# ArturKKK/graphcast-lite

Measured on AMD Instinct MI355X. Metric: training samples/sec (6h windows) + achieved HBM GB/s on mesh GCNConv, higher is better.
Workload: dtype f32

## Files before the change

### graphcast-lite_amd/csrc/aggregate.hip

```cpp
#include <algorithm>

#include <atomic>

#include "common.h"
#include "halo.h"
#include "mfma_io.h"

namespace {

template <int LPR, bool VL, bool VS, bool PRES, bool SPLIT>
__device__ __forceinline__ void agg_heavy_row(const int row, const int b, const int32_t* __restrict__ rowptr,
                                              const int32_t* __restrict__ col, const float* __restrict__ w,
                                              const float* __restrict__ H, int64_t ldh, int64_t bsh,
                                              const float* __restrict__ bias, float* __restrict__ Y, int64_t ldy,
                                              int64_t bsy, int32_t F, const int32_t* __restrict__ present,
                                              const float* __restrict__ H2, int64_t ldh2, int64_t bsh2, int32_t head) {
  constexpr int NG = 256 / LPR;
  __shared__ float red[NG][LPR * 4 + 1];
  const int g = threadIdx.x / LPR, l = threadIdx.x % LPR;
  const int c0 = l * 4;
  const bool cactive = c0 < F;
  const int cc = cactive ? c0 : 0;
  const float* __restrict__ Hb = H + (int64_t)b * bsh;
  const float* __restrict__ H2b = SPLIT ? H2 + (int64_t)b * bsh2 : nullptr;
  const int start = rowptr[row], end = rowptr[row + 1];
  float a0 = 0.f, a1 = 0.f, a2 = 0.f, a3 = 0.f;
  auto ld4 = [&](int j, float& x0, float& x1, float& x2, float& x3) {
    const float* p = Hb + (int64_t)j * ldh + cc;
    if (PRES) p = present[j] >= 0 ? p : reinterpret_cast<const float*>(gcl::mfma_io::zero4);
    if (SPLIT) p = j < head ? p : H2b + (int64_t)(j - head) * ldh2 + cc;
    if (VL) {
      const float4 v = *reinterpret_cast<const float4*>(p);
      x0 = v.x; x1 = v.y; x2 = v.z; x3 = v.w;
    } else {
      x0 = p[0];
      x1 = (cc + 1 < F) ? p[1] : 0.f;
      x2 = (cc + 2 < F) ? p[2] : 0.f;
      x3 = (cc + 3 < F) ? p[3] : 0.f;
    }
  };
  for (int e = start + g; e < end; e += 4 * NG) {
    const int e1 = e + NG, e2 = e + 2 * NG, e3 = e + 3 * NG;
    const int j0 = col[e], j1 = col[e1 < end ? e1 : e], j2 = col[e2 < end ? e2 : e], j3 = col[e3 < end ? e3 : e];
    const float w0 = w[e], w1 = e1 < end ? w[e1] : 0.f, w2 = e2 < end ? w[e2] : 0.f, w3 = e3 < end ? w[e3] : 0.f;
    float p0, p1, p2, p3, q0, q1, q2, q3, r0, r1, r2, r3, s0, s1, s2, s3;
    ld4(j0, p0, p1, p2, p3);
    ld4(j1, q0, q1, q2, q3);
    ld4(j2, r0, r1, r2, r3);
    ld4(j3, s0, s1, s2, s3);
    a0 += w0 * p0; a1 += w0 * p1; a2 += w0 * p2; a3 += w0 * p3;
    if (e1 < end) { a0 += w1 * q0; a1 += w1 * q1; a2 += w1 * q2; a3 += w1 * q3; }
    if (e2 < end) { a0 += w2 * r0; a1 += w2 * r1; a2 += w2 * r2; a3 += w2 * r3; }
    if (e3 < end) { a0 += w3 * s0; a1 += w3 * s1; a2 += w3 * s2; a3 += w3 * s3; }
  }
  red[g][c0] = a0; red[g][c0 + 1] = a1; red[g][c0 + 2] = a2; red[g][c0 + 3] = a3;
  __syncthreads();
  if (g == 0 && cactive) {
    float t0 = 0.f, t1 = 0.f, t2 = 0.f, t3 = 0.f;
#pragma unroll
    for (int q = 0; q < NG; ++q) { t0 += red[q][c0]; t1 += red[q][c0 + 1]; t2 += red[q][c0 + 2]; t3 += red[q][c0 + 3]; }
    if (bias) {
      t0 += bias[c0];
      if (c0 + 1 < F) t1 += bias[c0 + 1];
      if (c0 + 2 < F) t2 += bias[c0 + 2];
      if (c0 + 3 < F) t3 += bias[c0 + 3];
    }
    float* yp = Y + (int64_t)b * bsy + (int64_t)row * ldy + c0;
    if (VS) {
      *reinterpret_cast<float4*>(yp) = make_float4(t0, t1, t2, t3);
    } else {
      yp[0] = t0;
      if (c0 + 1 < F) yp[1] = t1;
      if (c0 + 2 < F) yp[2] = t2;
      if (c0 + 3 < F) yp[3] = t3;
    }
  }
}
// ... 13 lines not shown
}

template <int LPR, bool VL, bool VS, int EW, int ITER, bool PRES = false, bool SPLIT = false, bool HV = false>
__global__ __launch_bounds__(256) void agg_kernel(const int32_t* __restrict__ rowptr, const int32_t* __restrict__ col,
                                                  const float* __restrict__ w, const int32_t* __restrict__ ecol,
                                                  const float* __restrict__ ew, const float* __restrict__ H,
                                                  int64_t ldh, int64_t bsh, const float* __restrict__ bias,
                                                  float* __restrict__ Y, int64_t ldy, int64_t bsy, int32_t n,
                                                  int32_t B, int32_t F, int32_t nRB, int32_t xcd_map,
                                                  int32_t nt_store, const int32_t* __restrict__ order16,
                                                  const int32_t* __restrict__ present = nullptr,
                                                  const float* __restrict__ H2 = nullptr, int64_t ldh2 = 0,
                                                  int64_t bsh2 = 0, int32_t head = 0,
                                                  const int32_t* __restrict__ rows_heavy = nullptr, int32_t n_heavy = 0,
                                                  int32_t n_hb = 0, int32_t n_hb_pad = 0) {
  static_assert(!(PRES && SPLIT), "absent rows and a two-part source are not combined");
  constexpr int RPW = 64 / LPR;
  constexpr int EL = LPR < gcl::kEll ? LPR : gcl::kEll;
  static_assert(EW <= EL, "ELL width exceeds the lanes of a row group");
  int bid = blockIdx.x;
  if (HV) {
    if (bid < n_hb) {
      agg_heavy_row<LPR, VL, VS, PRES, SPLIT>(rows_heavy[bid % n_heavy], bid / n_heavy, rowptr, col, w, H, ldh, bsh, bias, Y, ldy,
                                              bsy, F, present, H2, ldh2, bsh2, head);
      return;
    }
    if (bid < n_hb_pad) return;
    bid -= n_hb_pad;
  }
  int b, rb;
  if (xcd_map) {
    const int xcd = bid & (gcl::kNumXCD - 1);
    const int slot = bid >> 3;
    b = xcd + gcl::kNumXCD * (slot / nRB);
    rb = slot % nRB;
  } else {
    b = bid / nRB;
    rb = bid % nRB;
  }
  if (b >= B) return;
  if (order16) {
    constexpr int RPB = RPW * 4 * ITER, K = 16 / RPB;
    rb = order16[rb / (K > 0 ? K : 1)] * (K > 0 ? K : 1) + rb % (K > 0 ? K : 1);
  }
  const int lane = threadIdx.x & 63;
  const int wave = threadIdx.x >> 6;
  const int sub = lane / LPR;
  const int l = lane % LPR;
  const int gbase = sub * LPR;
  const int c0 = l * 4;
  const bool cactive = c0 < F;
  const int cc = cactive ? c0 : 0;
  const float* __restrict__ Hb = H + (int64_t)b * bsh;
  const float* __restrict__ H2b = SPLIT ? H2 + (int64_t)b * bsh2 : nullptr;
  float* __restrict__ Yb = Y + (int64_t)b * bsy;

  float bz0 = 0.f, bz1 = 0.f, bz2 = 0.f, bz3 = 0.f;
  if (bias && cactive) {
    bz0 = bias[c0];
    if (VS || c0 + 1 < F) bz1 = bias[c0 + 1];
    if (VS || c0 + 2 < F) bz2 = bias[c0 + 2];
    if (VS || c0 + 3 < F) bz3 = bias[c0 + 3];
  }

  auto ld4 = [&](int j, float& x0, float& x1, float& x2, float& x3) {
    const float* p = Hb + (int64_t)j * ldh + cc;
    if (PRES) p = j >= 0 ? p : reinterpret_cast<const float*>(gcl::mfma_io::zero4);
    if (SPLIT) p = j < head ? p : H2b + (int64_t)(j - head) * ldh2 + cc;
    if (VL) {
      const float4 v = *reinterpret_cast<const float4*>(p);
      x0 = v.x; x1 = v.y; x2 = v.z; x3 = v.w;
    } else {
      x0 = p[0];
      x1 = (cc + 1 < F) ? p[1] : 0.f;
      x2 = (cc + 2 < F) ? p[2] : 0.f;
      x3 = (cc + 3 < F) ? p[3] : 0.f;
    }
  };

  const int row_first = (rb * 4 + wave) * (RPW * ITER) + sub;
  auto meta = [&](int row, int& start, int& end, int& cj, float& wj) {
    const int rc = row < n ? row : n - 1;
    start = rowptr[rc];
    end = rowptr[rc + 1];
    cj = ecol[(int64_t)rc * gcl::kEll + (l & (EL - 1))];
    wj = ew[(int64_t)rc * gcl::kEll + (l & (EL - 1))];
    if (PRES) cj = present[cj] >= 0 ? cj : -1;
  };
  int start, end, cj;
  float wj;
  meta(row_first, start, end, cj, wj);

#pragma unroll 1
  for (int it = 0; it < ITER; ++it) {
    const int row = row_first + it * RPW;
    int nstart = 0, nend = 0, ncj = 0;
    float nwj = 0.f;
    if (it + 1 < ITER) meta(row + RPW, nstart, nend, ncj, nwj);

    const int deg_all = end - start;
    const bool heavy = deg_all > gcl::kHeavy;
    const int deg = heavy ? 0 : deg_all;
    if (heavy) end = start;
    float a0 = 0.f, a1 = 0.f, a2 = 0.f, a3 = 0.f;
    {
      int jj[EW];
      float ww[EW], v0[EW], v1[EW], v2[EW], v3[EW];
// ... 250 lines not shown
            a0 = __fmaf_rn(wk, v.x, a0);
            a1 = __fmaf_rn(wk, v.y, a1);
            a2 = __fmaf_rn(wk, v.z, a2);
            a3 = __fmaf_rn(wk, v.w, a3);
          }
        }
      }
#undef GCL_HALO_MULADD
#undef GCL_HALO_FMA
      if (row < n && cactive && !(last & gcl::kHaloSkip)) {
        a0 += bz0; a1 += bz1; a2 += bz2; a3 += bz3;
        float* __restrict__ yp = Yb + (int64_t)row * ldy + c0;
        if (SMAP) {
          const int cr = sm[SMAP ? it : 0];
          yp = cr >= 0 ? Yc + (int64_t)b * bsc + (int64_t)cr * ldc + c0 : yp;
        }
        v4f v = {a0, a1, a2, a3};
        if (nt_store) __builtin_nontemporal_store(v, reinterpret_cast<v4f*>(yp));
        else *reinterpret_cast<v4f*>(yp) = v;
      }
    }
    GCL_AGG_STAMP(3)
#ifdef GCL_STAMPS
    st_acc[5] += 1;
#endif
    if (++m >= mend) break;
    __syncthreads();
    GCL_AGG_STAMP(4)
  }
#ifdef GCL_STAMPS
  if (lane == 0 && (blockIdx.x * NW + wave) < 4096)
    for (int i = 0; i < 8; ++i) agg_stamps[(blockIdx.x * NW + wave) * 8 + i] = st_acc[i];
#endif
}

#ifdef GCL_STAMPS
extern "C" int gcl_debug_read_agg_stamps(unsigned long long* host_out, int count) {
  GCL_CHECK_HIP(hipDeviceSynchronize());
  GCL_CHECK_HIP(hipMemcpyFromSymbol(host_out, HIP_SYMBOL(agg_stamps), sizeof(unsigned long long) * count));
  return GCL_OK;
}
#endif

struct AggArgs {
  const int32_t *rowptr, *col, *ecol, *heavy;
  const float *w, *ew;
  int ell_width, n_heavy;
  const gcl_halo* halo;
  const int32_t* order16 = nullptr;
  int32_t n_order16 = 0;
  const float* h2 = nullptr;
  int64_t ldh2 = 0, bsh2 = 0;
  int32_t head = 0;
  const int32_t* smap = nullptr;
  float* yc = nullptr;
  int64_t ldc = 0, bsc = 0;
  bool dry = false;
  bool heavy_inside = false;
};

template <int LPR>
int launch_agg_halo(const AggArgs& ga, const float* h, int64_t ldh, int64_t bsh, const float* bias, float* y,
                    int64_t ldy, int64_t bsy, int32_t n, int32_t B, int32_t F, hipStream_t st,
                    const int32_t* present = nullptr) {
  const int enabled = gcl::env_int("GCL_AGG_HALO", 1);
  static const int force_t = gcl::env_int("GCL_AGG_HALO_T", 0);
  static const int bpc_env = gcl::env_int("GCL_AGG_HALO_BPC", 0);
  static const int nt = gcl::env_int("GCL_AGG_NT", 1);
  if (!enabled || ga.ell_width != 8) return -1;
  if ((int64_t)n * ldh * 4 >= (int64_t)1 << 31 || ldh * 4 >= (int64_t)1 << 24 || n >= 1 << 24) return -1;
  constexpr int RPW = 64 / LPR;
  const gcl_halo* hl = nullptr;
  for (int t = 0; t < 2; ++t) {
    const gcl_halo& c = ga.halo[t];
    if (c.T == 0 || (force_t && c.T != force_t)) continue;
    const int64_t bytes = (int64_t)(c.smax + 1) * LPR * 16;
    if (bytes > 80 * 1024 || gcl::cdiv((c.smax - c.T) / RPW, 4) > 32) continue;
    hl = &c;
    break;
  }
  if (!hl) return -1;
  if (ga.dry) return GCL_OK;
  const int64_t lds = (int64_t)(hl->smax + 1) * LPR * 16;
  const int per_cu = (int)std::min<int64_t>(8, gcl::kLdsBytes / lds);
  const int J = 32 * (bpc_env > 0 ? bpc_env : per_cu);
  const int mpw = (int)gcl::cdiv((hl->smax - hl->T) / RPW, 4);
  dim3 grid((unsigned)(gcl::kNumXCD * J)), block(256);
  auto go = [&](auto kern) -> int {
    GCL_ENSURE_DYN_LDS(kern, (size_t)lds);
    hipLaunchKernelGGL(kern, grid, block, (size_t)lds, st, hl->list, hl->cnt, reinterpret_cast<const int2*>(hl->rec),
                       ga.rowptr, hl->opos, ga.w, hl->smax, h, ldh, bsh, bias, y, ldy, bsy, n, B, F, hl->ntiles, nt, present,
                       ga.smap, ga.yc, ga.ldc, ga.bsc);
    return GCL_OK;
  };
  int rc;
  if (ga.smap && hl->T == 64)
    rc = mpw <= 4 ? go(&agg_halo_loop_kernel<LPR, 64, 4, false, true>) : mpw <= 8 ? go(&agg_halo_loop_kernel<LPR, 64, 8, false, true>)
       : mpw <= 16 ? go(&agg_halo_loop_kernel<LPR, 64, 16, false, true>) : go(&agg_halo_loop_kernel<LPR, 64, 32, false, true>);
  else if (ga.smap)
    rc = mpw <= 4 ? go(&agg_halo_loop_kernel<LPR, 32, 4, false, true>) : mpw <= 8 ? go(&agg_halo_loop_kernel<LPR, 32, 8, false, true>)
       : mpw <= 16 ? go(&agg_halo_loop_kernel<LPR, 32, 16, false, true>) : go(&agg_halo_loop_kernel<LPR, 32, 32, false, true>);
  else if (present && hl->T == 64)
    rc = mpw <= 4 ? go(&agg_halo_loop_kernel<LPR, 64, 4, true>) : mpw <= 8 ? go(&agg_halo_loop_kernel<LPR, 64, 8, true>)
       : mpw <= 16 ? go(&agg_halo_loop_kernel<LPR, 64, 16, true>) : go(&agg_halo_loop_kernel<LPR, 64, 32, true>);
  else if (present)
    rc = mpw <= 4 ? go(&agg_halo_loop_kernel<LPR, 32, 4, true>) : mpw <= 8 ? go(&agg_halo_loop_kernel<LPR, 32, 8, true>)
       : mpw <= 16 ? go(&agg_halo_loop_kernel<LPR, 32, 16, true>) : go(&agg_halo_loop_kernel<LPR, 32, 32, true>);
  else if (hl->T == 64)
    rc = mpw <= 4 ? go(&agg_halo_loop_kernel<LPR, 64, 4>) : mpw <= 8 ? go(&agg_halo_loop_kernel<LPR, 64, 8>)
       : mpw <= 16 ? go(&agg_halo_loop_kernel<LPR, 64, 16>) : go(&agg_halo_loop_kernel<LPR, 64, 32>);
  else
    rc = mpw <= 4 ? go(&agg_halo_loop_kernel<LPR, 32, 4>) : mpw <= 8 ? go(&agg_halo_loop_kernel<LPR, 32, 8>)
       : mpw <= 16 ? go(&agg_halo_loop_kernel<LPR, 32, 16>) : go(&agg_halo_loop_kernel<LPR, 32, 32>);
  if (rc) return rc;
  GCL_CHECK_LAUNCH();
  return GCL_OK;
}

std::atomic<long long> g_heavy_launches{0};

template <int LPR>
int launch_agg_heavy(const AggArgs& ga, const float* h, int64_t ldh, int64_t bsh, const float* bias, float* y,
                     int64_t ldy, int64_t bsy, int32_t B, int32_t F, bool vl, bool vs, hipStream_t st,
                     const int32_t* present = nullptr) {
  g_heavy_launches.fetch_add(1, std::memory_order_relaxed);
  dim3 hgrid((unsigned)ga.n_heavy, (unsigned)B), block(256);
  if (ga.h2) {
    hipLaunchKernelGGL((agg_heavy_kernel<LPR, true, true, false, true>), hgrid, block, 0, st, ga.heavy, ga.rowptr, ga.col,
                       ga.w, h, ldh, bsh, bias, y, ldy, bsy, F, (const int32_t*)nullptr, ga.h2, ga.ldh2, ga.bsh2, ga.head);
    GCL_CHECK_LAUNCH();
    return GCL_OK;
  }
  if (present) {
#define GCL_AGGH(VL_, VS_)                                                                                       \
  hipLaunchKernelGGL((agg_heavy_kernel<LPR, VL_, VS_, true>), hgrid, block, 0, st, ga.heavy, ga.rowptr, ga.col, ga.w, \
                     h, ldh, bsh, bias, y, ldy, bsy, F, present)
    if (vl && vs) GCL_AGGH(true, true);
    else if (vl) GCL_AGGH(true, false);
    else if (vs) GCL_AGGH(false, true);
    else GCL_AGGH(false, false);
#undef GCL_AGGH
    GCL_CHECK_LAUNCH();
    return GCL_OK;
  }
#define GCL_AGGH(VL_, VS_)                                                                                       \
  hipLaunchKernelGGL((agg_heavy_kernel<LPR, VL_, VS_>), hgrid, block, 0, st, ga.heavy, ga.rowptr, ga.col, ga.w, h, \
                     ldh, bsh, bias, y, ldy, bsy, F, (const int32_t*)nullptr)
  if (vl && vs) GCL_AGGH(true, true);
  else if (vl) GCL_AGGH(true, false);
  else if (vs) GCL_AGGH(false, true);
  else GCL_AGGH(false, false);
#undef GCL_AGGH
  GCL_CHECK_LAUNCH();
  return GCL_OK;
}

template <int LPR>
int launch_agg(const AggArgs& ga, const float* h, int64_t ldh, int64_t bsh, const float* bias, float* y, int64_t ldy,
               int64_t bsy, int32_t n, int32_t B, int32_t F, hipStream_t st, const int32_t* present = nullptr) {
  constexpr int RPW = 64 / LPR;
  constexpr int EL = LPR < gcl::kEll ? LPR : gcl::kEll;
  if ((ga.smap || ga.dry) && ga.n_heavy > 0) return -1;
  const bool vl = (ldh % 4 == 0) && (bsh % 4 == 0) && gcl::aligned16(h) && ldh >= ((F + 3) / 4) * 4;
  const bool vs = (ldy % 4 == 0) && (bsy % 4 == 0) && gcl::aligned16(y) && (F % 4 == 0);
  if constexpr (LPR >= 16) {
    if (!ga.h2 && vl && vs && (!bias || gcl::aligned16(bias))) {
      const int hr = launch_agg_halo<LPR>(ga, h, ldh, bsh, bias, y, ldy, bsy, n, B, F, st, present);
      if (hr >= 0) {
        if (hr != GCL_OK || ga.n_heavy == 0 || ga.dry) return hr;
        return launch_agg_heavy<LPR>(ga, h, ldh, bsh, bias, y, ldy, bsy, B, F, true, true, st, present);
      }
    }
  }
  if (ga.smap || ga.dry) return -1;
  static const int iter_env = gcl::env_int("GCL_AGG_ITER", 0);
  static const int ew_env = gcl::env_int("GCL_AGG_EW", 0);
  static const int nt = gcl::env_int("GCL_AGG_NT", 1);
  int ewidth = ew_env > 0 ? ew_env : ga.ell_width;
  if (ewidth > EL) ewidth = EL;
  ewidth = ewidth >= 8 ? 8 : ewidth >= 4 ? 4 : ewidth >= 2 ? 2 : 1;
  const int iter = (!present && !ga.h2 && (iter_env == 1 || iter_env == 2 || iter_env == 4 || iter_env == 8)) ? iter_env
                                                                                                     : (ewidth >= 4 ? 1 : 2);
  int32_t nRB = (int32_t)gcl::cdiv(n, RPW * 4 * iter);
  if (ga.order16 && RPW * 4 * iter <= 16) nRB = ga.n_order16 * (16 / (RPW * 4 * iter));
  const int xcd_map = B >= gcl::kNumXCD ? 1 : 0;
  const int64_t nb = xcd_map ? (int64_t)gcl::kNumXCD * gcl::cdiv(B, gcl::kNumXCD) * nRB : (int64_t)B * nRB;
  GCL_CHECK_ARG(nb < (int64_t)INT32_MAX, "aggregate: grid too large");
  const bool hv = ga.heavy_inside && ga.n_heavy > 0 && vl && vs && iter == (ewidth >= 4 ? 1 : 2) && !gcl::env_int("GCL_AGG_HEAVY_SEPARATE", 0);
  const int32_t n_hb = hv ? ga.n_heavy * B : 0;
  const int32_t n_hb_pad = (int32_t)(gcl::cdiv(n_hb, gcl::kNumXCD) * gcl::kNumXCD);
  GCL_CHECK_ARG(nb + n_hb_pad < (int64_t)INT32_MAX, "aggregate: grid too large");
  dim3 grid((unsigned)nb), block(256), gridh((unsigned)(nb + n_hb_pad));
  const int32_t* order16 = (RPW * 4 * iter <= 16) ? ga.order16 : nullptr;
#define GCL_AGG4(VL_, VS_, EW_, IT_)                                                                             \
  hipLaunchKernelGGL((agg_kernel<LPR, VL_, VS_, EW_, IT_>), grid, block, 0, st, ga.rowptr, ga.col, ga.w, ga.ecol, \
                     ga.ew, h, ldh, bsh, bias, y, ldy, bsy, n, B, F, nRB, xcd_map, nt, order16, (const int32_t*)nullptr)
#define GCL_AGGP(VL_, VS_, EW_, IT_)                                                                                   \
  hipLaunchKernelGGL((agg_kernel<LPR, VL_, VS_, EW_, IT_, true>), grid, block, 0, st, ga.rowptr, ga.col, ga.w, ga.ecol, \
                     ga.ew, h, ldh, bsh, bias, y, ldy, bsy, n, B, F, nRB, xcd_map, nt, order16, present)
#define GCL_AGGH(EW_, IT_)                                                                                              \
  hipLaunchKernelGGL((agg_kernel<LPR, true, true, EW_, IT_, false, false, true>), gridh, block, 0, st, ga.rowptr, ga.col, \
                     ga.w, ga.ecol, ga.ew, h, ldh, bsh, bias, y, ldy, bsy, n, B, F, nRB, xcd_map, nt, order16,           \
                     (const int32_t*)nullptr, (const float*)nullptr, (int64_t)0, (int64_t)0, 0, ga.heavy, ga.n_heavy, n_hb, \
                     n_hb_pad)
#define GCL_AGGHP(EW_, IT_)                                                                                             \
  hipLaunchKernelGGL((agg_kernel<LPR, true, true, EW_, IT_, true, false, true>), gridh, block, 0, st, ga.rowptr, ga.col,  \
                     ga.w, ga.ecol, ga.ew, h, ldh, bsh, bias, y, ldy, bsy, n, B, F, nRB, xcd_map, nt, order16, present,  \
                     (const float*)nullptr, (int64_t)0, (int64_t)0, 0, ga.heavy, ga.n_heavy, n_hb, n_hb_pad)
#define GCL_AGGHS(EW_, IT_)                                                                                             \
  hipLaunchKernelGGL((agg_kernel<LPR, true, true, EW_, IT_, false, true, true>), gridh, block, 0, st, ga.rowptr, ga.col,  \
                     ga.w, ga.ecol, ga.ew, h, ldh, bsh, bias, y, ldy, bsy, n, B, F, nRB, xcd_map, nt, order16,           \
                     (const int32_t*)nullptr, ga.h2, ga.ldh2, ga.bsh2, ga.head, ga.heavy, ga.n_heavy, n_hb, n_hb_pad)
#define GCL_AGGS(EW_, IT_)                                                                                              \
  hipLaunchKernelGGL((agg_kernel<LPR, true, true, EW_, IT_, false, true>), grid, block, 0, st, ga.rowptr, ga.col, ga.w,  \
                     ga.ecol, ga.ew, h, ldh, bsh, bias, y, ldy, bsy, n, B, F, nRB, xcd_map, nt, order16,                \
                     (const int32_t*)nullptr, ga.h2, ga.ldh2, ga.bsh2, ga.head)
  if (ga.h2) {
    if (hv) {
      if constexpr (EL >= 8) {
        if (ewidth == 8) GCL_AGGHS(8, 1);
      }
      if (ewidth == 4) GCL_AGGHS(4, 1);
      else if (ewidth == 2) GCL_AGGHS(2, 2);
      else if (ewidth == 1) GCL_AGGHS(1, 2);
      GCL_CHECK_LAUNCH();
      return GCL_OK;
    }
    if constexpr (EL >= 8) {
      if (ewidth == 8) GCL_AGGS(8, 1);
    }
    if (ewidth == 4) GCL_AGGS(4, 1);
    else if (ewidth == 2) GCL_AGGS(2, 2);
    else if (ewidth == 1) GCL_AGGS(1, 2);
    GCL_CHECK_LAUNCH();
    if (ga.n_heavy > 0) return launch_agg_heavy<LPR>(ga, h, ldh, bsh, bias, y, ldy, bsy, B, F, true, true, st, nullptr);
    return GCL_OK;
  }
#define GCL_AGG3(VL_, VS_, EW_)              \
  do {                                       \
    if (present) {                           \
      if (EW_ >= 4) GCL_AGGP(VL_, VS_, EW_, 1); \
      else GCL_AGGP(VL_, VS_, EW_, 2);       \
    } else                                   \
    if (iter == 8) GCL_AGG4(VL_, VS_, EW_, 8); \
    else if (iter == 4) GCL_AGG4(VL_, VS_, EW_, 4); \
    else if (iter == 2) GCL_AGG4(VL_, VS_, EW_, 2); \
    else GCL_AGG4(VL_, VS_, EW_, 1);         \
  } while (0)
#define GCL_AGG2(VL_, VS_)                                        \
  do {                                                            \
    if constexpr (EL >= 8) { if (ewidth == 8) { GCL_AGG3(VL_, VS_, 8); break; } } \
    if (ewidth >= 4) GCL_AGG3(VL_, VS_, 4);                       \
    else if (ewidth == 2) GCL_AGG3(VL_, VS_, 2);                  \
    else GCL_AGG3(VL_, VS_, 1);                                   \
  } while (0)
  if (hv) {
    bool done = false;
    if constexpr (EL >= 8) {
      if (ewidth == 8) {
        if (present) GCL_AGGHP(8, 1);
        else GCL_AGGH(8, 1);
        done = true;
      }
    }
    if (done) {
    } else if (ewidth >= 4) {
      if (present) GCL_AGGHP(4, 1);
      else GCL_AGGH(4, 1);
    } else if (ewidth == 2) {
      if (present) GCL_AGGHP(2, 2);
// ... 43 lines not shown
  ga.w = transpose ? g->tw : g->w;
  ga.ecol = transpose ? g->tecol : g->ecol;
  ga.ew = transpose ? g->tew : g->ew;
  ga.ell_width = transpose ? g->tell_width : g->ell_width;
  ga.order16 = g->order16[transpose ? 1 : 0];
  ga.n_order16 = g->n_order16;
  ga.heavy = transpose ? g->theavy : g->heavy;
  ga.n_heavy = transpose ? g->n_theavy : g->n_heavy;
  ga.halo = g->halo[transpose ? 1 : 0];
  ga.h2 = h2;
  ga.ldh2 = ldh2;
  ga.bsh2 = bsh2;
  ga.head = head;
  GCL_CHECK_ARG(B <= 65535 || ga.n_heavy == 0, "aggregate: batch too large for the heavy-row launch");
  hipStream_t st = (hipStream_t)stream;
  const int lanes = (F + 3) / 4;
  if (lanes <= 4) return launch_agg<4>(ga, h, ldh, bsh, bias, y, ldy, bsy, g->n, B, F, st, present);
  if (lanes <= 8) return launch_agg<8>(ga, h, ldh, bsh, bias, y, ldy, bsy, g->n, B, F, st, present);
  if (lanes <= 16) return launch_agg<16>(ga, h, ldh, bsh, bias, y, ldy, bsy, g->n, B, F, st, present);
  if (lanes <= 32) return launch_agg<32>(ga, h, ldh, bsh, bias, y, ldy, bsy, g->n, B, F, st, present);
  return launch_agg<64>(ga, h, ldh, bsh, bias, y, ldy, bsy, g->n, B, F, st, present);
}

extern "C" int64_t gcl_aggregate_heavy_launches(void) { return (int64_t)g_heavy_launches.load(std::memory_order_relaxed); }

extern "C" int gcl_aggregate(const gcl_graph_t* g, int32_t transpose, const float* h, int64_t ldh, int64_t bsh,
                             const float* bias, float* y, int64_t ldy, int64_t bsy, int32_t B, int32_t F,
                             gcl_stream_t stream) {
  return aggregate_impl(g, transpose, h, ldh, bsh, nullptr, bias, y, ldy, bsy, B, F, stream);
}

extern "C" int gcl_aggregate_present(const gcl_graph_t* g, int32_t transpose, const float* h, int64_t ldh, int64_t bsh,
                                     const int32_t* present, const float* bias, float* y, int64_t ldy, int64_t bsy,
                                     int32_t B, int32_t F, gcl_stream_t stream) {
  GCL_CHECK_ARG(present, "aggregate_present: null presence table");
  return aggregate_impl(g, transpose, h, ldh, bsh, present, bias, y, ldy, bsy, B, F, stream);
}

extern "C" int gcl_aggregate_split(const gcl_graph_t* g, int32_t transpose, const float* h, int64_t ldh, int64_t bsh,
                                   const float* h2, int64_t ldh2, int64_t bsh2, int32_t head, const float* bias, float* y,
                                   int64_t ldy, int64_t bsy, int32_t B, int32_t F, gcl_stream_t stream) {
  GCL_CHECK_ARG(g && y, "aggregate_split: null argument");
  GCL_CHECK_ARG(head >= 0 && head <= g->n, "aggregate_split: head=%d outside [0, n=%d]", head, g->n);
  GCL_CHECK_ARG((h || head == 0) && (h2 || head == g->n), "aggregate_split: null source part");
  if (head == 0) h = h2;
  GCL_CHECK_ARG(F > 0 && F % 4 == 0 && ldh >= F && ldh2 >= F && ldh % 4 == 0 && bsh % 4 == 0 && ldh2 % 4 == 0 &&
                    bsh2 % 4 == 0 && ldy % 4 == 0 && bsy % 4 == 0 && gcl::aligned16(h) && gcl::aligned16(h2) &&
                    gcl::aligned16(y),
                "aggregate_split: both source parts and y need 16-byte rows (F %% 4 == 0, aligned bases and strides)");
  GCL_CHECK_ARG(h2 != y, "aggregate: in-place aggregation is not supported");
  return aggregate_impl(g, transpose, h, ldh, bsh, nullptr, bias, y, ldy, bsy, B, F, stream, h2, ldh2, bsh2, head);
}

extern "C" int gcl_aggregate_compact_ok(const gcl_graph_t* g, int32_t transpose, int64_t ldh, int64_t bsh, int64_t ldy,
                                        int64_t bsy, int32_t B, int32_t F) {
  if (!g || g->kind == GCL_GRAPH_GAT || B <= 0 || F <= 32 || F > 256 || F % 4 != 0 || ldh < F || ldy < F) return 0;
  AggArgs ca;
  ca.dry = true;
  return aggregate_impl(g, transpose, nullptr, ldh, bsh, nullptr, nullptr, nullptr, ldy, bsy, B, F, nullptr, nullptr, 0, 0, 0,
                        &ca) == GCL_OK ? 1 : 0;
}

extern "C" int gcl_aggregate_compact(const gcl_graph_t* g, int32_t transpose, const float* h, int64_t ldh, int64_t bsh,
                                     const int32_t* smap, float* y, int64_t ldy, int64_t bsy, float* yc, int64_t ldc,
                                     int64_t bsc, int32_t B, int32_t F, gcl_stream_t stream) {
  GCL_CHECK_ARG(g && smap, "aggregate_compact: null argument");
  GCL_CHECK_ARG(F % 4 == 0 && ldc >= F && ldc % 4 == 0 && bsc % 4 == 0 && gcl::aligned16(yc),
                "aggregate_compact: the compact destination needs 16-byte rows");
  GCL_CHECK_ARG(gcl_aggregate_compact_ok(g, transpose, ldh, bsh, ldy, bsy, B, F) && gcl::aligned16(h) && gcl::aligned16(y),
                "aggregate_compact: the source-tile kernel cannot take this call (ask gcl_aggregate_compact_ok first)");
  AggArgs ca;
  ca.smap = smap;
  ca.yc = yc;
  ca.ldc = ldc;
  ca.bsc = bsc;
  const int rc = aggregate_impl(g, transpose, h, ldh, bsh, nullptr, nullptr, y, ldy, bsy, B, F, stream, nullptr, 0, 0, 0, &ca);
  GCL_CHECK_ARG(rc != -1, "aggregate_compact: the source-tile kernel cannot take this call");
  return rc;
}
```

### graphcast-lite_amd/csrc/linear_x3.hip

```cpp
#include "mfma_io.h"
#include "x3.h"

namespace {

typedef unsigned int u32x2 __attribute__((ext_vector_type(2)));

#ifndef GCL_X3_ST_AUX
#define GCL_X3_ST_AUX 2
#endif
__device__ __forceinline__ float4 ld_stream(const float4* p) {
#ifndef GCL_X3_LD_PLAIN
  typedef float lv4f __attribute__((ext_vector_type(4)));
  const lv4f v = __builtin_nontemporal_load(reinterpret_cast<const lv4f*>(p));
  return make_float4(v.x, v.y, v.z, v.w);
#else
  return *p;
#endif
}
using namespace gcl::mfma_io;
using namespace gcl::x3;

constexpr int kRowB = 144;
constexpr int kImgB = 32 * kRowB;
constexpr int kTileB = 3 * kImgB;
// ... 151 lines not shown
        for (int c = 0; c < NS; ++c) acc[c] = mfma_mid(acc[c], ah, am, wf[c][s][0], wf[c][s][1]);
      }
#pragma unroll
      for (int s = 0; s < NKS; ++s) {
        const bf16x8 ah = *reinterpret_cast<const bf16x8*>(Aw + fo + s * 32);
#pragma unroll
        for (int c = 0; c < NS; ++c) acc[c] = mfma_hi(acc[c], ah, wf[c][s][0]);
      }
    }

#ifdef GCL_STAMPS
    asm volatile("" ::"v"(acc[0][0]));
#endif
    X3_STAMP(4);
    const int64_t r0 = t * 128 + wave * 32;
    const int64_t nr64 = rows - r0;
    const int nr = nr64 < 0 ? 0 : (nr64 < 32 ? (int)nr64 : 32);
    constexpr int OS = NS * 32, LPO = OS / 4, RPP = 64 / LPO;
    float* Ot = reinterpret_cast<float*>(Aw);
#pragma unroll
    for (int s = 0; s < NS; ++s)
#pragma unroll
      for (int r = 0; r < 16; ++r) Ot[d_row(r, lane) * OS + s * 32 + (lane & 31)] = acc[s][r];
    const __amdgpu_buffer_rsrc_t ry = make_rsrc(Y + r0 * ldy, (nr > 0 && !(abl & 1)) ? ((int64_t)(nr - 1) * ldy + N) * 4 : 0);
    const int orow = lane / LPO, ocol = (lane % LPO) * 4;
#pragma unroll
    for (int p = 0; p < 32 / RPP; ++p) {
      const int i = p * RPP + orow;
      float4 v = *reinterpret_cast<const float4*>(Ot + i * OS + ocol);
      v.x += bq.x; v.y += bq.y; v.z += bq.z; v.w += bq.w;
      buf_st4<GCL_X3_ST_AUX>(ry, (ocol < N) ? (unsigned)((i * ldy + ocol) * 4) : kOOB, v);
    }
    X3_STAMP(5);
  }
#ifdef GCL_STAMPS
  if (lane == 0 && blockIdx.x < 1024)
    for (int i = 0; i < 8; ++i) x3_stamps[(blockIdx.x * 4 + wave) * 8 + i] = stamp_acc[i];
#endif
}

constexpr int kBRowB = 128;
constexpr int kImg64B = 64 * kBRowB;
__device__ __forceinline__ int swz(int r) { return (((r >> 1) & 1) << 2) | (((r >> 3) & 1) << 1) | ((r >> 2) & 1); }
__device__ __forceinline__ int sw_off(int r, int b) { return r * kBRowB + ((((b >> 4) ^ swz(r)) << 4) | (b & 15)); }

typedef short s16x4 __attribute__((ext_vector_type(4)));
__device__ __forceinline__ bf16x8 tr_frag(const unsigned char* base, int o0, int o1) {
  typedef __attribute__((address_space(3))) s16x4 lds_s16x4;
  const s16x4 a = __builtin_amdgcn_ds_read_tr16_b64_v4i16((lds_s16x4*)(base + o0));
  const s16x4 b = __builtin_amdgcn_ds_read_tr16_b64_v4i16((lds_s16x4*)(base + o1));
  return __builtin_shufflevector(a, b, 0, 1, 2, 3, 4, 5, 6, 7);
}

template <int NO>
__global__ __launch_bounds__(256, 2) void linear_x3_bwd_kernel(
    const float* __restrict__ dY, int64_t lddy, const float* __restrict__ W, const float* __restrict__ P,
    int64_t ldp, const float* __restrict__ in_slope, float* __restrict__ dX, int64_t lddx, int64_t rows, int32_t Fin,
    int32_t Fout, float* __restrict__ part_dw, float* __restrict__ part_db, float* __restrict__ part_cs,
    double* __restrict__ part_slope) {
  constexpr int FoP = NO * 32, FiP = 64, NKO = NO * 2, NT = NO * 2;
  extern __shared__ __align__(16) unsigned char smem8[];
  unsigned char* Yimg = smem8;
  unsigned char* Pimg = smem8 + 3 * kImg64B;
  float* Stg = reinterpret_cast<float*>(smem8 + 6 * kImg64B);
  const int tid = threadIdx.x, lane = tid & 63, wave = __builtin_amdgcn_readfirstlane(tid >> 6);
  const int li = lane & 31, h = lane >> 5;
  const int rg = wave & 1, sg = wave >> 1;
  const int so = wave % NO, sc = wave / NO;
  const bool has_tile = wave < NT;

  bf16x8 wtf[NKO][3];
  {
    float2 wv[8];
#pragma unroll
    for (int i = 0; i < 8; ++i) {
      const int idx = i * 256 + tid;
      const int c = idx & 63, o = (idx >> 6) * 2;
      wv[i].x = (c < Fin && o < Fout) ? W[(int64_t)o * Fin + c] : 0.f;
      wv[i].y = (c < Fin && o + 1 < Fout) ? W[(int64_t)(o + 1) * Fin + c] : 0.f;
    }
#pragma unroll
    for (int i = 0; i < 8; ++i) {
      const int idx = i * 256 + tid;
      const int c = idx & 63, o = (idx >> 6) * 2;
      const Pk3 p = split2(wv[i].x, wv[i].y);
      unsigned char* d = Yimg + sw_off(c, o * 2);
      *reinterpret_cast<unsigned*>(d) = p.h;
      *reinterpret_cast<unsigned*>(d + kImg64B) = p.m;
      *reinterpret_cast<unsigned*>(d + 2 * kImg64B) = p.l;
    }
    __syncthreads();
#pragma unroll
    for (int s = 0; s < NKO; ++s)
#pragma unroll
      for (int p = 0; p < 3; ++p)
        wtf[s][p] = *reinterpret_cast<const bf16x8*>(Yimg + p * kImg64B + sw_off(32 * sg + li, (16 * s + 8 * h) * 2));
    __syncthreads();
  }

  const bool act = in_slope != nullptr;
  const float slope = act ? *in_slope : 1.f;
  const int64_t ntiles = (rows + 63) / 64;

  const int rsub = lane >> 4, csub = lane & 15;
  const bool yok = csub * 4 < Fout, pok = csub * 4 < Fin;
  const unsigned ym0 = csub * 4 < Fout ? ~0u : 0u, ym1 = csub * 4 + 1 < Fout ? ~0u : 0u, ym2 = csub * 4 + 2 < Fout ? ~0u : 0u,
                 ym3 = csub * 4 + 3 < Fout ? ~0u : 0u;
  float4 pre_y[4], pre_p[4];
  auto issue = [&](int64_t tile) {
    const int64_t r0 = tile * 64 + wave * 16;
#pragma unroll
    for (int it = 0; it < 4; ++it) {
      const int64_t row = r0 + it * 4 + rsub;
      const bool rok = row < rows;
      pre_y[it] = ld_stream((yok && rok) ? reinterpret_cast<const float4*>(dY + row * lddy + csub * 4) : zero4);
      pre_p[it] = ld_stream((pok && rok) ? reinterpret_cast<const float4*>(P + row * ldp + csub * 4) : zero4);
    }
  };

  int fo[NKO];
#pragma unroll
  for (int s = 0; s < NKO; ++s) fo[s] = sw_off(rg * 32 + li, (2 * s + h) * 16);
  const int g = lane >> 4, i16 = lane & 15;
  int troY[2], troP[2];
#pragma unroll
  for (int j = 0; j < 2; ++j) {
    const int r = 8 * (g >> 1) + 4 * j + (i16 >> 2), b = 32 * (g & 1) + 8 * (i16 & 3);
    troY[j] = sw_off(r, 64 * so + b);
    troP[j] = sw_off(r, 64 * sc + b);
  }

  f32x16 dw_hi, dw_lo;
#pragma unroll
  for (int r = 0; r < 16; ++r) dw_hi[r] = 0.f, dw_lo[r] = 0.f;
  float4 db4 = make_float4(0.f, 0.f, 0.f, 0.f), cs4 = make_float4(0.f, 0.f, 0.f, 0.f);
  double slope_acc = 0.0;
  float4 cur_p[4];

  issue(blockIdx.x);
#ifdef GCL_STAMPS
  unsigned long long stamp_acc[8] = {0, 0, 0, 0, 0, 0, 0, 0}, stamp_last = __builtin_amdgcn_s_memtime();
#endif
  for (int64_t t = blockIdx.x; t < ntiles; t += gridDim.x) {
#ifdef GCL_STAMPS
    asm volatile("s_waitcnt vmcnt(0)" ::: "memory");
#endif
    X3_STAMP(0);
#pragma unroll
    for (int it = 0; it < 4; ++it) {
      float4 y = pre_y[it];
      y.x = __uint_as_float(__float_as_uint(y.x) & ym0); y.y = __uint_as_float(__float_as_uint(y.y) & ym1);
      y.z = __uint_as_float(__float_as_uint(y.z) & ym2); y.w = __uint_as_float(__float_as_uint(y.w) & ym3);
      db4.x += y.x; db4.y += y.y; db4.z += y.z; db4.w += y.w;
      const float4 z = pre_p[it];
      cur_p[it] = z;
      float4 a;
      {
        const float mx = z.x * slope, my = z.y * slope, mz = z.z * slope, mw = z.w * slope;
        a.x = z.x > 0.f ? z.x : mx; a.y = z.y > 0.f ? z.y : my; a.z = z.z > 0.f ? z.z : mz; a.w = z.w > 0.f ? z.w : mw;
      }
      const Pk3 y01 = split2(y.x, y.y), y23 = split2(y.z, y.w), a01 = split2(a.x, a.y), a23 = split2(a.z, a.w);
      const int off = sw_off(wave * 16 + it * 4 + rsub, csub * 8);
      *reinterpret_cast<u32x2*>(Yimg + off) = u32x2{y01.h, y23.h};
      *reinterpret_cast<u32x2*>(Yimg + off + kImg64B) = u32x2{y01.m, y23.m};
      *reinterpret_cast<u32x2*>(Yimg + off + 2 * kImg64B) = u32x2{y01.l, y23.l};
      *reinterpret_cast<u32x2*>(Pimg + off) = u32x2{a01.h, a23.h};
      *reinterpret_cast<u32x2*>(Pimg + off + kImg64B) = u32x2{a01.m, a23.m};
      *reinterpret_cast<u32x2*>(Pimg + off + 2 * kImg64B) = u32x2{a01.l, a23.l};
    }
    X3_STAMP(1);
    __syncthreads();
    X3_STAMP(2);
    issue(t + gridDim.x);
    X3_STAMP(3);

    {
      f32x16 acc;
#pragma unroll
      for (int r = 0; r < 16; ++r) acc[r] = 0.f;
#pragma unroll
      for (int s = 0; s < NKO; ++s) {
        const bf16x8 ah = *reinterpret_cast<const bf16x8*>(Yimg + fo[s]);
        const bf16x8 am = *reinterpret_cast<const bf16x8*>(Yimg + fo[s] + kImg64B);
        const bf16x8 al = *reinterpret_cast<const bf16x8*>(Yimg + fo[s] + 2 * kImg64B);
        acc = mfma_lo(acc, ah, am, al, wtf[s][0], wtf[s][1], wtf[s][2]);
      }
#pragma unroll
      for (int s = 0; s < NKO; ++s) {
        const bf16x8 ah = *reinterpret_cast<const bf16x8*>(Yimg + fo[s]);
        const bf16x8 am = *reinterpret_cast<const bf16x8*>(Yimg + fo[s] + kImg64B);
        acc = mfma_mid(acc, ah, am, wtf[s][0], wtf[s][1]);
      }
#pragma unroll
      for (int s = 0; s < NKO; ++s) acc = mfma_hi(acc, *reinterpret_cast<const bf16x8*>(Yimg + fo[s]), wtf[s][0]);
#pragma unroll
      for (int r = 0; r < 16; ++r) Stg[(rg * 32 + d_row(r, lane)) * 64 + sg * 32 + li] = acc[r];
    }

    X3_STAMP(4);
    if (has_tile) {
#pragma unroll
      for (int s = 0; s < 4; ++s) {
        const unsigned char* ya = Yimg + s * 16 * kBRowB;
        const unsigned char* pa = Pimg + s * 16 * kBRowB;
        const bf16x8 ah = tr_frag(ya, troY[0], troY[1]), am = tr_frag(ya + kImg64B, troY[0], troY[1]),
                     al = tr_frag(ya + 2 * kImg64B, troY[0], troY[1]);
        const bf16x8 bh = tr_frag(pa, troP[0], troP[1]), bm = tr_frag(pa + kImg64B, troP[0], troP[1]),
                     bl = tr_frag(pa + 2 * kImg64B, troP[0], troP[1]);
        dw_lo = mfma_lo(dw_lo, ah, am, al, bh, bm, bl);
        dw_lo = mfma_mid(dw_lo, ah, am, bh, bm);
        dw_hi = mfma_hi(dw_hi, ah, bh);
      }
    }
#ifdef GCL_STAMPS
    asm volatile("" ::"v"(dw_hi[0]), "v"(dw_lo[0]));
#endif
    X3_STAMP(5);
    __syncthreads();
    X3_STAMP(6);

    {
      const int64_t r0 = t * 64;
      const int64_t nr = (rows - r0) < 64 ? (rows - r0) : 64;
      const __amdgpu_buffer_rsrc_t rx = make_rsrc(dX + r0 * lddx, nr > 0 ? ((nr - 1) * lddx + Fin) * 4 : 0);
#pragma unroll
      for (int it = 0; it < 4; ++it) {
        const int row = wave * 16 + it * 4 + rsub;
        float4 v = *reinterpret_cast<const float4*>(Stg + row * 64 + csub * 4);
        const float4 z = cur_p[it];
        const bool nx = act && z.x <= 0.f, ny = act && z.y <= 0.f, nz = act && z.z <= 0.f, nw = act && z.w <= 0.f;
        slope_acc += (double)(((nx ? v.x * z.x : 0.f) + (ny ? v.y * z.y : 0.f)) + ((nz ? v.z * z.z : 0.f) + (nw ? v.w * z.w : 0.f)));
        v.x = nx ? v.x * slope : v.x; v.y = ny ? v.y * slope : v.y; v.z = nz ? v.z * slope : v.z; v.w = nw ? v.w * slope : v.w;
        cs4.x += v.x; cs4.y += v.y; cs4.z += v.z; cs4.w += v.w;
        buf_st4<GCL_X3_ST_AUX>(rx, pok ? (unsigned)((row * lddx + csub * 4) * 4) : kOOB, v);
      }
    }
    X3_STAMP(7);
  }
#ifdef GCL_STAMPS
  if (lane == 0 && blockIdx.x < 1024)
    for (int i = 0; i < 8; ++i) x3_stamps[(blockIdx.x * 4 + wave) * 8 + i] = stamp_acc[i];
#endif

  constexpr size_t REC = (size_t)FoP * FiP + FoP + FiP;
  float* out = part_dw + (size_t)blockIdx.x * REC;
  if (has_tile) {
#pragma unroll
    for (int r = 0; r < 16; ++r) out[(size_t)(so * 32 + d_row(r, lane)) * FiP + sc * 32 + li] = dw_hi[r] + dw_lo[r];
  }
  __syncthreads();
  float* red = reinterpret_cast<float*>(smem8);
  {
    float* rdb = red + (wave * 4 + rsub) * 64 + csub * 4;
    *reinterpret_cast<float4*>(rdb) = db4;
    *reinterpret_cast<float4*>(rdb + 16 * 64) = cs4;
  }
  for (int off = 32; off > 0; off >>= 1) slope_acc += __shfl_down(slope_acc, off, 64);
  double* dred = reinterpret_cast<double*>(red + 2 * 16 * 64);
  if (lane == 0) dred[wave] = slope_acc;
  __syncthreads();
  if (tid < 128) {
    const int which = tid >> 6, c = tid & 63;
    float s = 0.f;
#pragma unroll
    for (int q = 0; q < 16; ++q) s += red[(which * 16 + q) * 64 + c];
    if (which == 0) {
      if (part_db && c < FoP) part_db[(size_t)blockIdx.x * REC + c] = s;
    } else {
      if (part_cs) part_cs[(size_t)blockIdx.x * REC + c] = s;
    }
  }
  if (part_slope && tid == 0) part_slope[blockIdx.x] = (dred[0] + dred[1]) + (dred[2] + dred[3]);
}

int x3_ablate() {
#ifndef GCL_STAMPS
  return 0;
#endif
  static const int v = gcl::env_int("GCL_ABLATE", 0);
  return v;
}

}

#ifdef GCL_STAMPS
extern "C" int gcl_debug_read_stamps_x3(unsigned long long* host_out, int count) {
  GCL_CHECK_HIP(hipDeviceSynchronize());
  GCL_CHECK_HIP(hipMemcpyFromSymbol(host_out, HIP_SYMBOL(x3_stamps), sizeof(unsigned long long) * count));
  return GCL_OK;
}
#endif

namespace gcl {

bool x3_linear_fwd_applicable(const float* x, int64_t ldx, const float* y, int64_t ldy, int K, int N, int akind) {
  if (!env_int("GCL_X3", 1)) return false;
  if (K < 1 || K > 64 || N < 4 || N > 64 || (N & 3)) return false;
  if ((ldx & 3) || (ldy & 3) || !aligned16(x) || !aligned16(y)) return false;
  if (ldx * 4 * 35 >= ((int64_t)1 << 31) || ldy * 4 * 35 >= ((int64_t)1 << 31)) return false;
  return akind == kActNone || akind == kActPrelu || akind == kActSilu;
}

int x3_linear_fwd(const float* x, int64_t ldx, int akind, const float* slope, const float* W, const float* bias,
                  float* y, int64_t ldy, int64_t rows, int K, int N, hipStream_t st) {
  if (rows == 0) return GCL_OK;
  const int64_t ntiles = cdiv(rows, 128);
  const int grid = (int)(ntiles < 2 * kNumCU ? ntiles : 2 * kNumCU);
  const size_t lds = 4 * (size_t)kTileB;
#define GCL_X3F3(NS_, SILU_, NKS_)                                                                                \
  hipLaunchKernelGGL((linear_x3_fwd_kernel<NS_, SILU_, NKS_>), dim3(grid), dim3(256), lds, st, x, ldx, slope, akind, \
                     W, bias, y, ldy, rows, K, N, x3_ablate())
#define GCL_X3F(NS_, SILU_)           \
  do {                                \
    if (K <= 32) GCL_X3F3(NS_, SILU_, 2); \
    else GCL_X3F3(NS_, SILU_, 4);     \
  } while (0)
  if (akind == kActSilu) {
    if (N > 32) GCL_X3F(2, true);
    else GCL_X3F(1, true);
  } else {
    if (N > 32) GCL_X3F(2, false);
    else GCL_X3F(1, false);
  }
#undef GCL_X3F3
#undef GCL_X3F
  GCL_CHECK_LAUNCH();
  return GCL_OK;
}

bool x3_linear_bwd_applicable(const float* dy, int64_t lddy, const float* x, int64_t ldx, const float* dx, int64_t lddx,
                              int Fin, int Fout) {
  if (!env_int("GCL_X3", 1)) return false;
  if (Fin < 33 || Fin > 64 || (Fin & 3) || Fout < 1 || Fout > 64) return false;
  if (lddy < ((Fout + 3) & ~3) || (lddy & 3) || (ldx & 3) || (lddx & 3) || lddx < Fin) return false;
  if (!aligned16(dy) || !aligned16(x) || !aligned16(dx)) return false;
  return lddx * 4 * 70 < ((int64_t)1 << 31);
}

int x3_linear_bwd_blocks(int64_t rows) {
  const int64_t ntiles = cdiv(rows, 64);
  return (int)(ntiles < 2 * kNumCU ? ntiles : 2 * kNumCU);
}

int x3_linear_bwd(const float* dy, int64_t lddy, const float* W, const float* x, int64_t ldx, const float* in_slope,
                  float* dx, int64_t lddx, int64_t rows, int Fin, int Fout, float* part_dw, float* part_db,
                  float* part_cs, double* part_slope, hipStream_t st) {
  const int grid = x3_linear_bwd_blocks(rows);
  const size_t lds = 6 * (size_t)kImg64B + 64 * 64 * sizeof(float);
#define GCL_X3B(NO_)                                                                                              \
  do {                                                                                                            \
    auto kern = linear_x3_bwd_kernel<NO_>;                                                                        \
    GCL_ENSURE_DYN_LDS(kern, gcl::kLdsBytes);                                                                     \
    hipLaunchKernelGGL(kern, dim3(grid), dim3(256), lds, st, dy, lddy, W, x, ldx, in_slope, dx, lddx, rows, Fin, Fout, \
                       part_dw, part_db, part_cs, part_slope);                                                    \
  } while (0)
  if (Fout > 32) GCL_X3B(2);
  else GCL_X3B(1);
#undef GCL_X3B
  GCL_CHECK_LAUNCH();
  return GCL_OK;
}

}
```

### graphcast-lite_amd/csrc/misc.hip

```cpp
#include "common.h"

namespace {

struct Walk3 {
  int c, i, C, N, sc, si;
  int64_t b, sb;
  __device__ __forceinline__ Walk3(int64_t idx, int64_t stride, int N_, int C_) : C(C_), N(N_) {
    c = (int)(idx % C_);
    const int64_t r = idx / C_;
    i = (int)(r % N_);
    b = r / N_;
    sc = (int)(stride % C_);
    const int64_t t = stride / C_;
    si = (int)(t % N_);
    sb = t / N_;
  }
  __device__ __forceinline__ void next() {
    c += sc;
    i += si;
    b += sb;
    if (c >= C) { c -= C; ++i; }
    if (i >= N) { i -= N; ++b; }
  }
};

__global__ __launch_bounds__(256) void assemble_kernel(const float* __restrict__ x, const float* __restrict__ gs,
                                                       const float* __restrict__ ms, float* __restrict__ out,
                                                       int64_t ldo, int32_t B, int32_t G, int32_t M, int32_t Cdyn,
                                                       int32_t Cs, const float* __restrict__ tail, int32_t r) {
  const int C = Cdyn + Cs;
  const int64_t total = (int64_t)B * (G + M) * C;
  const int64_t stride = (int64_t)gridDim.x * 256;
  int64_t idx = (int64_t)blockIdx.x * 256 + threadIdx.x;
  for (Walk3 w(idx, stride, G + M, C); idx < total; idx += stride, w.next()) {
    const int c = w.c, i = w.i;
    const int64_t b = w.b;
    float v;
    if (i < G)
      v = c < Cdyn ? x[(b * G + i) * Cdyn + c] : gs[(int64_t)i * Cs + (c - Cdyn)];
    else if (i >= G + M - r)
      v = tail[(b * r + (i - (G + M - r))) * C + c];
    else
      v = c < Cdyn ? 0.f : ms[(int64_t)(i - G) * Cs + (c - Cdyn)];
    out[(b * (G + M) + i) * ldo + c] = v;
  }
}

__global__ __launch_bounds__(256) void assemble4_kernel(const float* __restrict__ x, const float* __restrict__ gs,
                                                        const float* __restrict__ ms, float* __restrict__ out,
                                                        int64_t ldo, int32_t B, int32_t G, int32_t M, int32_t Cdyn,
                                                        int32_t Cs, const float* __restrict__ tail, int32_t r) {
  const int C4 = (Cdyn + Cs) >> 2;
  const int64_t total = (int64_t)B * (G + M) * C4;
  const int64_t stride = (int64_t)gridDim.x * 256;
  int64_t idx = (int64_t)blockIdx.x * 256 + threadIdx.x;
  for (Walk3 w(idx, stride, G + M, C4); idx < total; idx += stride, w.next()) {
    const int c0 = w.c * 4, i = w.i;
    const int64_t b = w.b;
    float v[4];
#pragma unroll
    for (int q = 0; q < 4; ++q) {
      const int c = c0 + q;
      if (i < G)
        v[q] = c < Cdyn ? x[(b * G + i) * Cdyn + c] : gs[(int64_t)i * Cs + (c - Cdyn)];
      else if (i >= G + M - r)
        v[q] = tail[(b * r + (i - (G + M - r))) * (Cdyn + Cs) + c];
      else
        v[q] = c < Cdyn ? 0.f : ms[(int64_t)(i - G) * Cs + (c - Cdyn)];
    }
    *reinterpret_cast<float4*>(out + (b * (G + M) + i) * ldo + c0) = make_float4(v[0], v[1], v[2], v[3]);
  }
}

__global__ __launch_bounds__(256) void wmse_kernel(const float* __restrict__ delta, int64_t ldd, int64_t bsd,
                                                   const float* __restrict__ xl, int64_t ldx, int64_t bsx,
                                                   const float* __restrict__ y, int64_t ldy, int64_t bsy,
                                                   const float* __restrict__ node_w, const float* __restrict__ chan_w,
                                                   float inv_wsum, float grad_scale, float* __restrict__ dd,
                                                   float* __restrict__ out_state, float* __restrict__ part,
                                                   int32_t B, int32_t G, int32_t C) {
  __shared__ float red[4];
  const int64_t total = (int64_t)B * G * C;
  float acc = 0.f;
  const int64_t stride = (int64_t)gridDim.x * 256;
  int64_t idx = (int64_t)blockIdx.x * 256 + threadIdx.x;
  for (Walk3 wk(idx, stride, G, C); idx < total; idx += stride, wk.next()) {
    const int c = wk.c, g = wk.i;
    const int64_t b = wk.b;
    float o = delta[b * bsd + (int64_t)g * ldd + c];
    if (xl) o += xl[b * bsx + (int64_t)g * ldx + c];
    const float t = y[b * bsy + (int64_t)g * ldy + c];
    float w = 1.f;
    if (chan_w) w *= chan_w[c];
    if (node_w) w *= node_w[g];
    const float d = o - t;
    acc += (d * d) * w;
    if (dd) dd[idx] = 2.f * w * d * inv_wsum * grad_scale;
    if (out_state) out_state[idx] = o;
  }
  for (int off = 32; off > 0; off >>= 1) acc += __shfl_down(acc, off, 64);
  if ((threadIdx.x & 63) == 0) red[threadIdx.x >> 6] = acc;
  __syncthreads();
  if (threadIdx.x == 0) part[blockIdx.x] = red[0] + red[1] + red[2] + red[3];
}

__global__ void wmse_final_kernel(const float* __restrict__ part, int32_t nparts, float inv_wsum,
                                  const float* __restrict__ loss_prev, float* __restrict__ loss) {
  __shared__ double red[4];
  double s = 0.0;
  for (int p = threadIdx.x; p < nparts; p += 256) s += (double)part[p];
  for (int off = 32; off > 0; off >>= 1) s += __shfl_down(s, off, 64);
  if ((threadIdx.x & 63) == 0) red[threadIdx.x >> 6] = s;
  __syncthreads();
  if (threadIdx.x == 0) {
    const float l = (float)((red[0] + red[1] + red[2] + red[3]) * (double)inv_wsum);
    *loss = loss_prev ? *loss_prev + l : l;
  }
}

__global__ __launch_bounds__(256) void adam_kernel(float* __restrict__ p, const float* __restrict__ g,
                                                   float* __restrict__ m, float* __restrict__ v, int64_t count,
                                                   float lr, float b1, float b2, float eps, float wd, float bc1,
                                                   float bc2_sqrt, float gscale) {
  for (int64_t i = (int64_t)blockIdx.x * 256 + threadIdx.x; i < count; i += (int64_t)gridDim.x * 256) {
    float pi = p[i], mi = m[i], vi = v[i];
    gcl::adam_elem(pi, g[i], mi, vi, lr, b1, b2, eps, wd, bc1, bc2_sqrt, gscale);
    m[i] = mi;
    v[i] = vi;
    p[i] = pi;
  }
}

__global__ void adam_tick_kernel(int32_t* __restrict__ step, float* __restrict__ bc, float b1, float b2) {
  const int t = *step + 1;
  *step = t;
  bc[0] = (float)(1.0 - pow((double)b1, (double)t));
  bc[1] = (float)sqrt(1.0 - pow((double)b2, (double)t));
}

__global__ __launch_bounds__(256) void adam_dev_kernel(float* __restrict__ p, const float* __restrict__ g,
                                                       float* __restrict__ m, float* __restrict__ v, int64_t count,
                                                       float lr, float b1, float b2, float eps, float wd,
                                                       const float* __restrict__ bc, float gscale) {
  const float bc1 = bc[0], bc2_sqrt = bc[1];
  for (int64_t i = (int64_t)blockIdx.x * 256 + threadIdx.x; i < count; i += (int64_t)gridDim.x * 256) {
    float gi = g[i] * gscale;
    if (wd != 0.f) gi += wd * p[i];
    const float mi = b1 * m[i] + (1.f - b1) * gi;
    const float vi = b2 * v[i] + (1.f - b2) * gi * gi;
    m[i] = mi;
// ... 127 lines not shown
}

__global__ __launch_bounds__(256) void window_pack_kernel(const _Float16* __restrict__ series, int64_t T, int32_t n_lon,
                                                          int32_t n_lat, int32_t Ct, const int64_t* __restrict__ t0,
                                                          const float* __restrict__ mean, const float* __restrict__ stdv,
                                                          int32_t C, int32_t first, int32_t frames,
                                                          float* __restrict__ out, int32_t B) {
  const int64_t G = (int64_t)n_lon * n_lat;
  const int64_t row = (int64_t)frames * C;
  const int64_t total = (int64_t)B * G * row;
  for (int64_t idx = (int64_t)blockIdx.x * 256 + threadIdx.x; idx < total; idx += (int64_t)gridDim.x * 256) {
    const int k = (int)(idx % row);
    const int64_t bg = idx / row;
    const int64_t g = bg % G;
    const int b = (int)(bg / G);
    const int f = k / C, c = k - f * C;
    const int lat = (int)(g / n_lon), lon = (int)(g - (int64_t)lat * n_lon);
    const int64_t t = t0[b] + first + f;
    float v = __builtin_nanf("");
    if (t >= 0 && t < T) {
      const float x = (float)series[(((int64_t)t * n_lon + lon) * n_lat + lat) * Ct + c];
      v = (x - mean[c]) / stdv[c];
    }
    out[idx] = v;
  }
}

__global__ __launch_bounds__(256) void ar_step_bwd_kernel(const float* __restrict__ dd, const float* __restrict__ g_loss,
                                                          const float* __restrict__ g_new,
                                                          const int32_t* __restrict__ chan_kind, int32_t has_y,
                                                          int32_t residual, float* __restrict__ d_delta,
                                                          float* __restrict__ d_state, int32_t B, int32_t G, int32_t obs,
                                                          int32_t C) {
  const float gl = g_loss ? *g_loss : 1.f;
  const int64_t total = (int64_t)B * G * obs * C;
  const int64_t stride = (int64_t)gridDim.x * 256;
  int64_t idx = (int64_t)blockIdx.x * 256 + threadIdx.x;
  for (Walk3 w(idx, stride, obs, C); idx < total; idx += stride, w.next()) {
    const int c = w.c, k = w.i;
    const int64_t bg = w.b;
    float ds = (g_new && k >= 1) ? g_new[idx - C] : 0.f;
    if (k == obs - 1) {
      int kind = chan_kind ? chan_kind[c] : 0;
      if (kind == 2 && !has_y) kind = 0;
      const float gd = gl * dd[bg * C + c];
      const float gn = g_new ? g_new[idx] : 0.f;
      d_delta[bg * C + c] = gd + (kind == 0 ? gn : 0.f);
      ds += (residual ? gd : 0.f) + ((kind == 1 || (kind == 0 && residual)) ? gn : 0.f);
    }
    if (d_state) d_state[idx] = ds;
  }
}

__global__ __launch_bounds__(256) void pad_rows_kernel(const float* __restrict__ src, int64_t lds, int64_t bss,
                                                       int32_t rows_src, int32_t F_src, float* __restrict__ dst,
                                                       int64_t ldd, int64_t bsd, int32_t rows_dst, int32_t F_dst,
                                                       int32_t B) {
  const int64_t total = (int64_t)B * rows_dst * F_dst;
  const int64_t stride = (int64_t)gridDim.x * 256;
  int64_t idx = (int64_t)blockIdx.x * 256 + threadIdx.x;
  for (Walk3 w(idx, stride, rows_dst, F_dst); idx < total; idx += stride, w.next()) {
    const int c = w.c, r = w.i;
    const int64_t b = w.b;
    const bool in = r < rows_src && c < F_src;
    dst[b * bsd + (int64_t)r * ldd + c] = in ? src[b * bss + (int64_t)r * lds + c] : 0.f;
  }
}

using gcl::grid_for;
constexpr int kLossBlocks = 1024;

}

extern "C" int gcl_assemble_input(const float* x, const float* gs, const float* ms, float* out, int64_t ldo,
                                  int32_t B, int32_t G, int32_t M, int32_t Cdyn, int32_t Cs, gcl_stream_t stream) {
  return gcl_assemble_input_tail(x, gs, ms, nullptr, 0, out, ldo, B, G, M, Cdyn, Cs, stream);
}

extern "C" int gcl_assemble_input_tail(const float* x, const float* gs, const float* ms, const float* tail, int32_t r,
                                       float* out, int64_t ldo, int32_t B, int32_t G, int32_t M, int32_t Cdyn, int32_t Cs,
                                       gcl_stream_t stream) {
  GCL_CHECK_ARG(x && gs && (ms || r == M) && out, "assemble_input: null argument");
  GCL_CHECK_ARG(B > 0 && G > 0 && M >= 0 && Cdyn >= 0 && Cs >= 0 && ldo >= Cdyn + Cs, "assemble_input: bad shape");
  GCL_CHECK_ARG(r >= 0 && r <= M && (r == 0 || tail), "assemble_input: tail rows r=%d outside [0, M=%d] or no tail", r, M);
  const int64_t total = (int64_t)B * (G + M) * (Cdyn + Cs);
  if (((Cdyn + Cs) & 3) == 0 && (ldo & 3) == 0 && gcl::aligned16(out))
    hipLaunchKernelGGL(assemble4_kernel, dim3(grid_for(total / 4, 8192)), dim3(256), 0, (hipStream_t)stream, x, gs, ms, out,
                       ldo, B, G, M, Cdyn, Cs, tail, r);
  else
    hipLaunchKernelGGL(assemble_kernel, dim3(grid_for(total, 8192)), dim3(256), 0, (hipStream_t)stream, x, gs, ms, out,
                     ldo, B, G, M, Cdyn, Cs, tail, r);
  GCL_CHECK_LAUNCH();
  return GCL_OK;
}

extern "C" size_t gcl_wmse_ws_bytes(int32_t B, int32_t G, int32_t C) {
  (void)B; (void)G; (void)C;
  return (size_t)kLossBlocks * sizeof(float);
}

extern "C" int gcl_wmse_fwd_bwd(const float* delta, int64_t ldd, int64_t bsd, const float* x_last, int64_t ldx,
                                int64_t bsx, const float* y, int64_t ldy, int64_t bsy, const float* node_w,
                                const float* chan_w, float inv_wsum, float grad_scale, float* d_delta,
                                float* out_state, const float* loss_prev, float* loss_out, int32_t B, int32_t G,
                                int32_t C, void* ws, size_t ws_bytes, gcl_stream_t stream) {
  GCL_CHECK_ARG(delta && y && loss_out, "wmse: null argument");
  GCL_CHECK_ARG(B > 0 && G > 0 && C > 0 && ldd >= C && ldy >= C && (!x_last || ldx >= C), "wmse: bad shape");
  GCL_CHECK_ARG(ws && ws_bytes >= gcl_wmse_ws_bytes(B, G, C), "wmse: workspace too small");
  hipStream_t st = (hipStream_t)stream;
  const int64_t total = (int64_t)B * G * C;
  const unsigned nb = grid_for(total, kLossBlocks);
  hipLaunchKernelGGL(wmse_kernel, dim3(nb), dim3(256), 0, st, delta, ldd, bsd, x_last, ldx, bsx, y, ldy, bsy, node_w,
                     chan_w, inv_wsum, grad_scale, d_delta, out_state, (float*)ws, B, G, C);
  hipLaunchKernelGGL(wmse_final_kernel, dim3(1), dim3(256), 0, st, (const float*)ws, (int)nb, inv_wsum, loss_prev,
                     loss_out);
  GCL_CHECK_LAUNCH();
  return GCL_OK;
}

extern "C" int gcl_adam_step(float* p, const float* g, float* m, float* v, int64_t count, float lr, float beta1,
                             float beta2, float eps, float weight_decay, int32_t step, float grad_scale,
                             gcl_stream_t stream) {
  GCL_CHECK_ARG(p && g && m && v, "adam: null argument");
  GCL_CHECK_ARG(count >= 0 && step >= 1, "adam: bad count/step");
  if (count == 0) return GCL_OK;
  const double bc1 = 1.0 - pow((double)beta1, (double)step);
  const double bc2 = 1.0 - pow((double)beta2, (double)step);
  hipLaunchKernelGGL(adam_kernel, dim3(grid_for(count, 1024)), dim3(256), 0, (hipStream_t)stream, p, g, m, v, count,
                     lr, beta1, beta2, eps, weight_decay, (float)bc1, (float)sqrt(bc2), grad_scale);
  GCL_CHECK_LAUNCH();
  return GCL_OK;
}

extern "C" int gcl_copy_rows(const float* src, int64_t lds, int64_t bss, float* dst, int64_t ldd, int64_t bsd,
                             int32_t B, int32_t rows, int32_t F, gcl_stream_t stream) {
  GCL_CHECK_ARG(src && dst, "copy_rows: null argument");
  GCL_CHECK_ARG(B > 0 && rows >= 0 && F > 0 && lds >= F && ldd >= F, "copy_rows: bad shape");
  if (rows == 0) return GCL_OK;
  const int vec = (F % 4 == 0) && (lds % 4 == 0) && (ldd % 4 == 0) && (bss % 4 == 0) && (bsd % 4 == 0) &&
                  gcl::aligned16(src) && gcl::aligned16(dst);
  const int64_t total = (int64_t)B * rows * (vec ? F / 4 : F);
  hipLaunchKernelGGL(copy_rows_kernel, dim3(grid_for(total, 8192)), dim3(256), 0, (hipStream_t)stream, src, lds, bss,
                     dst, ldd, bsd, B, rows, F, vec);
  GCL_CHECK_LAUNCH();
  return GCL_OK;
}

extern "C" int gcl_gather2_rows(const float* a, int64_t lda, int64_t bsa, const int32_t* map_a, const float* b,
                                int64_t ldb, int64_t bsb, const int32_t* map_b, float* dst, int64_t ldd, int64_t bsd,
                                int32_t B, int32_t nd, int32_t F, int32_t sum_batch, gcl_stream_t stream) {
  GCL_CHECK_ARG(a && dst, "gather2_rows: null argument");
  GCL_CHECK_ARG(B > 0 && nd >= 0 && F > 0 && F % 4 == 0, "gather2_rows: F must be a positive multiple of 4 (F=%d)", F);
  GCL_CHECK_ARG(lda % 4 == 0 && bsa % 4 == 0 && ldd % 4 == 0 && bsd % 4 == 0 && gcl::aligned16(a) && gcl::aligned16(dst) &&
                    (!b || (ldb % 4 == 0 && bsb % 4 == 0 && gcl::aligned16(b))),
                "gather2_rows: rows must be 16-B aligned");
  if (nd == 0) return GCL_OK;
  if (sum_batch && !gcl::env_int("GCL_NO_BATCH_SUM", 0)) {
    const int64_t tot = (int64_t)nd * (F / 4);
    const int bs = tot < (int64_t)256 * gcl::kNumCU * 4 ? 64 : 256;
    const int64_t nbl = gcl::cdiv(tot, bs);
    const unsigned nb = (unsigned)(nbl > 8192 ? 8192 : nbl);
    hipLaunchKernelGGL(batch_sum_rows_kernel, dim3(nb), dim3(bs), 0, (hipStream_t)stream, a, lda, bsa, map_a, dst, ldd,
                       bsd, B, nd, F / 4, sum_batch);
    GCL_CHECK_LAUNCH();
    return GCL_OK;
  }
  const int64_t total = (int64_t)(sum_batch ? 1 : B) * nd * (F / 4);
  hipLaunchKernelGGL(gather2_kernel, dim3(grid_for(total, 8192)), dim3(256), 0, (hipStream_t)stream, a, lda, bsa, map_a,
                     b, ldb, bsb, map_b, dst, ldd, bsd, B, nd, F / 4, sum_batch);
  GCL_CHECK_LAUNCH();
  return GCL_OK;
}

extern "C" int gcl_adam_step_dev(float* p, const float* g, float* m, float* v, int64_t count, float lr, float beta1,
                                 float beta2, float eps, float weight_decay, int32_t* step_dev, float* bc_dev,
                                 float grad_scale, gcl_stream_t stream) {
  GCL_CHECK_ARG(p && g && m && v && step_dev && bc_dev, "adam_dev: null argument");
  GCL_CHECK_ARG(count >= 0, "adam_dev: bad count");
  hipStream_t st = (hipStream_t)stream;
  hipLaunchKernelGGL(adam_tick_kernel, dim3(1), dim3(1), 0, st, step_dev, bc_dev, beta1, beta2);
  if (count > 0)
    hipLaunchKernelGGL(adam_dev_kernel, dim3(grid_for(count, 1024)), dim3(256), 0, st, p, g, m, v, count, lr, beta1,
                       beta2, eps, weight_decay, bc_dev, grad_scale);
  GCL_CHECK_LAUNCH();
  return GCL_OK;
}

extern "C" int gcl_ar_step_bwd(const float* dd, const float* g_loss, const float* g_new, const int32_t* chan_kind,
                               int32_t has_y, int32_t residual, float* d_delta, float* d_state, int32_t B, int32_t G,
                               int32_t obs, int32_t C, gcl_stream_t stream) {
  GCL_CHECK_ARG(dd && d_delta, "ar_step_bwd: null argument");
  GCL_CHECK_ARG(B > 0 && G > 0 && obs >= 1 && C > 0, "ar_step_bwd: bad shape");
  const int64_t total = (int64_t)B * G * obs * C;
  hipLaunchKernelGGL(ar_step_bwd_kernel, dim3(grid_for(total, 8192)), dim3(256), 0, (hipStream_t)stream, dd, g_loss,
                     g_new, chan_kind, has_y, residual, d_delta, d_state, B, G, obs, C);
  GCL_CHECK_LAUNCH();
  return GCL_OK;
}

extern "C" int gcl_pad_rows(const float* src, int64_t lds, int64_t bss, int32_t rows_src, int32_t F_src, float* dst,
                            int64_t ldd, int64_t bsd, int32_t rows_dst, int32_t F_dst, int32_t B, gcl_stream_t stream) {
  GCL_CHECK_ARG(src && dst, "pad_rows: null argument");
  GCL_CHECK_ARG(B > 0 && rows_src >= 0 && rows_dst >= rows_src && F_src >= 0 && F_dst >= F_src && lds >= F_src && ldd >= F_dst,
                "pad_rows: bad shape");
  const int64_t total = (int64_t)B * rows_dst * F_dst;
  if (total > 0)
    hipLaunchKernelGGL(pad_rows_kernel, dim3(grid_for(total, 8192)), dim3(256), 0, (hipStream_t)stream, src, lds, bss,
                       rows_src, F_src, dst, ldd, bsd, rows_dst, F_dst, B);
  GCL_CHECK_LAUNCH();
  return GCL_OK;
}

extern "C" int gcl_zero(void* ptr, size_t nbytes, gcl_stream_t stream) {
  GCL_CHECK_ARG(ptr || nbytes == 0, "zero: null argument");
  if (nbytes) GCL_CHECK_HIP(hipMemsetAsync(ptr, 0, nbytes, (hipStream_t)stream));
  return GCL_OK;
}

extern "C" int gcl_ar_advance(const float* state, const float* delta, int64_t ldd, int64_t bsd, const float* y_step,
                              int64_t ldy, int64_t bsy, const int32_t* chan_kind, float* new_state, float* out,
                              int64_t ldo, int64_t bso, int32_t out_off, int32_t B, int32_t G, int32_t obs, int32_t C,
                              int32_t residual, gcl_stream_t stream) {
  GCL_CHECK_ARG(state && delta && new_state, "ar_advance: null argument");
  GCL_CHECK_ARG(ldd >= C, "ar_advance: delta row stride smaller than C");
  GCL_CHECK_ARG(state != new_state, "ar_advance: the window shift cannot be done in place");
  GCL_CHECK_ARG(B > 0 && G > 0 && obs >= 1 && C > 0, "ar_advance: bad shape");
  GCL_CHECK_ARG(!out || (ldo >= out_off + C), "ar_advance: output row too short for out_off + C");
  const int64_t total = (int64_t)B * G * obs * C;
  hipLaunchKernelGGL(ar_advance_kernel, dim3(grid_for(total, 8192)), dim3(256), 0, (hipStream_t)stream, state, delta,
                     ldd, bsd, y_step, ldy, bsy, chan_kind, new_state, out, ldo, bso, out_off, B, G, obs, C, residual);
  GCL_CHECK_LAUNCH();
  return GCL_OK;
}

extern "C" int gcl_window_pack(const uint16_t* series, int64_t T, int32_t n_lon, int32_t n_lat, int32_t Ct,
                               const int64_t* t0, const float* mean, const float* stdv, int32_t C, int32_t obs,
                               int32_t pred, float* X, float* Y, int32_t B, gcl_stream_t stream) {
  GCL_CHECK_ARG(series && t0 && mean && stdv && X, "window_pack: null argument");
  GCL_CHECK_ARG(T > 0 && n_lon > 0 && n_lat > 0 && Ct > 0 && C > 0 && C <= Ct && obs > 0 && pred >= 0 && B > 0,
                "window_pack: bad shape (T=%lld grid %dx%d C=%d of %d obs=%d pred=%d)", (long long)T, n_lon, n_lat, C, Ct,
                obs, pred);
  GCL_CHECK_ARG(pred == 0 || Y, "window_pack: pred > 0 needs the Y buffer");
  const int64_t G = (int64_t)n_lon * n_lat;
  hipLaunchKernelGGL(window_pack_kernel, dim3(grid_for((int64_t)B * G * obs * C, 16384)), dim3(256), 0,
                     (hipStream_t)stream, (const _Float16*)series, T, n_lon, n_lat, Ct, t0, mean, stdv, C, 0, obs, X, B);
  if (pred > 0)
    hipLaunchKernelGGL(window_pack_kernel, dim3(grid_for((int64_t)B * G * pred * C, 16384)), dim3(256), 0,
                       (hipStream_t)stream, (const _Float16*)series, T, n_lon, n_lat, Ct, t0, mean, stdv, C, obs, pred, Y, B);
  GCL_CHECK_LAUNCH();
  return GCL_OK;
}
```

### graphcast-lite_amd/functional.py

```python
from typing import List, Optional

import os

import torch

from . import hip


def _grad_slot(p: Optional[torch.Tensor], needs: bool):
    if p is None or not needs:
        return None, False, True
    if p.grad is not None:
        return p.grad, True, True
    return torch.zeros_like(p), False, False


class _Grads:

    def __init__(self, params: List[Optional[torch.Tensor]], needs: List[bool]):
        self.dst, self.acc, self.ret_none = [], [], []
        for p, nd in zip(params, needs):
            d, a, r = _grad_slot(p, nd)
            self.dst.append(d)
            self.acc.append(a)
            self.ret_none.append(r)

    def out(self):
        return tuple(None if r else d for d, r in zip(self.dst, self.ret_none))


_ZERO = {}


def _token(like: torch.Tensor, shape):
    z = _ZERO.get(like.device)
    if z is None:
        if like.is_cuda and torch.cuda.is_current_stream_capturing():
            return like.new_zeros(()).expand(shape)
        with torch.inference_mode(False):
            z = _ZERO[like.device] = torch.zeros((), dtype=torch.float32, device=like.device)
    return z.expand(shape)


def _flat3(x: torch.Tensor):
    if x.dim() == 2:
        x = x.unsqueeze(0)
    if not x.is_contiguous():
        x = x.contiguous()
    return x


class MLPFn(torch.autograd.Function):
    @staticmethod
    def forward(ctx, x, owner, has_ln: bool, eps: float, *params):
        L = (len(params) - (2 if has_ln else 0) + 1) // 3
        shape = x.shape
        x2 = hip.rows2d(x.detach())
        zs = []
        cur, slope = x2, None
        for k in range(L):
            W, b = params[3 * k], params[3 * k + 1]
            z = hip.linear_fwd(cur, W.detach(), b.detach(), slope)
            zs.append(z)
            cur = z
            slope = params[3 * k + 2].detach() if k < L - 1 else None
        stats = None
        out = cur
        if has_ln:
            out, stats = hip.layernorm_fwd(cur, params[-2].detach(), params[-1].detach(), eps)
        ctx.owner, ctx.has_ln, ctx.L = owner, has_ln, L
        ctx.x2, ctx.zs, ctx.stats = x2, zs, stats
        ctx.params = params
        return out.view(shape[:-1] + (out.shape[-1],))

    @staticmethod
    def backward(ctx, dy):
        params, L = ctx.params, ctx.L
        needs = list(ctx.needs_input_grad[4:])
        G = _Grads(list(params), needs)
        dy2 = hip.rows2d(dy)
        zs = ctx.zs
        if ctx.has_ln:
            gi, bi = len(params) - 2, len(params) - 1
            dgam = G.dst[gi] if G.dst[gi] is not None else torch.zeros_like(params[gi])
            dbet = G.dst[bi] if G.dst[bi] is not None else torch.zeros_like(params[bi])
            dz = hip.layernorm_bwd(dy2, zs[-1], params[gi].detach(), ctx.stats, dgam, dbet, G.acc[gi] and G.acc[bi])
        else:
            dz = dy2
        dx = None
        for k in range(L - 1, -1, -1):
            W = params[3 * k].detach()
            inp = ctx.x2 if k == 0 else zs[k - 1]
            slope = None if k == 0 else params[3 * k - 1].detach()
            wi, bi = 3 * k, 3 * k + 1
# ... 148 lines not shown
                split.keep_split_out(tail)
                ps.append(None)
                cur = _token(cur, (B, n, Fout))
                continue
            if hip.gcn_layer_fusable(graph, cur, W.shape[1], Fout):
                last_rows = int(out_rows) if (k == L - 1 and out_rows and out_rows < n and not has_ln and _ROWS_OUT) else None
                p = hip.gcn_layer_fwd(graph, cur, act_k, slope_k, W, b, rows_out=last_rows,
                                      present=present if k == L - 1 else None)
                if k == L - 1 and ldh != Fout and not has_ln:
                    pad_last = (ldh, Fout, None)
                elif ldh != Fout:
                    p = p.contiguous()
                ps.append(p)
                cur = p
                continue
            if k == L - 1 and ldh != Fout and not has_ln:
                Wp = torch.nn.functional.pad(W, (0, 0, 0, ldh - Fout))
                bp = torch.nn.functional.pad(b, (0, ldh - Fout))
                h = hip.linear_fwd(cur.reshape(B * n, -1), Wp, None, slope_k, act=act_k)
                p = hip.aggregate(graph, h.view(B, n, ldh), bp)
                ps.append(p)
                cur = p[..., :Fout]
                pad_last = (ldh, Fout, Wp)
                continue
            h = hip.linear_fwd(cur.reshape(B * n, -1) if not cur.is_contiguous() else cur.view(B * n, -1), W, None, slope_k,
                               ld_out=ldh, act=act_k)
            h3 = torch.as_strided(h, (B, n, Fout), (n * ldh, ldh, 1))
            p = hip.aggregate(graph, h3, b)
            ps.append(p)
            cur = p
        ctx.akind, ctx.slope_t, ctx.pad_last = akind, slope_t, pad_last
        out, stats = cur, None
        if mapped:
            stats = land.ln_write(cur.view(B * n, -1), params[-2].detach(), params[-1].detach(), eps, present is not None)
            out = _token(cur, (B, n, cur.shape[2]))
        elif has_ln:
            o2, stats = hip.layernorm_fwd(cur.view(B * n, -1), params[-2].detach(), params[-1].detach(), eps)
            out = o2.view(B, n, -1)
        ctx.land, ctx.present = land, present
        ctx.owner, ctx.graph, ctx.L, ctx.has_ln = owner, graph, L, has_ln
        ctx.x3, ctx.ps, ctx.stats, ctx.params, ctx.squeeze = x3, ps, stats, params, squeeze
        ctx.n_rows, ctx.out_rows = n, (int(out_rows) if out_rows and out_rows < n else 0)
        if ctx.out_rows:
            out = out[:, :ctx.out_rows, :]
        return out[0] if squeeze else out

    @staticmethod
    def backward(ctx, dy):
        params, L, graph = ctx.params, ctx.L, ctx.graph
        needs = list(ctx.needs_input_grad[10:])
        G = _Grads(list(params), needs)
        dy, parts = GradLanding.claim_parts(ctx.split, dy)
        dy, dy_map = GradLanding.claim(ctx.land, dy)
        dy3 = dy if (dy_map is not None or parts is not None) else _flat3(dy)
        B, n = dy3.shape[0], ctx.n_rows
        ps = ctx.ps
        pad = ctx.pad_last
        dy_rows = dy3
        if ctx.out_rows and (ctx.has_ln or pad is None):
            dy3 = hip.pad_rows(dy3, n, dy3.shape[2])
        bi_last = 2 * L - 1
        cs_done = False
        if ctx.has_ln:
            gi, bi = len(params) - 2, len(params) - 1
            dgam = G.dst[gi] if G.dst[gi] is not None else torch.zeros_like(params[gi])
            dbet = G.dst[bi] if G.dst[bi] is not None else torch.zeros_like(params[bi])
            cs = G.dst[bi_last] if (pad is None and _LN_COLSUM) else None
            if ctx.present is not None and dy_map is None:
                raise RuntimeError("the processor's output received a gradient from outside the decoder-input gather, but its "
                                   "dropped rows were not kept (set GCL_NO_ROW_SKIP=1 to keep them)")
            dp = hip.layernorm_bwd(None if dy_map is not None else dy3.view(B * n, -1), ps[-1].view(B * n, -1),
                                   params[gi].detach(), ctx.stats, dgam, dbet, G.acc[gi] and G.acc[bi], colsum_dx=cs,
                                   acc_colsum=bool(cs is not None and G.acc[bi_last]), dy_map=dy_map,
                                   skip=ctx.present is not None).view(B, n, -1)
            cs_done = cs is not None
        else:
            dp = dy3
        si = 2 * L
        dsl = G.dst[si] if params[si] is not None else None
        slope_t, akind = ctx.slope_t, ctx.akind
        dx = None
        Fo = params[2 * (L - 1)].shape[0]
        Fp = Fo
        if pad is not None:
            Fp = pad[0]
            dp = hip.pad_rows(dy_rows if not ctx.has_ln else dp, n, Fp)
        if G.dst[bi_last] is not None and not cs_done:
            src = dy_rows if not ctx.has_ln else dp[..., :Fo]
            if parts is not None:
                hip.colsum_split(parts[0], parts[1], G.dst[bi_last], G.acc[bi_last])
            else:
                hip.colsum(src.reshape(-1, Fo), G.dst[bi_last], G.acc[bi_last])
        dzc = None
        assert ctx.present is None or parts is None
        for k in range(L - 1, -1, -1):
            W = params[2 * k].detach()
            wi = 2 * k
            inp = (ctx.x3 if k == 0 else ps[k - 1]).view(-1, (ctx.x3 if k == 0 else ps[k - 1]).shape[-1])
            if k == L - 1 and ctx.present is not None:
                dh2 = hip.aggregate_present(graph, dp, ctx.present, transpose=True).view(B * n, -1)
            elif k == L - 1 and parts is not None:
                dh2 = hip.aggregate_split(graph, parts[0], parts[1], transpose=True).view(B * n, -1)
            elif (k == 0 and ctx.lat is not None and ctx.lat.smap is not None and ctx.lat.Md > 0 and _compact_store()
                  and dp.is_contiguous() and hip.aggregate_compact_ok(graph, dp, transpose=True)):
                dzc = torch.empty(B, ctx.lat.Md + ctx.lat.r, dp.shape[2], dtype=torch.float32, device=dp.device)
                dh2 = hip.aggregate_compact(graph, dp, ctx.lat.smap, dzc, transpose=True).view(B * n, -1)
            else:
                dh2 = hip.aggregate(graph, dp, None, transpose=True).view(B * n, -1)
            if k == L - 1 and Fp != Fo:
                dh2 = dh2[:, :Fo]
            dW = G.dst[wi] if G.dst[wi] is not None else torch.zeros_like(params[wi])
            if k > 0:
                dp = hip.linear_bwd_all(dh2, W, inp, slope_t, dsl, dW, None, G.dst[2 * k - 1], G.acc[wi],
                                        acc_colsum=G.acc[2 * k - 1], act=akind).view(B, n, -1)
            elif ctx.lat is not None:
                if ctx.enc_shape is not None:
                    dx = _lat_first_layer_bwd(ctx.lat, None, dh2.reshape(B, n, -1), W, dW, G.acc[wi], ctx.needs_input_grad[0],
                                              Pc=ctx.x3, enc_shape=ctx.enc_shape, dzc=dzc)
                else:
                    dx = _lat_first_layer_bwd(ctx.lat, ctx.x3, dh2.reshape(B, n, -1), W, dW, G.acc[wi],
                                              ctx.needs_input_grad[0], dzc=dzc)
            elif ctx.needs_input_grad[0]:
                dx = hip.linear_bwd_all(dh2, W, inp, None, None, dW, None, None, G.acc[wi],
                                        act=hip.ACT_NONE).view(B, n, -1)
            else:
                hip.linear_bwd_dw(dh2, inp, None, dW, None, G.acc[wi])
        if dx is not None and ctx.squeeze:
            dx = dx[0]
        return (dx,) + (None,) * 9 + G.out()


class GATLayerFn(torch.autograd.Function):

    @staticmethod
    def forward(ctx, x, owner, graph, H: int, want_alpha: bool, act, lat, slope, W, att_src, att_dst, bias):
        squeeze = x.dim() == 2
        tail = lat.tail if lat is not None else None
        x3 = x.detach() if tail is not None else _flat3(x.detach())
        B, n, _ = x3.shape
        Cc = W.shape[0] // H
        sl = slope.detach() if slope is not None else None
        ctx.lat = ctx.tab = None
        if lat is not None:
            assert sl is None, "a LatSource feeds the first layer of a stack (no input activation)"
            if tail is None and not x3.is_contiguous():
                x3 = x3.contiguous()
            ne, D = x3.shape[1], x3.shape[2]
            nc = lat.Md + lat.r
            Pc = tail if tail is not None else \
                hip.copy_rows(x3[:, lat.G:, :], torch.empty(B, nc, D, dtype=torch.float32, device=x3.device))
            h = hip.linear_fwd(Pc.view(B * nc, D), W.detach(), None, None, act=act).view(B, nc, H * Cc)
            ctx.lat, ctx.tab, ctx.enc_shape = lat, lat.compact_tab(ne), x3.shape
            x3 = Pc
            GradLanding.expect_tail(lat.landing)
        else:
# ... 112 lines not shown
        y = hip.aggregate(graph, x3, None)
        return y[0] if squeeze else y

    @staticmethod
    def backward(ctx, dy):
        dx = hip.aggregate(ctx.graph, _flat3(dy), None, transpose=True)
        return (dx[0] if ctx.squeeze else dx), None


class AssembleFn(torch.autograd.Function):

    @staticmethod
    def forward(ctx, x, grid_static, mesh_static, tail3=None):
        squeeze = x.dim() == 2
        x3 = _flat3(x.detach())
        ctx.squeeze, ctx.G, ctx.Cdyn = squeeze, x3.shape[1], x3.shape[2]
        out = hip.assemble_input(x3, grid_static, mesh_static, tail3)
        return out[0] if squeeze else out

    @staticmethod
    def backward(ctx, dy):
        dy3 = dy if dy.dim() == 3 else dy.unsqueeze(0)
        dx = dy3[:, : ctx.G, : ctx.Cdyn].contiguous()
        return (dx[0] if ctx.squeeze else dx), None, None, None


class WeightedMSEFn(torch.autograd.Function):

    @staticmethod
    def forward(ctx, delta, x_last, y, node_w, chan_w, inv_wsum: float):
        loss, dd, _ = hip.wmse_fwd_bwd(delta.detach(), x_last, y, node_w, chan_w, inv_wsum, 1.0, want_grad=True)
        ctx.dd = dd
        return loss

    @staticmethod
    def backward(ctx, g):
        d = ctx.dd * g
        return d, (d if ctx.needs_input_grad[1] else None), None, None, None, None


class ARStepLossFn(torch.autograd.Function):

    @staticmethod
    def forward(ctx, state4, delta3, y3, loss_prev, node_w, chan_w, inv_wsum: float, kinds, residual: bool,
                advance: bool):
        st = state4.detach()
        if not st.is_contiguous():
            st = st.contiguous()
        B, G, obs, Cc = st.shape
        d3 = delta3.detach()
        if d3.stride(2) != 1:
            d3 = d3.contiguous()
        x_last = st[:, :, obs - 1, :] if residual else None
        loss, dd, _ = hip.wmse_fwd_bwd(d3, x_last, y3, node_w, chan_w, inv_wsum, 1.0, want_grad=True,
                                       loss_prev=loss_prev.detach() if loss_prev is not None else None)
        new_state = hip.ar_advance(st, d3, y3, kinds, None, 0, residual) if advance else st.new_empty(0)
        ctx.dd, ctx.kinds, ctx.residual, ctx.advance, ctx.obs, ctx.has_y = dd, kinds, residual, advance, obs, y3 is not None
        if not advance:
            ctx.mark_non_differentiable(new_state)
        return loss, new_state

    @staticmethod
    def backward(ctx, g_loss, g_new):
        g_new = g_new if (ctx.advance and g_new is not None and g_new.numel()) else None
        d_delta, d_state = hip.ar_step_bwd(ctx.dd, g_loss, g_new, ctx.kinds, ctx.has_y, ctx.residual, ctx.obs,
                                           want_state=ctx.needs_input_grad[0])
        return d_state, d_delta, None, (g_loss if ctx.needs_input_grad[3] else None), None, None, None, None, None, None


class Gather2Fn(torch.autograd.Function):

    @staticmethod
    def forward(ctx, a, b, maps, nd: int, B: int, landing=None):
        map_a, map_b, inv_a, inv_b = maps
        a3 = a.detach()
        ctx.maps, ctx.B, ctx.landing = maps, B, landing
        ctx.sa, ctx.sb = a3.shape, (b.shape if b is not None else None)
        buf = landing.take_decoder_input(a3) if landing is not None else None
        if buf is not None:
            return buf
        if not a3.is_contiguous():
            a3 = a3.contiguous()
        b3 = b.detach() if b is not None else None
        if b3 is not None and not b3.is_contiguous():
            b3 = b3.contiguous()
        return hip.gather2_rows(a3, map_a, b3, map_b, nd, B)

    @staticmethod
    def backward(ctx, g):
        map_a, map_b, inv_a, inv_b = ctx.maps
        g = g.contiguous()
        da = db = None
        land = ctx.landing
        if ctx.needs_input_grad[0]:
            bc = ctx.sa[0] == 1 and ctx.B > 1
            if land is not None and not bc:
                da = land.head_grad(g, inv_a, ctx.sa, ctx.B)
            if da is None:
                da = hip.gather2_rows(g, inv_a, None, None, ctx.sa[1], ctx.B, sum_batch=bc)
        if ctx.sb is not None and ctx.needs_input_grad[1]:
            bc = ctx.sb[0] == 1 and ctx.B > 1
            if land is not None and not bc:
                db = land.offer(g, inv_b, ctx.sb)
            if db is None:
                db = hip.gather2_rows(g, inv_b, None, None, ctx.sb[1], ctx.B, sum_batch=bc)
        return da, db, None, None, None, None


class GradLanding:

    def __init__(self, head: int, head_identity: bool = False):
        self.head, self.buf, self.mesh_pending = head, None, False
        self.head_identity, self.split_ready, self.part_head, self.part_tail = head_identity, False, None, None
        self.proc_ready, self.proc_src, self.proc_map = False, None, None
        self.dec_buf, self.dec_map, self.dec_rows, self.dec_filled = None, None, None, False
        self.out_wanted, self.out_tail, self.dec_head_placed = False, None, False

    @staticmethod
    def expect_tail(land):
# ... 291 lines not shown
```

### graphcast-lite_amd/hip.py

```python
import ctypes as C
import os
from typing import Optional

import torch

_HERE = os.path.dirname(os.path.abspath(__file__))
LIB_PATH = os.environ.get("GCL_LIB") or os.path.join(_HERE, "libgcl_hip.so")

GRAPH_GCN, GRAPH_GAT, GRAPH_MEAN = 0, 1, 2

_lib = None

_i32, _i64, _f32, _vp, _sz = C.c_int32, C.c_int64, C.c_float, C.c_void_p, C.c_size_t

_SIGNATURES = {
    "gcl_version": (C.c_int, []),
    "gcl_last_error": (C.c_char_p, []),
    "gcl_graph_count_edges": (C.c_int, [_vp, _i64, _i32, _i32, C.POINTER(_i64)]),
    "gcl_graph_build_host": (C.c_int, [_vp, _i64, _i32, _i32] + [_vp] * 8),
    "gcl_graph_create": (C.c_int, [_vp, _i64, _i32, _i32, C.POINTER(_vp)]),
    "gcl_graph_destroy": (None, [_vp]),
    "gcl_graph_num_nodes": (_i32, [_vp]),
    "gcl_graph_num_edges": (_i64, [_vp]),
    "gcl_graph_max_in_degree": (_i32, [_vp]),
    "gcl_graph_export_edges": (C.c_int, [_vp, _vp]),
    "gcl_graph_eperm_device": (_vp, [_vp]),
    "gcl_graph_halo_info": (C.c_int, [_vp, _i32, _i32, _vp]),
    "gcl_linear_fwd": (C.c_int, [_vp, _i64, _vp, _vp, _vp, _vp, _i64, _i64, _i32, _i32, _vp]),
    "gcl_linear_bwd_dx": (C.c_int, [_vp, _i64, _vp, _vp, _i64, _vp, _vp, _vp, _i64, _i64, _i32, _i32, _vp, _sz, _vp]),
    "gcl_linear_bwd_dw": (C.c_int, [_vp, _i64, _vp, _i64, _vp, _vp, _vp, _i64, _i32, _i32, _i32, _vp, _sz, _vp]),
    "gcl_linear_bwd_ws_bytes": (_sz, [_i64, _i32, _i32]),
    "gcl_linear_bwd_all": (C.c_int, [_vp, _i64, _vp, _vp, _i64, _vp, _vp, _vp, _i64, _vp, _vp, _vp, _i64, _i32, _i32,
                                     _i32, _vp, _sz, _vp]),
    "gcl_linear_bwd_all_deferred": (C.c_int, [_vp, _i64, _vp, _vp, _i64, _vp, _vp, _vp, _i64, _vp, _vp, _vp, _i64, _i32,
                                              _i32, _i32, _vp, _sz, _vp, _vp]),
    "gcl_reduce_jobs": (C.c_int, [_vp, _i32, _vp]),
    "gcl_layernorm_bwd_deferred": (C.c_int, [_vp, _i64, _i64, _vp, _i32, _i32, _vp, _i64, _vp, _vp, _vp, _i64, _vp, _vp, _vp,
                                             _i32, _i64, _i32, _vp, _sz, _vp, _vp]),
    "gcl_colsum_deferred": (C.c_int, [_vp, _i64, _i64, _i32, _vp, _i32, _vp, _sz, _vp, _vp]),
    "gcl_colsum_split_deferred": (C.c_int, [_vp, _i64, _i64, _vp, _i64, _i64, _i32, _i32, _i32, _i32, _vp, _i32, _vp, _sz,
                                            _vp, _vp]),
    "gcl_linear_bwd_dw_deferred": (C.c_int, [_vp, _i64, _vp, _i64, _vp, _vp, _vp, _i64, _i32, _i32, _i32, _vp, _sz, _vp,
                                             _vp]),
    "gcl_dense_bwd_dw_deferred": (C.c_int, [_vp, _i64, _vp, _i64, _i32, _vp, _vp, _i64, _vp, _i64, _i32, _i32, _i32, _vp,
                                            C.c_size_t, _vp, _vp]),
    "gcl_linear_bwd_all_ws_bytes": (_sz, [_i64, _i32, _i32]),
    "gcl_aggregate": (C.c_int, [_vp, _i32, _vp, _i64, _i64, _vp, _vp, _i64, _i64, _i32, _i32, _vp]),
    "gcl_aggregate_present": (C.c_int, [_vp, _i32, _vp, _i64, _i64, _vp, _vp, _vp, _i64, _i64, _i32, _i32, _vp]),
    "gcl_aggregate_compact_ok": (C.c_int, [_vp, _i32, _i64, _i64, _i64, _i64, _i32, _i32]),
    "gcl_aggregate_compact": (C.c_int, [_vp, _i32, _vp, _i64, _i64, _vp, _vp, _i64, _i64, _vp, _i64, _i64, _i32, _i32, _vp]),
    "gcl_aggregate_heavy_launches": (_i64, []),
    "gcl_aggregate_split": (C.c_int, [_vp, _i32, _vp, _i64, _i64, _vp, _i64, _i64, _i32, _vp, _vp, _i64, _i64, _i32, _i32,
                                      _vp]),
    "gcl_gat_fwd": (C.c_int, [_vp, _vp, _i64, _i64, _vp, _vp, _vp, _vp, _vp, _vp, _vp, _i64, _i64, _i32, _i32, _i32, _vp]),
    "gcl_gat_bwd": (C.c_int, [_vp, _vp, _i64, _i64, _vp, _i64, _i64, _vp, _vp, _vp, _vp, _vp, _vp, _i64, _i64,
                              _vp, _vp, _vp, _i32, _i32, _i32, _i32, _vp, _sz, _vp]),
    "gcl_gat_bwd_ws_bytes": (_sz, [_i64, _i32, _i32, _i32, _i32]),
    "gcl_gat_fwd_tab": (C.c_int, [_vp, _vp, _i64, _i64, _vp, _vp, _vp, _vp, _vp, _vp, _vp, _vp, _i64, _i64, _i32, _i32, _i32, _vp]),
    "gcl_gat_bwd_tab": (C.c_int, [_vp, _vp, _i64, _i64, _vp, _i64, _i64, _vp, _vp, _vp, _vp, _vp, _vp, _vp, _i64, _i64,
                                  _vp, _vp, _vp, _i32, _i32, _i32, _i32, _vp, _sz, _vp]),
    "gcl_gat_tab_ok": (C.c_int, [_vp, _i64, _i32, _i32]),
    "gcl_gat_alpha_to_edge_order": (C.c_int, [_vp, _vp, _vp, _i32, _vp]),
    "gcl_gat_prune": (C.c_int, [_vp, _vp, _f32, _vp, C.POINTER(_i64), _vp, _sz, _vp]),
    "gcl_gat_prune_ws_bytes": (_sz, [_i64]),
    "gcl_layernorm_fwd": (C.c_int, [_vp, _i64, _vp, _vp, _f32, _vp, _i64, _vp, _i64, _i32, _vp]),
    "gcl_layernorm_bwd": (C.c_int, [_vp, _i64, _vp, _i64, _vp, _vp, _vp, _i64, _vp, _vp, _i32, _i64, _i32, _vp, _sz, _vp]),
    "gcl_layernorm_bwd_cs": (C.c_int, [_vp, _i64, _vp, _i64, _vp, _vp, _vp, _i64, _vp, _vp, _vp, _i32, _i64, _i32, _vp, _sz, _vp]),
    "gcl_layernorm_bwd_map": (C.c_int, [_vp, _i64, _i64, _vp, _i32, _vp, _i64, _vp, _vp, _vp, _i64, _vp, _vp, _vp, _i32, _i64,
                                        _i32, _vp, _sz, _vp]),
    "gcl_layernorm_fwd_map_skip": (C.c_int, [_vp, _i64, _vp, _vp, _f32, _vp, _i64, _i64, _vp, _i32, _vp, _i32, _vp, _i64, _i32,
                                             _vp]),
    "gcl_layernorm_bwd_map_skip": (C.c_int, [_vp, _i64, _i64, _vp, _i32, _vp, _i64, _vp, _vp, _vp, _i64, _vp, _vp, _vp, _i32,
                                             _i64, _i32, _vp, _sz, _vp]),
    "gcl_layernorm_bwd_ws_bytes": (_sz, [_i64, _i32]),
    "gcl_graphnorm_fwd": (C.c_int, [_vp, _i64, _i64, _vp, _vp, _f32, _vp, _i64, _i64, _vp, _i32, _i32, _i32, _vp, _sz, _vp]),
    "gcl_graphnorm_bwd": (C.c_int, [_vp, _i64, _i64, _vp, _i64, _i64, _vp, _vp, _f32, _vp, _i64, _i64, _vp, _vp,
                                    _i32, _i32, _i32, _i32, _vp, _sz, _vp]),
    "gcl_graphnorm_ws_bytes": (_sz, [_i32, _i32, _i32]),
    "gcl_colsum": (C.c_int, [_vp, _i64, _i64, _i32, _vp, _i32, _vp, _sz, _vp]),
    "gcl_colsum_ws_bytes": (_sz, [_i64, _i32]),
    "gcl_colsum_split": (C.c_int, [_vp, _i64, _i64, _vp, _i64, _i64, _i32, _i32, _i32, _i32, _vp, _i32, _vp, _sz, _vp]),
    "gcl_assemble_input": (C.c_int, [_vp, _vp, _vp, _vp, _i64, _i32, _i32, _i32, _i32, _i32, _vp]),
    "gcl_assemble_input_tail": (C.c_int, [_vp, _vp, _vp, _vp, _i32, _vp, _i64, _i32, _i32, _i32, _i32, _i32, _vp]),
    "gcl_wmse_fwd_bwd": (C.c_int, [_vp, _i64, _i64, _vp, _i64, _i64, _vp, _i64, _i64, _vp, _vp, _f32, _f32, _vp,
                                   _vp, _vp, _vp, _i32, _i32, _i32, _vp, _sz, _vp]),
    "gcl_ar_step_bwd": (C.c_int, [_vp, _vp, _vp, _vp, _i32, _i32, _vp, _vp, _i32, _i32, _i32, _i32, _vp]),
    "gcl_pad_rows": (C.c_int, [_vp, _i64, _i64, _i32, _i32, _vp, _i64, _i64, _i32, _i32, _i32, _vp]),
    "gcl_zero": (C.c_int, [_vp, _sz, _vp]),
    "gcl_wmse_ws_bytes": (_sz, [_i32, _i32, _i32]),
    "gcl_adam_step": (C.c_int, [_vp, _vp, _vp, _vp, _i64, _f32, _f32, _f32, _f32, _f32, _i32, _f32, _vp]),
    "gcl_adam_step_dev": (C.c_int, [_vp, _vp, _vp, _vp, _i64, _f32, _f32, _f32, _f32, _f32, _vp, _vp, _f32, _vp]),
    "gcl_adam_step_groups": (C.c_int, [_vp, _vp, _vp, _vp, _i64, _vp, _i32, _vp, _vp, _vp, _vp, _f32, _f32, _f32, _f32,
                                       _f32, _vp]),
    "gcl_copy_rows": (C.c_int, [_vp, _i64, _i64, _vp, _i64, _i64, _i32, _i32, _i32, _vp]),
    "gcl_dense_fwd": (C.c_int, [_vp, _i64, _i32, _vp, _vp, _i64, _vp, _vp, _i64, _vp, _i64, _i64, _i32, _i32, _vp]),
    "gcl_dense_bwd_dx": (C.c_int, [_vp, _i64, _vp, _i64, _vp, _i64, _i32, _vp, _vp, _vp, _i64, _vp, _i64, _i64, _i32, _i32,
                                   _vp, C.c_size_t, _vp]),
    "gcl_dense_bwd_dw": (C.c_int, [_vp, _i64, _vp, _i64, _i32, _vp, _vp, _i64, _vp, _i64, _i32, _i32, _i32, _vp,
                                   C.c_size_t, _vp]),
    "gcl_gcn_layer_fwd": (C.c_int, [_vp, _vp, _i64, _i64, _i32, _vp, _vp, _vp, _vp, _i64, _i64, _i32, _i32, _i32, _i32, _vp]),
    "gcl_gcn_layer_fwd_rows": (C.c_int, [_vp, _vp, _i64, _i64, _i32, _vp, _vp, _vp, _vp, _i64, _i64, _i32, _i32, _i32, _i32, _i32, _vp]),
    "gcl_gcn_layer_fwd_split": (C.c_int, [_vp, _vp, _i64, _i64, _i32, _vp, _vp, _vp, _vp, _i64, _i64, _vp, _i64, _i64, _i32, _i32, _i32,
                                          _i32, _i32, _vp]),
    "gcl_gcn_layer_fwd_split_ok": (C.c_int, [_vp, _i64, _i64, _i64, _i64, _i64, _i64, _i32, _i32, _i32, _i32, _i32]),
    "gcl_gcn_layer_fwd_present": (C.c_int, [_vp, _vp, _i64, _i64, _i32, _vp, _vp, _vp, _vp, _i64, _i64, _vp, _i32, _i32, _i32, _i32,
                                            _vp]),
    "gcl_layernorm_fwd_map": (C.c_int, [_vp, _i64, _vp, _vp, _f32, _vp, _i64, _i64, _vp, _i32, _vp, _i64, _i32, _vp]),
    "gcl_gcn_layer_fwd_tab": (C.c_int, [_vp, _vp, _i64, _i64, _i64, _vp, _i32, _vp, _vp, _vp, _vp, _i64, _i64, _i32, _i32, _i32, _i32, _vp]),
    "gcl_gcn_layer_fwd_tab_ok": (C.c_int, [_vp, _i64, _i64, _i64, _i32, _i32, _i32]),
    "gcl_segment_reduce": (C.c_int, [_vp, _i64, _i64, _vp, _vp, _i32, _vp, _i64, _i64, _i32, _i32, _i32, _vp]),
    "gcl_edge_combine": (C.c_int, [_vp, _vp, _vp, _i64, _i64, _vp, _vp, _vp, _i64, _i64, _vp, _vp, _i32, _i64, _i32, _vp]),
    "gcl_act_fwd": (C.c_int, [_vp, _vp, _i64, _i32, _vp, _vp]),
    "gcl_act_bwd": (C.c_int, [_vp, _vp, _vp, _i64, _i32, _vp, _vp, _vp, C.c_size_t, _vp]),
    "gcl_act_bwd_ws_bytes": (C.c_size_t, []),
    "gcl_window_pack": (C.c_int, [_vp, _i64, _i32, _i32, _i32, _vp, _vp, _vp, _i32, _i32, _i32, _vp, _vp, _i32, _vp]),
    "gcl_ar_advance": (C.c_int, [_vp, _vp, _i64, _i64, _vp, _i64, _i64, _vp, _vp, _vp, _i64, _i64, _i32, _i32, _i32, _i32,
                                 _i32, _i32, _vp]),
    "gcl_gather2_rows": (C.c_int, [_vp, _i64, _i64, _vp, _vp, _i64, _i64, _vp, _vp, _i64, _i64, _i32, _i32, _i32, _i32, _vp]),
    "gcl_roi_gather_rows": (C.c_int, [_vp, _i32, _i32] + [_vp, _i64, _i64, _i32] * 3 + [_vp, _i64, _i64, _i32, _i32, _vp]),
    "gcl_roi_compose": (C.c_int, [_vp, _i64, _i64, _vp, _i64, _i64, _vp, _vp, _i64, _i64, _i32, _i32, _i32, _vp]),
    "gcl_segment_wsum": (C.c_int, [_vp, _i64, _i64, _i32, _i32, _vp, _vp, _vp, _vp, _i64, _i64, _vp, _i64, _i64, _i32,
                                   _i32, _i32, _i32, _vp]),
    "gcl_cross_update_fwd": (C.c_int, [_vp, _i64, _i64, _vp, _i64, _i64, _vp, _vp, _vp, _f32, _vp, _vp, _vp, _i32, _i32,
                                       _i32, _vp]),
    "gcl_nudge": (C.c_int, [_vp, _i64, _i64, _vp, _i64, _i64, _vp, _f32, _f32, _i32, _vp, _i64, _i64, _i32, _i32, _i32,
                            _vp]),
    "gcl_nudge_rows": (C.c_int, [_vp, _i64, _i64, _vp, _i64, _i64, _vp, _i32, _vp, _vp, _vp, _vp, _i64, _i64, _i32, _i32,
                                 _i32, _vp]),
    "gcl_oi_max_stations": (C.c_int, []),
    "gcl_oi_station_cov": (C.c_int, [_vp, _vp, _i32, C.c_double, C.c_double, C.c_double, _vp, _vp]),
    "gcl_oi_factor": (C.c_int, [_vp, _i32, _vp]),
    "gcl_oi_solve": (C.c_int, [_vp, _i32, _vp, _vp, _vp, _i32, _vp]),
    "gcl_oi_innovation": (C.c_int, [_vp, _i64, _i64, _vp, _i64, _i64, _vp, _vp, _vp, _i32, _i32, _i32, _vp, _vp]),
    "gcl_oi_analysis": (C.c_int, [_vp, _i64, _i64, _vp, _i64, _i64, _vp, _i32, _vp, _vp, _vp, _vp, _i32, _vp, _vp, _vp,
                                  _vp, _i32, _f32, _f32, _f32, _f32, _i32, _vp]),
    "gcl_oi_analysis_rows": (C.c_int, [_vp, _i64, _i64, _vp, _i64, _i64, _vp, _i32, _vp, _vp, _vp, _vp, _i32, _vp, _vp,
                                       _vp, _vp, _i32, _vp, _vp, _f32, _f32, _i32, _vp]),
    "gcl_verify_colstats_ws_bytes": (_sz, [_i32, _i32, _i32, _i32]),
    "gcl_verify_colstats": (C.c_int, [_vp, _i64, _i64, _i32, _i32] + [_vp, _i64, _i64, _vp] * 4
# ... 449 lines not shown


def aggregate_present(graph: Graph, h3, present, bias=None, transpose=False, out=None):
    B, n, F = h3.shape
    assert n == graph.n, f"graph has {graph.n} nodes, features have {n} rows"
    assert h3.stride(2) == 1 and present.dtype == torch.int32 and present.numel() == n and present.is_contiguous()
    if out is None:
        out = torch.empty(B, n, F, dtype=torch.float32, device=h3.device)
    tok = _probe_begin("aggregate_present", graph=graph, transpose=bool(transpose), B=B, F=F)
    _check(lib().gcl_aggregate_present(graph.handle, _agg_flags(transpose), _p(h3), h3.stride(1), h3.stride(0),
                                       _pi(present), _p(bias), _p(out), out.stride(1), out.stride(0), B, F, _stream()))
    _probe_end(tok)
    return out


def aggregate_compact_ok(graph: Graph, h3, transpose=False) -> bool:
    B, n, F = h3.shape
    return bool(lib().gcl_aggregate_compact_ok(graph.handle, 1 if transpose else 0, h3.stride(1), h3.stride(0), F, n * F, B, F))


def aggregate_compact(graph: Graph, h3, smap, outc, transpose=False, out=None):
    B, n, F = h3.shape
    assert n == graph.n and h3.stride(2) == 1 and outc.stride(2) == 1 and outc.shape[0] == B and outc.shape[2] == F
    assert smap.dtype == torch.int32 and smap.numel() == n and smap.is_contiguous()
    if out is None:
        out = torch.empty(B, n, F, dtype=torch.float32, device=h3.device)
    tok = _probe_begin("aggregate_compact", graph=graph, transpose=bool(transpose), B=B, F=F)
    _check(lib().gcl_aggregate_compact(graph.handle, 1 if transpose else 0, _p(h3), h3.stride(1), h3.stride(0), _pi(smap),
                                       _p(out), out.stride(1), out.stride(0), _p(outc), outc.stride(1), outc.stride(0), B, F,
                                       _stream()))
    _probe_end(tok)
    return out


def aggregate_heavy_launches() -> int:
    return int(lib().gcl_aggregate_heavy_launches())


def aggregate_split(graph: Graph, a3, b3, transpose=False, out=None):
    B, head, F = a3.shape
    n = head + b3.shape[1]
    assert n == graph.n, f"graph has {graph.n} nodes, the two parts have {n} rows"
    assert b3.shape[0] == B and b3.shape[2] == F and a3.stride(2) == 1 and b3.stride(2) == 1
    if out is None:
        out = torch.empty(B, n, F, dtype=torch.float32, device=a3.device)
    tok = _probe_begin("aggregate_split", graph=graph, transpose=bool(transpose), B=B, F=F)
    _check(lib().gcl_aggregate_split(graph.handle, _agg_flags(transpose), _p(a3), a3.stride(1), a3.stride(0), _p(b3),
                                     b3.stride(1), b3.stride(0), head, None, _p(out), out.stride(1), out.stride(0), B, F,
                                     _stream()))
    _probe_end(tok)
    return out


def layernorm_fwd(x, gamma, beta, eps=1e-5):
    rows, F = x.shape
    y = torch.empty(rows, F, dtype=torch.float32, device=x.device)
    stats = torch.empty(rows, 2, dtype=torch.float32, device=x.device)
    _check(lib().gcl_layernorm_fwd(_p(x), _ld(x), _p(gamma), _p(beta), float(eps), _p(y), F, _p(stats), rows, F, _stream()))
    return y, stats


def layernorm_fwd_map(x, gamma, beta, eps, out3, pos):
    rows, F = x.shape
    n_per = pos.numel()
    assert out3.stride(2) == 1 and rows % n_per == 0 and out3.shape[0] == rows // n_per
    stats = torch.empty(rows, 2, dtype=torch.float32, device=x.device)
    _check(lib().gcl_layernorm_fwd_map(_p(x), _ld(x), _p(gamma), _p(beta), float(eps), _p(out3), out3.stride(1), out3.stride(0),
                                       _pi(pos), n_per, _p(stats), rows, F, _stream()))
    return stats


def layernorm_fwd_map_skip(x, gamma, beta, eps, out3, pos, rlist):
    rows, F = x.shape
    n_per = pos.numel()
    assert out3.stride(2) == 1 and rows % n_per == 0 and out3.shape[0] == rows // n_per and rlist.stride(0) == 1
    stats = torch.empty(rows, 2, dtype=torch.float32, device=x.device)
    _check(lib().gcl_layernorm_fwd_map_skip(_p(x), _ld(x), _p(gamma), _p(beta), float(eps), _p(out3), out3.stride(1),
                                            out3.stride(0), _pi(pos), n_per, _pi(rlist), rlist.numel(), _p(stats), rows, F,
                                            _stream()))
    return stats


def layernorm_bwd(dy, x, gamma, stats, dgamma, dbeta, accumulate: bool, colsum_dx=None, acc_colsum: bool = False,
                  dy_map=None, skip: bool = False):
    rows, F = x.shape
    dx = torch.empty(rows, F, dtype=torch.float32, device=x.device)
    nb = lib().gcl_layernorm_bwd_ws_bytes(rows, F)
    acc = (ACC_DW if accumulate else 0) | (ACC_COLSUM if acc_colsum else 0)
    if dy_map is not None:
        src3, pos = dy_map
        assert src3.stride(2) == 1 and src3.shape[2] >= F and rows % pos.numel() == 0 and src3.shape[0] == rows // pos.numel()
    else:
        assert not skip, "skip needs the mapped gradient"
    if _deferred.active:
        if dy_map is not None:
            a = (_p(src3), src3.stride(1), src3.stride(0), _pi(pos), pos.numel(), 1 if skip else 0)
        else:
            a = (_p(dy), _ld(dy), 0, None, 0, 0)
        _queue(nb, x.device, (dgamma, dbeta, colsum_dx), 1, lambda ws, jobs: lib().gcl_layernorm_bwd_deferred(
            *a, _p(x), _ld(x), _p(gamma), _p(stats), _p(dx), F, _p(dgamma), _p(dbeta), _p(colsum_dx), acc, rows, F,
            ws.data_ptr(), ws.numel(), _stream(), C.cast(jobs, C.c_void_p)))
        return dx
    ws = workspace(nb, x.device)
    if dy_map is not None:
        fn = lib().gcl_layernorm_bwd_map_skip if skip else lib().gcl_layernorm_bwd_map
        _check(fn(_p(src3), src3.stride(1), src3.stride(0), _pi(pos), pos.numel(), _p(x), _ld(x),
# ... 86 lines not shown
    if tab is not None:
        n = graph.n
    dy3 = dy3.contiguous()
    dh = torch.empty(B, n, HC, dtype=torch.float32, device=h3.device)
    nb = lib().gcl_gat_bwd_ws_bytes(graph.e, n, B, H, Cc)
    ws = workspace(nb, h3.device)
    tok = _probe_begin("gat_bwd", graph=graph, B=B, H=H, C=Cc)
    if tab is not None:
        _check(lib().gcl_gat_bwd_tab(graph.handle, _p(dy3), Cc, n * Cc, _p(h3), h3.stride(1), h3.stride(0), _pi(tab), _p(att_src),
                                     _p(att_dst), _p(a_s), _p(a_d), _p(alpha), _p(dh), HC, n * HC, _p(d_att_src),
                                     _p(d_att_dst), _p(d_bias), 1 if accumulate else 0, B, H, Cc, ws.data_ptr(), ws.numel(),
                                     _stream()))
    else:
        _check(lib().gcl_gat_bwd(graph.handle, _p(dy3), Cc, n * Cc, _p(h3), h3.stride(1), h3.stride(0), _p(att_src),
                                 _p(att_dst), _p(a_s), _p(a_d), _p(alpha), _p(dh), HC, n * HC, _p(d_att_src), _p(d_att_dst),
                                 _p(d_bias), 1 if accumulate else 0, B, H, Cc, ws.data_ptr(), ws.numel(), _stream()))
    _probe_end(tok)
    return dh


def gat_alpha_edge_order(graph: Graph, alpha_slots_1sample, H):
    out = torch.empty(graph.e, H, dtype=torch.float32, device=alpha_slots_1sample.device)
    _check(lib().gcl_gat_alpha_to_edge_order(graph.handle, _p(alpha_slots_1sample.contiguous()), _p(out), H, _stream()))
    return out


def gat_prune(graph: Graph, alpha_edges, threshold: float) -> torch.Tensor:
    buf = torch.empty(2 * graph.e, dtype=torch.int64)
    kept = _i64(0)
    nb = lib().gcl_gat_prune_ws_bytes(graph.e)
    ws = workspace(nb, alpha_edges.device)
    _check(lib().gcl_gat_prune(graph.handle, _p(alpha_edges.contiguous()), float(threshold), buf.data_ptr(),
                               C.byref(kept), ws.data_ptr(), ws.numel(), _stream()))
    k = kept.value
    return buf[: 2 * k].view(2, k).clone()


def assemble_input(x3, grid_static, mesh_static, tail3=None):
    B, G, Cdyn = x3.shape
    M, Cs = mesh_static.shape
    x3 = x3.contiguous()
    out = torch.empty(B, G + M, Cdyn + Cs, dtype=torch.float32, device=x3.device)
    if tail3 is not None and tail3.is_contiguous() and tail3.shape[2] == Cdyn + Cs:
        _check(lib().gcl_assemble_input_tail(_p(x3), _p(grid_static), _p(mesh_static), _p(tail3), tail3.shape[1], _p(out),
                                             Cdyn + Cs, B, G, M, Cdyn, Cs, _stream()))
        return out
    _check(lib().gcl_assemble_input(_p(x3), _p(grid_static), _p(mesh_static), _p(out), Cdyn + Cs, B, G, M, Cdyn, Cs, _stream()))
    if tail3 is not None:
        copy_rows(tail3, out[:, G + M - tail3.shape[1]:, :])
    return out


def wmse_fwd_bwd(delta3, x_last3, y3, node_w, chan_w, inv_wsum, grad_scale, want_grad=True, want_state=False,
                 loss_prev=None):
    B, G, Cc = delta3.shape
    dev = delta3.device
    if delta3.stride(2) != 1:
        delta3 = delta3.contiguous()
    dd = torch.empty(B, G, Cc, dtype=torch.float32, device=dev) if want_grad else None
    st = torch.empty(B, G, Cc, dtype=torch.float32, device=dev) if want_state else None
    loss = torch.empty((), dtype=torch.float32, device=dev)
    nb = lib().gcl_wmse_ws_bytes(B, G, Cc)
    ws = workspace(nb, dev)
    xl = x_last3
    _check(lib().gcl_wmse_fwd_bwd(
        _p(delta3), delta3.stride(1), delta3.stride(0), _p(xl), xl.stride(1) if xl is not None else 0, xl.stride(0) if xl is not None else 0,
        _p(y3), y3.stride(1), y3.stride(0), _p(node_w), _p(chan_w), float(inv_wsum), float(grad_scale), _p(dd), _p(st),
        _p(loss_prev), _p(loss), B, G, Cc, ws.data_ptr(), ws.numel(), _stream()))
    return loss, dd, st


def adam_step(p, g, m, v, lr, beta1, beta2, eps, weight_decay, step, grad_scale=1.0):
    _check(lib().gcl_adam_step(_p(p), _p(g), _p(m), _p(v), p.numel(), lr, beta1, beta2, eps, weight_decay, int(step),
                               float(grad_scale), _stream()))


def adam_step_dev(p, g, m, v, lr, beta1, beta2, eps, weight_decay, step_dev, bc_dev, grad_scale=1.0):
    assert step_dev.dtype == torch.int32 and step_dev.is_cuda
    _check(lib().gcl_adam_step_dev(_p(p), _p(g), _p(m), _p(v), p.numel(), lr, beta1, beta2, eps, weight_decay,
                                   step_dev.data_ptr(), _p(bc_dev), float(grad_scale), _stream()))


def adam_step_groups(p, g, m, v, chunk_param, active, lr, step, bc, beta1, beta2, eps, weight_decay, grad_scale=1.0):
    P = step.numel()
    assert p.is_cuda and p.numel() % 64 == 0 and chunk_param.numel() == p.numel() // 64
    assert step.dtype == active.dtype == chunk_param.dtype == torch.int32 and lr.dtype == bc.dtype == torch.float32
    assert active.numel() == lr.numel() == P and bc.numel() == 2 * P
    _check(lib().gcl_adam_step_groups(_p(p), _p(g), _p(m), _p(v), p.numel(), _pi(chunk_param), P, _pi(active),
                                      _p(lr), _pi(step), _p(bc), beta1, beta2, eps, weight_decay, float(grad_scale),
                                      _stream()))


def copy_rows(src3, dst3):
    B, rows, F = src3.shape
    _check(lib().gcl_copy_rows(_p(src3), src3.stride(1), src3.stride(0), _p(dst3), dst3.stride(1), dst3.stride(0), B, rows, F, _stream()))
    return dst3


def _pi(t):
    if t is None:
        return None
    assert t.is_cuda and t.dtype == torch.int32 and t.is_contiguous()
    return t.data_ptr()


def gather2_rows(a3, map_a, b3, map_b, nd: int, B: int, sum_batch: bool = False, out=None, deal: int = 0):
    F = a3.shape[-1]
    if sum_batch and deal > 1:
        assert out is not None and nd % deal == 0 and out.shape == (nd // deal, deal, F) and out.stride(2) == 1
        flag = deal
    else:
        if out is None:
            out = torch.empty(1 if sum_batch else B, nd, F, dtype=torch.float32, device=a3.device)
        assert out.shape == (1 if sum_batch else B, nd, F) and out.stride(2) == 1
        flag = 1 if sum_batch else 0
    bsa = a3.stride(0) if (a3.shape[0] > 1 or sum_batch) else 0
    bsb = 0 if b3 is None else (b3.stride(0) if b3.shape[0] > 1 else 0)
    _check(lib().gcl_gather2_rows(_p(a3), a3.stride(1), bsa, _pi(map_a), _p(b3), 0 if b3 is None else b3.stride(1),
                                  bsb, _pi(map_b), _p(out), out.stride(1), out.stride(0), B, nd, F, flag, _stream()))
    return out

# ... 20 lines not shown
    B, G, Cc = pred3.shape
    assert corr3.dim() == 3 and corr3.shape[0] == B and corr3.shape[2] >= Cc and pos.numel() == G
    assert pred3.stride(2) == 1 and corr3.stride(2) == 1
    if out is None:
        out = torch.empty(B, G, Cc, dtype=torch.float32, device=pred3.device)
    _check(lib().gcl_roi_compose(_p(pred3), pred3.stride(1), pred3.stride(0), _p(corr3), corr3.stride(1), corr3.stride(0),
                                 _pi(pos), _p(out), out.stride(1), out.stride(0), B, G, Cc, _stream()))
    return out


def segment_wsum(src3, idx, w, rowptr, out3=None, addend3=None, act=ACT_NONE, accumulate: bool = False):
    n = rowptr.numel() - 1
    if out3 is None:
        B = src3.shape[0] if addend3 is None else addend3.shape[0]
        D = src3.shape[2] if addend3 is None else addend3.shape[2]
        out3 = torch.empty(B, n, D, dtype=torch.float32, device=src3.device)
    B, _, D = out3.shape
    assert out3.shape[1] == n and src3.stride(2) == 1 and out3.stride(2) == 1 and src3.shape[2] >= D
    assert src3.shape[0] in (1, B) and (addend3 is None or (addend3.shape == out3.shape and addend3.stride(2) == 1))
    assert w is None or (w.is_cuda and w.dtype == torch.float32 and w.is_contiguous())
    _check(lib().gcl_segment_wsum(_p(src3), src3.stride(1), src3.stride(0) if src3.shape[0] > 1 else 0, src3.shape[1],
                                  int(act), _pi(idx), w.data_ptr() if w is not None else None, _pi(rowptr), _p(addend3),
                                  addend3.stride(1) if addend3 is not None else 0,
                                  addend3.stride(0) if addend3 is not None else 0, _p(out3), out3.stride(1),
                                  out3.stride(0), 1 if accumulate else 0, B, n, D, _stream()))
    return out3


def cross_update_fwd(h3, msg3, rowptr, gamma, beta, eps=1e-5):
    B, n, D = h3.shape
    assert h3.stride(2) == 1 and msg3.stride(2) == 1 and msg3.shape[0] == B and msg3.shape[2] == D
    assert rowptr.numel() == n + 1
    pre = torch.empty(B, n, D, dtype=torch.float32, device=h3.device)
    y = torch.empty(B, n, D, dtype=torch.float32, device=h3.device)
    stats = torch.empty(B * n, 2, dtype=torch.float32, device=h3.device)
    _check(lib().gcl_cross_update_fwd(_p(h3), h3.stride(1), h3.stride(0), _p(msg3), msg3.stride(1), msg3.stride(0),
                                      _pi(rowptr), _p(gamma), _p(beta), float(eps), _p(pre), _p(y), _p(stats), B, n, D,
                                      _stream()))
    return pre, y, stats


def ar_advance(state4, delta3, y_step3, chan_kind, out3, out_off: int, residual: bool):
    B, G, obs, Cc = state4.shape
    assert state4.is_contiguous() and delta3.stride(2) == 1
    new_state = torch.empty_like(state4)
    _check(lib().gcl_ar_advance(
        _p(state4), _p(delta3), delta3.stride(1), delta3.stride(0), _p(y_step3), y_step3.stride(1) if y_step3 is not None else 0,
        y_step3.stride(0) if y_step3 is not None else 0, _pi(chan_kind), _p(new_state), _p(out3),
        out3.stride(1) if out3 is not None else 0, out3.stride(0) if out3 is not None else 0, int(out_off), B, G, obs, Cc,
        1 if residual else 0, _stream()))
    return new_state


def ar_step_bwd(dd3, g_loss, g_new4, chan_kind, has_y: bool, residual: bool, obs: int, want_state: bool):
    B, G, Cc = dd3.shape
    d_delta = torch.empty_like(dd3)
    d_state = torch.empty(B, G, obs, Cc, dtype=torch.float32, device=dd3.device) if want_state else None
    if g_new4 is not None and not g_new4.is_contiguous():
        g_new4 = g_new4.contiguous()
    _check(lib().gcl_ar_step_bwd(_p(dd3), _p(g_loss), _p(g_new4), _pi(chan_kind), 1 if has_y else 0, 1 if residual else 0,
                                 _p(d_delta), _p(d_state), B, G, obs, Cc, _stream()))
    return d_delta, d_state


def pad_rows(src3, rows_dst: int, F_dst: int):
    B, r, F = src3.shape
    assert src3.stride(2) == 1
    dst = torch.empty(B, rows_dst, F_dst, dtype=torch.float32, device=src3.device)
    _check(lib().gcl_pad_rows(_p(src3), src3.stride(1), src3.stride(0), r, F, _p(dst), F_dst, rows_dst * F_dst, rows_dst, F_dst,
                              B, _stream()))
    return dst


def zero_(t: torch.Tensor):
    assert t.is_contiguous() and t.is_cuda
    _check(lib().gcl_zero(t.data_ptr(), t.numel() * t.element_size(), _stream()))
    return t


def segment_reduce(src3, perm, rowptr, mean: bool, out3=None):
    B, _, D = src3.shape
    n = rowptr.numel() - 1
    if out3 is None:
        out3 = torch.empty(B, n, D, dtype=torch.float32, device=src3.device)
    assert src3.stride(2) == 1 and out3.stride(2) == 1 and tuple(out3.shape) == (B, n, D)
    _check(lib().gcl_segment_reduce(_p(src3), src3.stride(1), src3.stride(0), _pi(perm), _pi(rowptr), 1 if mean else 0,
                                    _p(out3), out3.stride(1), out3.stride(0), B, n, D, _stream()))
    return out3


def edge_combine(base3, extra3, A3, ia, sa, C3, ic, out3=None):
    ref = base3 if base3 is not None else extra3
    if ref is not None:
        B, E, D = ref.shape
    else:
        B, E, D = (A3 if A3 is not None else C3).shape[0], ia.numel() if ia is not None else ic.numel(), \
            (A3 if A3 is not None else C3).shape[2]
    for t in (base3, extra3):
        assert t is None or t.is_contiguous()
    if out3 is None:
        out3 = torch.empty(B, E, D, dtype=torch.float32, device=(A3 if ref is None else ref).device)
    _check(lib().gcl_edge_combine(
        _p(base3), _p(extra3), _p(A3), A3.stride(1) if A3 is not None else 0, A3.stride(0) if A3 is not None else 0,
        _pi(ia), _p(sa), _p(C3), C3.stride(1) if C3 is not None else 0, C3.stride(0) if C3 is not None else 0, _pi(ic),
        _p(out3), B, E, D, _stream()))
    return out3


def act_fwd(x, act, slope=None):
    y = torch.empty_like(x)
    assert x.is_contiguous()
    _check(lib().gcl_act_fwd(_p(x), _p(y), x.numel(), int(act), _p(slope), _stream()))
# ... 962 lines not shown
```

### graphcast-lite_amd/train.py

```python
import os

import torch
import torch.distributed as dist

from . import hip
from .capture import Captured, graph_enabled
from .functional import ARStepLossFn, WeightedMSEFn


class FileNames:

    EXPERIMENT_CONFIG = "config.json"
    TRAIN_X = "X_train.pt"
    TRAIN_Y = "y_train.pt"
    TEST_X = "X_test.pt"
    TEST_Y = "y_test.pt"
    SAVED_MODEL = "best_model.pth"
    SAVED_RESULTS = "results.json"
    CHECKPOINT = "checkpoint.pth"


def save_checkpoint(path, model, optimiser, epoch, ar_steps, best_val_loss, patience_counter, train_losses,
                    val_losses):
    torch.save({
        "epoch": epoch,
        "ar_steps": ar_steps,
        "best_val_loss": best_val_loss,
        "patience_counter": patience_counter,
        "train_losses": train_losses,
        "val_losses": val_losses,
        "model_state_dict": model.state_dict(),
        "optimizer_state_dict": optimiser.state_dict(),
    }, path)


def load_checkpoint(path, model, optimiser, device):
    ckpt = torch.load(path, map_location=device, weights_only=True)
    model.load_state_dict(ckpt["model_state_dict"])
    optimiser.load_state_dict(ckpt["optimizer_state_dict"])
    return {
        "start_epoch": ckpt["epoch"] + 1,
        "ar_steps": ckpt["ar_steps"],
        "best_val_loss": ckpt["best_val_loss"],
        "patience_counter": ckpt["patience_counter"],
        "train_losses": ckpt["train_losses"],
        "val_losses": ckpt["val_losses"],
    }


def get_lat_weights(lat_dim, lon_dim, device, flat_lats=None):
    if flat_lats is not None:
        w = torch.cos(torch.deg2rad(torch.from_numpy(flat_lats.copy()).float()))
        w = w / w.mean()
        return w.view(1, -1, 1).to(device)
    w = torch.cos(torch.deg2rad(torch.linspace(-90, 90, lat_dim)))
    w = w / w.mean()
    return w.view(1, -1).expand(lon_dim, lat_dim).reshape(-1).view(1, -1, 1).to(device)


def build_boundary_mask(n_lon, n_lat, width, device):
# ... 471 lines not shown
        self.lat_weights, self.channel_mask, self.spatial_mask = lat_weights, channel_mask, spatial_mask
        self._ar_steps, self.world = ar_steps, world_size
        self.use_residual = use_residual
        self.static_channels, self.forcing_channels = static_channels, forcing_channels
        super().__init__(graph_enabled(use_graph), required=use_graph is True)
        self._sparse = bool(getattr(model, "using_sparse_gat", False))
        self.split_finish = (world_size > 1) if split_finish is None else bool(split_finish or world_size > 1)
        if world_size > 1:
            if not (dist.is_available() and dist.is_initialized()):
                raise RuntimeError(f"TrainStep(world_size={world_size}) needs an initialised torch.distributed process group")
            if dist.get_world_size() != world_size:
                raise RuntimeError(f"TrainStep(world_size={world_size}) but the process group has {dist.get_world_size()} ranks")
            self.sync_from_rank0()

    @property
    def ar_steps(self) -> int:
        return self._ar_steps

    @ar_steps.setter
    def ar_steps(self, value):
        if int(value) != self._ar_steps:
            self._ar_steps = int(value)
            self.reset_graph()

    def sync_from_rank0(self):
        for t in (self.flat.flat, self.opt.m, self.opt.v, self.opt.step_dev):
            dist.broadcast(t, src=0)

    @property
    def launch_mode(self) -> str:
        if self.graph_active and self.split_finish:
            return "hipGraph replay (fwd+bwd; all-reduce + Adam eager)"
        return super().launch_mode

    def _fwd_bwd(self, X, y, threshold=0.0, epoch=0, batch_num=1):
        self.flat.zero_grad()
        loss = batch_loss(self.model, X, y, threshold, epoch, batch_num, self.lat_weights, self.ar_steps,
                          self.channel_mask, self.spatial_mask, self.static_channels, self.forcing_channels,
                          self.use_residual)
        defer = _DEFER_REDUCTIONS and loss.is_cuda
        if defer:
            hip.defer_begin()
        try:
            loss.backward(self._loss_root(loss))
        except BaseException:
            if defer:
                hip.defer_flush(drop=True)
            raise
        if defer:
            hip.defer_flush()
        return loss.detach()

    def _loss_root(self, loss):
        one = getattr(self, "_one", None)
        if one is not None and one.device == loss.device and one.dtype == loss.dtype and loss.dim() == 0:
            return one
        if loss.dim() != 0 or not loss.is_cuda or torch.cuda.is_current_stream_capturing():
            return None
        with torch.inference_mode(False):
            self._one = torch.ones((), dtype=loss.dtype, device=loss.device)
        return self._one

    def _finish(self):
        scale = allreduce_gradients(self.flat, self.world)
        self.opt.step(grad_scale=scale)

    def _eager(self, X, y, threshold=0.0, epoch=0, batch_num=1):
        loss = self._fwd_bwd(X, y, threshold, epoch, batch_num)
        self._finish()
        return loss

    def _work(self, X, y, threshold=0.0, epoch=0, batch_num=1):
        if self.split_finish:
            return self._fwd_bwd(X, y, threshold, epoch, batch_num)
        return self._eager(X, y, threshold, epoch, batch_num)

    def __call__(self, X, y, threshold=0.0, epoch=0, batch_num=1):
        if self.opt.sync():
            self.reset_graph()
        if self._sparse and batch_num == 0:
            self.reset_graph()
            return self._eager(X, y, threshold, epoch, batch_num)
        loss = self._run(X, y, threshold=threshold, epoch=epoch, batch_num=batch_num)
        if self.split_finish:
            self._finish()
        return loss.detach()

    def input_buffers(self):
        return tuple(self._static) if self.graph_active else None


def build_optimizer(model, config, pretrained: bool):
    freeze_proc = getattr(config, "freeze_processor_epochs", 0)
    proc_lr_factor = getattr(config, "finetune_processor_lr_factor", 0.1)
    base_lr = config.learning_rate
    if pretrained and freeze_proc > 0:
        proc_params = list(model.processor.parameters())
        proc_ids = {id(p) for p in proc_params}
        other_params = [p for p in model.parameters() if id(p) not in proc_ids]
        for p in proc_params:
            p.requires_grad = False
        return torch.optim.Adam([{"params": other_params, "lr": base_lr},
                                 {"params": proc_params, "lr": base_lr * proc_lr_factor}])
    return torch.optim.Adam(params=model.parameters(), lr=base_lr)


def loss_masks(config, dataset_metadata, device):
    device = torch.device(device)
    lat_weights = None
    if getattr(config, "use_latitude_weighting", False) and dataset_metadata:
        if getattr(dataset_metadata, "flat_grid", False) and hasattr(dataset_metadata, "cordinates"):
            lat_weights = get_lat_weights(0, 0, device, flat_lats=dataset_metadata.cordinates[0])
        else:
            lat_weights = get_lat_weights(dataset_metadata.num_latitudes, dataset_metadata.num_longitudes, device)
# ... 156 lines not shown
```

### include/gcl.h

```cpp
#ifndef GCL_H
#define GCL_H

#include <stddef.h>
#include <stdint.h>

#ifdef __cplusplus
extern "C" {
#endif

#define GCL_VERSION 100

#define GCL_OK 0
#define GCL_EINVAL (-1)
#define GCL_EHIP (-2)
#define GCL_ENOMEM (-3)
#define GCL_EUNSUPPORTED (-4)

typedef struct gcl_graph gcl_graph_t;
typedef void* gcl_stream_t;

int gcl_version(void);
const char* gcl_last_error(void);

#define GCL_GRAPH_GCN 0
// ... 48 lines not shown
  float* sout;
  int32_t nparts, ns;
} gcl_reduce_job;
int gcl_linear_bwd_all_deferred(const float* dy, int64_t lddy, const float* W, const float* x, int64_t ldx,
                                const float* in_slope, float* d_in_slope, float* dx, int64_t lddx, float* dW,
                                float* db, float* colsum_dx, int64_t rows, int32_t Fin, int32_t Fout,
                                int32_t accumulate, void* ws, size_t ws_bytes, gcl_stream_t stream,
                                gcl_reduce_job* job);
int gcl_reduce_jobs(const gcl_reduce_job* jobs, int32_t n, gcl_stream_t stream);
int gcl_layernorm_bwd_deferred(const float* dy, int64_t lddy, int64_t bsdy, const int32_t* pos, int32_t n_per,
                               int32_t skip, const float* x, int64_t ldx, const float* gamma, const float* stats,
                               float* dx, int64_t lddx, float* dgamma, float* dbeta, float* colsum_dx,
                               int32_t accumulate, int64_t rows, int32_t F, void* ws, size_t ws_bytes,
                               gcl_stream_t stream, gcl_reduce_job* job);
int gcl_colsum_deferred(const float* x, int64_t ldx, int64_t rows, int32_t F, float* out, int32_t accumulate, void* ws,
                        size_t ws_bytes, gcl_stream_t stream, gcl_reduce_job* job);
int gcl_colsum_split_deferred(const float* a, int64_t lda, int64_t bsa, const float* b, int64_t ldb, int64_t bsb,
                              int32_t head, int32_t n, int32_t B, int32_t F, float* out, int32_t accumulate, void* ws,
                              size_t ws_bytes, gcl_stream_t stream, gcl_reduce_job* job);
int gcl_linear_bwd_dw_deferred(const float* dy, int64_t lddy, const float* x, int64_t ldx, const float* in_slope,
                               float* dW, float* db, int64_t rows, int32_t Fin, int32_t Fout, int32_t accumulate,
                               void* ws, size_t ws_bytes, gcl_stream_t stream, gcl_reduce_job* job );
int gcl_dense_bwd_dw_deferred(const float* dy, int64_t lddy, const float* x, int64_t ldx, int32_t act,
                              const float* slope, float* dW, int64_t lddw, float* db, int64_t rows, int32_t Fin,
                              int32_t Fout, int32_t accumulate, void* ws, size_t ws_bytes, gcl_stream_t stream,
                              gcl_reduce_job* job );

#define GCL_ACT_NONE 0
#define GCL_ACT_PRELU 1
#define GCL_ACT_SILU 2
int gcl_dense_fwd(const float* x, int64_t ldx, int32_t act, const float* slope, const float* W,
                  int64_t ldw, const float* bias, const float* addend, int64_t ldadd, float* y,
                  int64_t ldy, int64_t rows, int32_t Fin, int32_t Fout, gcl_stream_t stream);
int gcl_dense_bwd_dx(const float* dy, int64_t lddy, const float* W, int64_t ldw, const float* z,
                     int64_t ldz, int32_t act, const float* slope, float* d_slope,
                     const float* addend, int64_t ldadd, float* dx, int64_t lddx, int64_t rows,
                     int32_t Fin, int32_t Fout, void* ws, size_t ws_bytes, gcl_stream_t stream);
int gcl_dense_bwd_dw(const float* dy, int64_t lddy, const float* x, int64_t ldx, int32_t act,
                     const float* slope, float* dW, int64_t lddw, float* db, int64_t rows,
                     int32_t Fin, int32_t Fout, int32_t accumulate, void* ws, size_t ws_bytes,
                     gcl_stream_t stream);

int gcl_aggregate(const gcl_graph_t* g, int32_t transpose, const float* h, int64_t ldh, int64_t bsh,
                  const float* bias, float* y, int64_t ldy, int64_t bsy, int32_t B, int32_t F,
                  gcl_stream_t stream);
#define GCL_AGG_HEAVY_INSIDE 2
int64_t gcl_aggregate_heavy_launches(void);
int gcl_aggregate_present(const gcl_graph_t* g, int32_t transpose, const float* h, int64_t ldh, int64_t bsh,
                          const int32_t* present , const float* bias, float* y, int64_t ldy, int64_t bsy,
                          int32_t B, int32_t F, gcl_stream_t stream);
int gcl_aggregate_split(const gcl_graph_t* g, int32_t transpose, const float* h, int64_t ldh, int64_t bsh,
                        const float* h2, int64_t ldh2, int64_t bsh2, int32_t head, const float* bias, float* y,
                        int64_t ldy, int64_t bsy, int32_t B, int32_t F, gcl_stream_t stream);
int gcl_aggregate_compact_ok(const gcl_graph_t* g, int32_t transpose, int64_t ldh, int64_t bsh, int64_t ldy, int64_t bsy,
                             int32_t B, int32_t F);
int gcl_aggregate_compact(const gcl_graph_t* g, int32_t transpose, const float* h, int64_t ldh, int64_t bsh,
                          const int32_t* smap , float* y, int64_t ldy, int64_t bsy, float* yc, int64_t ldc,
                          int64_t bsc, int32_t B, int32_t F, gcl_stream_t stream);

int gcl_gat_fwd(const gcl_graph_t* g, const float* h, int64_t ldh, int64_t bsh,
                const float* att_src , const float* att_dst , const float* bias ,
                float* a_src , float* a_dst , float* alpha ,
                float* y, int64_t ldy, int64_t bsy, int32_t B, int32_t H, int32_t C,
                gcl_stream_t stream);
int gcl_gat_bwd(const gcl_graph_t* g, const float* dy, int64_t lddy, int64_t bsdy,
                const float* h, int64_t ldh, int64_t bsh, const float* att_src, const float* att_dst,
                const float* a_src, const float* a_dst, const float* alpha,
                float* dh, int64_t lddh, int64_t bsdh, float* d_att_src, float* d_att_dst,
                float* d_bias, int32_t accumulate, int32_t B, int32_t H, int32_t C,
                void* ws, size_t ws_bytes, gcl_stream_t stream);
size_t gcl_gat_bwd_ws_bytes(int64_t e_prime, int32_t n, int32_t B, int32_t H, int32_t C);
int gcl_gat_fwd_tab(const gcl_graph_t* g, const float* h, int64_t ldh, int64_t bsh, const int32_t* tab ,
                    const float* att_src, const float* att_dst, const float* bias, float* a_src, float* a_dst,
                    float* alpha, float* y, int64_t ldy, int64_t bsy, int32_t B, int32_t H, int32_t C,
                    gcl_stream_t stream);
int gcl_gat_bwd_tab(const gcl_graph_t* g, const float* dy, int64_t lddy, int64_t bsdy, const float* h, int64_t ldh,
                    int64_t bsh, const int32_t* tab , const float* att_src, const float* att_dst,
                    const float* a_src, const float* a_dst, const float* alpha, float* dh, int64_t lddh, int64_t bsdh,
                    float* d_att_src, float* d_att_dst, float* d_bias, int32_t accumulate, int32_t B, int32_t H,
                    int32_t C, void* ws, size_t ws_bytes, gcl_stream_t stream);
int gcl_gat_tab_ok(const gcl_graph_t* g, int64_t ldh, int32_t H, int32_t C);
int gcl_gat_alpha_to_edge_order(const gcl_graph_t* g, const float* alpha_slots, float* alpha_edges,
                                int32_t H, gcl_stream_t stream);
int gcl_gat_prune(const gcl_graph_t* g, const float* alpha_edges, float threshold,
                  int64_t* edge_index_out, int64_t* kept, void* ws, size_t ws_bytes,
                  gcl_stream_t stream);
size_t gcl_gat_prune_ws_bytes(int64_t e_prime);

int gcl_layernorm_fwd(const float* x, int64_t ldx, const float* gamma, const float* beta, float eps,
                      float* y, int64_t ldy, float* stats, int64_t rows, int32_t F,
                      gcl_stream_t stream);
int gcl_layernorm_fwd_map(const float* x, int64_t ldx, const float* gamma, const float* beta, float eps, float* y,
                          int64_t ldy, int64_t bsy, const int32_t* pos , int32_t n_per, float* stats,
                          int64_t rows, int32_t F, gcl_stream_t stream);
int gcl_layernorm_bwd(const float* dy, int64_t lddy, const float* x, int64_t ldx, const float* gamma,
                      const float* stats, float* dx, int64_t lddx, float* dgamma, float* dbeta,
                      int32_t accumulate, int64_t rows, int32_t F, void* ws, size_t ws_bytes,
                      gcl_stream_t stream);
int gcl_layernorm_bwd_cs(const float* dy, int64_t lddy, const float* x, int64_t ldx, const float* gamma,
                         const float* stats, float* dx, int64_t lddx, float* dgamma, float* dbeta,
                         float* colsum_dx, int32_t accumulate, int64_t rows, int32_t F, void* ws,
                         size_t ws_bytes, gcl_stream_t stream);
int gcl_layernorm_bwd_map(const float* dy, int64_t lddy, int64_t bsdy, const int32_t* pos, int32_t n_per,
                          const float* x, int64_t ldx, const float* gamma, const float* stats, float* dx,
                          int64_t lddx, float* dgamma, float* dbeta, float* colsum_dx, int32_t accumulate,
                          int64_t rows, int32_t F, void* ws, size_t ws_bytes, gcl_stream_t stream);
int gcl_layernorm_fwd_map_skip(const float* x, int64_t ldx, const float* gamma, const float* beta, float eps, float* y,
                               int64_t ldy, int64_t bsy, const int32_t* pos , int32_t n_per,
                               const int32_t* rlist , int32_t n_list, float* stats, int64_t rows, int32_t F,
                               gcl_stream_t stream);
int gcl_layernorm_bwd_map_skip(const float* dy, int64_t lddy, int64_t bsdy, const int32_t* pos, int32_t n_per,
                               const float* x, int64_t ldx, const float* gamma, const float* stats, float* dx,
                               int64_t lddx, float* dgamma, float* dbeta, float* colsum_dx, int32_t accumulate,
                               int64_t rows, int32_t F, void* ws, size_t ws_bytes, gcl_stream_t stream);
size_t gcl_layernorm_bwd_ws_bytes(int64_t rows, int32_t F);
int gcl_graphnorm_fwd(const float* x, int64_t ldx, int64_t bsx, const float* gamma, const float* beta,
                      float eps, float* y, int64_t ldy, int64_t bsy, float* stats, int32_t B,
                      int32_t n, int32_t F, void* ws, size_t ws_bytes, gcl_stream_t stream);
int gcl_graphnorm_bwd(const float* dy, int64_t lddy, int64_t bsdy, const float* x, int64_t ldx,
                      int64_t bsx, const float* gamma, const float* stats, float eps, float* dx,
                      int64_t lddx, int64_t bsdx, float* dgamma, float* dbeta, int32_t accumulate,
                      int32_t B, int32_t n, int32_t F, void* ws, size_t ws_bytes, gcl_stream_t stream);
size_t gcl_graphnorm_ws_bytes(int32_t B, int32_t n, int32_t F);

int gcl_colsum(const float* x, int64_t ldx, int64_t rows, int32_t F, float* out, int32_t accumulate,
               void* ws, size_t ws_bytes, gcl_stream_t stream);
size_t gcl_colsum_ws_bytes(int64_t rows, int32_t F);
int gcl_colsum_split(const float* a, int64_t lda, int64_t bsa, const float* b, int64_t ldb, int64_t bsb, int32_t head,
                     int32_t n, int32_t B, int32_t F, float* out, int32_t accumulate, void* ws, size_t ws_bytes,
                     gcl_stream_t stream);

int gcl_assemble_input(const float* x , const float* grid_static ,
                       const float* mesh_static , float* out, int64_t ldo, int32_t B,
                       int32_t G, int32_t M, int32_t Cdyn, int32_t Cs, gcl_stream_t stream);
int gcl_assemble_input_tail(const float* x, const float* grid_static, const float* mesh_static, const float* tail,
                            int32_t r, float* out, int64_t ldo, int32_t B, int32_t G, int32_t M, int32_t Cdyn,
                            int32_t Cs, gcl_stream_t stream);

int gcl_wmse_fwd_bwd(const float* delta, int64_t ldd, int64_t bsd, const float* x_last, int64_t ldx,
                     int64_t bsx, const float* y, int64_t ldy_, int64_t bsy, const float* node_w,
                     const float* chan_w, float inv_wsum, float grad_scale, float* d_delta,
                     float* out_state, const float* loss_prev, float* loss_out, int32_t B, int32_t G,
                     int32_t C, void* ws, size_t ws_bytes, gcl_stream_t stream);
size_t gcl_wmse_ws_bytes(int32_t B, int32_t G, int32_t C);

int gcl_adam_step(float* p, const float* g, float* m, float* v, int64_t count, float lr, float beta1,
                  float beta2, float eps, float weight_decay, int32_t step, float grad_scale,
                  gcl_stream_t stream);

int gcl_adam_step_dev(float* p, const float* g, float* m, float* v, int64_t count, float lr, float beta1,
                      float beta2, float eps, float weight_decay, int32_t* step_dev, float* bc_dev,
                      float grad_scale, gcl_stream_t stream);

int gcl_adam_step_groups(float* p, const float* g, float* m, float* v, int64_t count, const int32_t* chunk_param,
                         int32_t num_params, const int32_t* active, const float* lr, int32_t* step, float* bc,
                         float beta1, float beta2, float eps, float weight_decay, float grad_scale,
                         gcl_stream_t stream);

int gcl_copy_rows(const float* src, int64_t lds, int64_t bss, float* dst, int64_t ldd, int64_t bsd,
                  int32_t B, int32_t rows, int32_t F, gcl_stream_t stream);

int gcl_gcn_layer_fwd(const gcl_graph_t* g, const float* x, int64_t ldx, int64_t bsx, int32_t act,
                      const float* slope, const float* W , const float* bias, float* y,
                      int64_t ldy, int64_t bsy, int32_t B, int32_t Fin, int32_t Fout, int32_t Fout_store,
                      gcl_stream_t stream);
int gcl_gcn_layer_fwd_rows(const gcl_graph_t* g, const float* x, int64_t ldx, int64_t bsx, int32_t act,
                           const float* slope, const float* W , const float* bias, float* y,
                           int64_t ldy, int64_t bsy, int32_t B, int32_t Fin, int32_t Fout, int32_t Fout_store,
                           int32_t rows_out, gcl_stream_t stream);
int gcl_gcn_layer_fwd_split(const gcl_graph_t* g, const float* x, int64_t ldx, int64_t bsx, int32_t act,
                            const float* slope, const float* W , const float* bias, float* ya, int64_t lda,
                            int64_t bsa, float* yb, int64_t ldb, int64_t bsb, int32_t head, int32_t B, int32_t Fin,
                            int32_t Fout, int32_t Fout_store, gcl_stream_t stream);
int gcl_gcn_layer_fwd_split_ok(const gcl_graph_t* g, int64_t ldx, int64_t bsx, int64_t lda, int64_t bsa, int64_t ldb,
                               int64_t bsb, int32_t head, int32_t B, int32_t Fin, int32_t Fout, int32_t Fout_store);
int gcl_gcn_layer_fwd_present(const gcl_graph_t* g, const float* x, int64_t ldx, int64_t bsx, int32_t act,
                              const float* slope, const float* W, const float* bias, float* y, int64_t ldy, int64_t bsy,
                              const int32_t* present , int32_t B, int32_t Fin, int32_t Fout, int32_t Fout_store,
                              gcl_stream_t stream);
int gcl_gcn_layer_fwd_tab(const gcl_graph_t* g, const float* x, int64_t ldx, int64_t bsx, int64_t x_rows,
                          const int32_t* tab , int32_t act, const float* slope, const float* W ,
                          const float* bias, float* y, int64_t ldy, int64_t bsy, int32_t B, int32_t Fin, int32_t Fout,
                          int32_t Fout_store, gcl_stream_t stream);
int gcl_gcn_layer_fwd_tab_ok(const gcl_graph_t* g, int64_t ldx, int64_t bsx, int64_t x_rows, int32_t B, int32_t Fin,
                             int32_t Fout);

int gcl_segment_reduce(const float* src, int64_t ld_src, int64_t bs_src, const int32_t* perm,
                       const int32_t* rowptr , int32_t mean, float* out, int64_t ld_out,
                       int64_t bs_out, int32_t B, int32_t n, int32_t D, gcl_stream_t stream);
int gcl_edge_combine(const float* base, const float* extra, const float* A, int64_t lda, int64_t bsa,
                     const int32_t* ia, const float* sa, const float* C, int64_t ldc, int64_t bsc,
                     const int32_t* ic, float* out, int32_t B, int64_t E, int32_t D,
                     gcl_stream_t stream);
int gcl_act_fwd(const float* x, float* y, int64_t count, int32_t act, const float* slope,
                gcl_stream_t stream);
int gcl_act_bwd(const float* x, const float* dy, float* dx, int64_t count, int32_t act,
                const float* slope, float* d_slope, void* ws, size_t ws_bytes, gcl_stream_t stream);
size_t gcl_act_bwd_ws_bytes(void);

int gcl_window_pack(const uint16_t* series , int64_t T, int32_t n_lon, int32_t n_lat,
                    int32_t Ct, const int64_t* t0, const float* mean, const float* stdv, int32_t C,
                    int32_t obs, int32_t pred, float* X , float* Y ,
                    int32_t B, gcl_stream_t stream);

int gcl_ar_advance(const float* state, const float* delta, int64_t ldd, int64_t bsd, const float* y_step,
                   int64_t ldy, int64_t bsy, const int32_t* chan_kind, float* new_state, float* out,
                   int64_t ldo, int64_t bso, int32_t out_off, int32_t B, int32_t G, int32_t obs, int32_t C,
                   int32_t residual, gcl_stream_t stream);
int gcl_ar_step_bwd(const float* dd, const float* g_loss, const float* g_new, const int32_t* chan_kind,
                    int32_t has_y, int32_t residual, float* d_delta, float* d_state, int32_t B, int32_t G,
                    int32_t obs, int32_t C, gcl_stream_t stream);

int gcl_pad_rows(const float* src, int64_t lds, int64_t bss, int32_t rows_src, int32_t F_src, float* dst,
                 int64_t ldd, int64_t bsd, int32_t rows_dst, int32_t F_dst, int32_t B, gcl_stream_t stream);
int gcl_zero(void* ptr, size_t nbytes, gcl_stream_t stream);

int gcl_gather2_rows(const float* a, int64_t lda, int64_t bsa, const int32_t* map_a, const float* b,
                     int64_t ldb, int64_t bsb, const int32_t* map_b, float* dst, int64_t ldd, int64_t bsd,
                     int32_t B, int32_t nd, int32_t F, int32_t sum_batch, gcl_stream_t stream);

int gcl_roi_gather_rows(const int32_t* rows, int32_t n, int32_t rows_src, const float* s0, int64_t ld0,
                        int64_t bs0, int32_t w0, const float* s1, int64_t ld1, int64_t bs1, int32_t w1,
                        const float* s2, int64_t ld2, int64_t bs2, int32_t w2, float* dst, int64_t ldd,
                        int64_t bsd, int32_t Fp, int32_t B, gcl_stream_t stream);
int gcl_roi_compose(const float* pred, int64_t ldp, int64_t bsp, const float* corr, int64_t ldc, int64_t bsc,
                    const int32_t* pos, float* out, int64_t ldo, int64_t bso, int32_t B, int32_t G, int32_t C,
                    gcl_stream_t stream);

int gcl_segment_wsum(const float* src, int64_t ld_src, int64_t bs_src, int32_t n_src, int32_t act,
                     const int32_t* idx, const float* w, const int32_t* rowptr, const float* addend,
                     int64_t ld_add, int64_t bs_add, float* out, int64_t ld_out, int64_t bs_out,
                     int32_t accumulate, int32_t B, int32_t n, int32_t D, gcl_stream_t stream);
int gcl_cross_update_fwd(const float* h, int64_t ld_h, int64_t bs_h, const float* msg, int64_t ld_msg,
                         int64_t bs_msg, const int32_t* rowptr, const float* gamma, const float* beta,
                         float eps, float* pre, float* y, float* stats, int32_t B, int32_t n, int32_t D,
                         gcl_stream_t stream);

int gcl_nudge(const float* f, int64_t ldf, int64_t bsf, const float* obs, int64_t ldo, int64_t bso,
              const uint8_t* chan_mask, float c0, float c1, int32_t form, float* out, int64_t ldt,
              int64_t bst, int32_t B, int32_t G, int32_t C, gcl_stream_t stream);
int gcl_nudge_rows(const float* f, int64_t ldf, int64_t bsf, const float* obs, int64_t ldo, int64_t bso,
                   const uint8_t* station_mask, int32_t n_net, const int32_t* net_of_row, const float* alpha,
                   const uint8_t* chan_mask, float* out, int64_t ldt, int64_t bst, int32_t B, int32_t G,
                   int32_t C, gcl_stream_t stream);
int gcl_oi_max_stations(void);
int gcl_oi_station_cov(const double* lat, const double* lon, int32_t m, double sb2, double rl2,
                       double diag, double* S, gcl_stream_t stream);
int gcl_oi_factor(double* M, int32_t m, gcl_stream_t stream);
int gcl_oi_solve(const double* M, int32_t m, const double* rhs, double* tmp, float* W, int32_t n,
                 gcl_stream_t stream);
int gcl_oi_innovation(const float* obs, int64_t ldo, int64_t bso, const float* xb, int64_t ldx,
                      int64_t bsx, const int32_t* obs_row, const int32_t* node_row, const int32_t* chans,
                      int32_t m, int32_t nch, int32_t B, double* rhs, gcl_stream_t stream);
int gcl_oi_analysis(const float* xb, int64_t ldx, int64_t bsx, float* xa, int64_t lda, int64_t bsa,
                    const int32_t* chans, int32_t nch, const int32_t* node_row, const double* nlat,
                    const double* nlon, const float* ncos, int32_t n_nodes, const double* slat,
                    const double* slon, const float* scos, const float* W, int32_t m, float sb2, float rl2,
                    float th_cut, float a_cut, int32_t B, gcl_stream_t stream);
int gcl_oi_analysis_rows(const float* xb, int64_t ldx, int64_t bsx, float* xa, int64_t lda, int64_t bsa,
                         const int32_t* chans, int32_t nch, const int32_t* node_row, const double* nlat,
                         const double* nlon, const float* ncos, int32_t n_nodes, const double* slat,
                         const double* slon, const float* scos, const float* W, int32_t m,
                         const float* sb2_row, const float* rl2_row, float th_cut, float a_cut, int32_t B,
                         gcl_stream_t stream);
// ... 184 lines not shown
```

Measured before the change: 27220.

## Add head-only aggregation, lean x3 backward variants, and padded-stride loss gradients

Adds a head-only aggregation entry point that treats rows past a head index as zeros, so a padded or concatenated source no longer has to be materialised before aggregating. Specialises the x3 linear backward kernel at compile time on activation, bias-grad, column-sum and masking flags, dropping unused reductions and the extra barrier when those outputs are not requested. The weighted-MSE and AR-step backward kernels gain variants that write gradients straight into a padded leading dimension, which is meant to avoid later pad/copy kernels. The loss-root constant is now taken from a shared helper; more template instances mean larger binaries, and the new paths only pay off where callers use them.

```diff
diff --git a/graphcast-lite_amd/csrc/aggregate.hip b/graphcast-lite_amd/csrc/aggregate.hip
--- a/graphcast-lite_amd/csrc/aggregate.hip
+++ b/graphcast-lite_amd/csrc/aggregate.hip
@@ -7,6 +7,8 @@
 #include "mfma_io.h"
 
 namespace {
+
+__device__ __attribute__((aligned(16))) float agg_zero_row[256];
 
 template <int LPR, bool VL, bool VS, bool PRES, bool SPLIT>
 __device__ __forceinline__ void agg_heavy_row(const int row, const int b, const int32_t* __restrict__ rowptr,
@@ -22,7 +24,7 @@
   const bool cactive = c0 < F;
   const int cc = cactive ? c0 : 0;
   const float* __restrict__ Hb = H + (int64_t)b * bsh;
-  const float* __restrict__ H2b = SPLIT ? H2 + (int64_t)b * bsh2 : nullptr;
+  const float* __restrict__ H2b = SPLIT ? (H2 ? H2 + (int64_t)b * bsh2 : agg_zero_row) : nullptr;
   const int start = rowptr[row], end = rowptr[row + 1];
   float a0 = 0.f, a1 = 0.f, a2 = 0.f, a3 = 0.f;
   auto ld4 = [&](int j, float& x0, float& x1, float& x2, float& x3) {
@@ -142,7 +144,7 @@
   const bool cactive = c0 < F;
   const int cc = cactive ? c0 : 0;
   const float* __restrict__ Hb = H + (int64_t)b * bsh;
-  const float* __restrict__ H2b = SPLIT ? H2 + (int64_t)b * bsh2 : nullptr;
+  const float* __restrict__ H2b = SPLIT ? (H2 ? H2 + (int64_t)b * bsh2 : agg_zero_row) : nullptr;
   float* __restrict__ Yb = Y + (int64_t)b * bsy;
 
   float bz0 = 0.f, bz1 = 0.f, bz2 = 0.f, bz3 = 0.f;
@@ -499,6 +501,8 @@
   const float* h2 = nullptr;
   int64_t ldh2 = 0, bsh2 = 0;
   int32_t head = 0;
+  bool zero_tail = false;
+  bool two_part() const { return h2 != nullptr || zero_tail; }
   const int32_t* smap = nullptr;
   float* yc = nullptr;
   int64_t ldc = 0, bsc = 0;
@@ -572,7 +576,7 @@
                      const int32_t* present = nullptr) {
   g_heavy_launches.fetch_add(1, std::memory_order_relaxed);
   dim3 hgrid((unsigned)ga.n_heavy, (unsigned)B), block(256);
-  if (ga.h2) {
+  if (ga.two_part()) {
     hipLaunchKernelGGL((agg_heavy_kernel<LPR, true, true, false, true>), hgrid, block, 0, st, ga.heavy, ga.rowptr, ga.col,
                        ga.w, h, ldh, bsh, bias, y, ldy, bsy, F, (const int32_t*)nullptr, ga.h2, ga.ldh2, ga.bsh2, ga.head);
     GCL_CHECK_LAUNCH();
@@ -611,7 +615,7 @@
   const bool vl = (ldh % 4 == 0) && (bsh % 4 == 0) && gcl::aligned16(h) && ldh >= ((F + 3) / 4) * 4;
   const bool vs = (ldy % 4 == 0) && (bsy % 4 == 0) && gcl::aligned16(y) && (F % 4 == 0);
   if constexpr (LPR >= 16) {
-    if (!ga.h2 && vl && vs && (!bias || gcl::aligned16(bias))) {
+    if (!ga.two_part() && vl && vs && (!bias || gcl::aligned16(bias))) {
       const int hr = launch_agg_halo<LPR>(ga, h, ldh, bsh, bias, y, ldy, bsy, n, B, F, st, present);
       if (hr >= 0) {
         if (hr != GCL_OK || ga.n_heavy == 0 || ga.dry) return hr;
@@ -626,7 +630,7 @@
   int ewidth = ew_env > 0 ? ew_env : ga.ell_width;
   if (ewidth > EL) ewidth = EL;
   ewidth = ewidth >= 8 ? 8 : ewidth >= 4 ? 4 : ewidth >= 2 ? 2 : 1;
-  const int iter = (!present && !ga.h2 && (iter_env == 1 || iter_env == 2 || iter_env == 4 || iter_env == 8)) ? iter_env
+  const int iter = (!present && !ga.two_part() && (iter_env == 1 || iter_env == 2 || iter_env == 4 || iter_env == 8)) ? iter_env
                                                                                                      : (ewidth >= 4 ? 1 : 2);
   int32_t nRB = (int32_t)gcl::cdiv(n, RPW * 4 * iter);
   if (ga.order16 && RPW * 4 * iter <= 16) nRB = ga.n_order16 * (16 / (RPW * 4 * iter));
@@ -662,7 +666,7 @@
   hipLaunchKernelGGL((agg_kernel<LPR, true, true, EW_, IT_, false, true>), grid, block, 0, st, ga.rowptr, ga.col, ga.w,  \
                      ga.ecol, ga.ew, h, ldh, bsh, bias, y, ldy, bsy, n, B, F, nRB, xcd_map, nt, order16,                \
                      (const int32_t*)nullptr, ga.h2, ga.ldh2, ga.bsh2, ga.head)
-  if (ga.h2) {
+  if (ga.two_part()) {
     if (hv) {
       if constexpr (EL >= 8) {
         if (ewidth == 8) GCL_AGGHS(8, 1);
@@ -812,6 +816,19 @@
   return aggregate_impl(g, transpose, h, ldh, bsh, nullptr, bias, y, ldy, bsy, B, F, stream, h2, ldh2, bsh2, head);
 }
 
+extern "C" int gcl_aggregate_head(const gcl_graph_t* g, int32_t transpose, const float* h, int64_t ldh, int64_t bsh,
+                                  int32_t head, const float* bias, float* y, int64_t ldy, int64_t bsy, int32_t B, int32_t F,
+                                  gcl_stream_t stream) {
+  GCL_CHECK_ARG(g && h && y, "aggregate_head: null argument");
+  GCL_CHECK_ARG(head > 0 && head <= g->n, "aggregate_head: head=%d outside (0, n=%d]", head, g->n);
+  GCL_CHECK_ARG(F > 0 && F % 4 == 0 && ldh >= F && ldh % 4 == 0 && bsh % 4 == 0 && ldy % 4 == 0 && bsy % 4 == 0 &&
+                    gcl::aligned16(h) && gcl::aligned16(y),
+                "aggregate_head: the source and y need 16-byte rows (F %% 4 == 0, aligned bases and strides)");
+  AggArgs za;
+  za.zero_tail = true;
+  return aggregate_impl(g, transpose, h, ldh, bsh, nullptr, bias, y, ldy, bsy, B, F, stream, nullptr, 0, 0, head, &za);
+}
+
 extern "C" int gcl_aggregate_compact_ok(const gcl_graph_t* g, int32_t transpose, int64_t ldh, int64_t bsh, int64_t ldy,
                                         int64_t bsy, int32_t B, int32_t F) {
   if (!g || g->kind == GCL_GRAPH_GAT || B <= 0 || F <= 32 || F > 256 || F % 4 != 0 || ldh < F || ldy < F) return 0;
diff --git a/graphcast-lite_amd/csrc/linear_x3.hip b/graphcast-lite_amd/csrc/linear_x3.hip
--- a/graphcast-lite_amd/csrc/linear_x3.hip
+++ b/graphcast-lite_amd/csrc/linear_x3.hip
@@ -227,8 +227,8 @@
   return __builtin_shufflevector(a, b, 0, 1, 2, 3, 4, 5, 6, 7);
 }
 
-template <int NO>
-__global__ __launch_bounds__(256, 2) void linear_x3_bwd_kernel(
+template <int NO, bool ACT, bool DB, bool CS, bool YMASK>
+__device__ __forceinline__ void linear_x3_bwd_body(
     const float* __restrict__ dY, int64_t lddy, const float* __restrict__ W, const float* __restrict__ P,
     int64_t ldp, const float* __restrict__ in_slope, float* __restrict__ dX, int64_t lddx, int64_t rows, int32_t Fin,
     int32_t Fout, float* __restrict__ part_dw, float* __restrict__ part_db, float* __restrict__ part_cs,
@@ -273,7 +273,7 @@
     __syncthreads();
   }
 
-  const bool act = in_slope != nullptr;
+  const bool act = ACT && in_slope != nullptr;
   const float slope = act ? *in_slope : 1.f;
   const int64_t ntiles = (rows + 63) / 64;
 
@@ -324,13 +324,15 @@
 #pragma unroll
     for (int it = 0; it < 4; ++it) {
       float4 y = pre_y[it];
-      y.x = __uint_as_float(__float_as_uint(y.x) & ym0); y.y = __uint_as_float(__float_as_uint(y.y) & ym1);
-      y.z = __uint_as_float(__float_as_uint(y.z) & ym2); y.w = __uint_as_float(__float_as_uint(y.w) & ym3);
-      db4.x += y.x; db4.y += y.y; db4.z += y.z; db4.w += y.w;
+      if (YMASK) {
+        y.x = __uint_as_float(__float_as_uint(y.x) & ym0); y.y = __uint_as_float(__float_as_uint(y.y) & ym1);
+        y.z = __uint_as_float(__float_as_uint(y.z) & ym2); y.w = __uint_as_float(__float_as_uint(y.w) & ym3);
+      }
+      if (DB) { db4.x += y.x; db4.y += y.y; db4.z += y.z; db4.w += y.w; }
       const float4 z = pre_p[it];
-      cur_p[it] = z;
-      float4 a;
-      {
+      float4 a = z;
+      if (ACT) {
+        cur_p[it] = z;
         const float mx = z.x * slope, my = z.y * slope, mz = z.z * slope, mw = z.w * slope;
         a.x = z.x > 0.f ? z.x : mx; a.y = z.y > 0.f ? z.y : my; a.z = z.z > 0.f ? z.z : mz; a.w = z.w > 0.f ? z.w : mw;
       }
@@ -402,11 +404,13 @@
       for (int it = 0; it < 4; ++it) {
         const int row = wave * 16 + it * 4 + rsub;
         float4 v = *reinterpret_cast<const float4*>(Stg + row * 64 + csub * 4);
-        const float4 z = cur_p[it];
-        const bool nx = act && z.x <= 0.f, ny = act && z.y <= 0.f, nz = act && z.z <= 0.f, nw = act && z.w <= 0.f;
-        slope_acc += (double)(((nx ? v.x * z.x : 0.f) + (ny ? v.y * z.y : 0.f)) + ((nz ? v.z * z.z : 0.f) + (nw ? v.w * z.w : 0.f)));
-        v.x = nx ? v.x * slope : v.x; v.y = ny ? v.y * slope : v.y; v.z = nz ? v.z * slope : v.z; v.w = nw ? v.w * slope : v.w;
-        cs4.x += v.x; cs4.y += v.y; cs4.z += v.z; cs4.w += v.w;
+        if (ACT) {
+          const float4 z = cur_p[it];
+          const bool nx = act && z.x <= 0.f, ny = act && z.y <= 0.f, nz = act && z.z <= 0.f, nw = act && z.w <= 0.f;
+          slope_acc += (double)(((nx ? v.x * z.x : 0.f) + (ny ? v.y * z.y : 0.f)) + ((nz ? v.z * z.z : 0.f) + (nw ? v.w * z.w : 0.f)));
+          v.x = nx ? v.x * slope : v.x; v.y = ny ? v.y * slope : v.y; v.z = nz ? v.z * slope : v.z; v.w = nw ? v.w * slope : v.w;
+        }
+        if (CS) { cs4.x += v.x; cs4.y += v.y; cs4.z += v.z; cs4.w += v.w; }
         buf_st4<GCL_X3_ST_AUX>(rx, pok ? (unsigned)((row * lddx + csub * 4) * 4) : kOOB, v);
       }
     }
@@ -423,29 +427,54 @@
 #pragma unroll
     for (int r = 0; r < 16; ++r) out[(size_t)(so * 32 + d_row(r, lane)) * FiP + sc * 32 + li] = dw_hi[r] + dw_lo[r];
   }
+  if (!(ACT || DB || CS)) return;
   __syncthreads();
   float* red = reinterpret_cast<float*>(smem8);
   {
     float* rdb = red + (wave * 4 + rsub) * 64 + csub * 4;
-    *reinterpret_cast<float4*>(rdb) = db4;
-    *reinterpret_cast<float4*>(rdb + 16 * 64) = cs4;
-  }
-  for (int off = 32; off > 0; off >>= 1) slope_acc += __shfl_down(slope_acc, off, 64);
+    if (DB) *reinterpret_cast<float4*>(rdb) = db4;
+    if (CS) *reinterpret_cast<float4*>(rdb + 16 * 64) = cs4;
+  }
   double* dred = reinterpret_cast<double*>(red + 2 * 16 * 64);
-  if (lane == 0) dred[wave] = slope_acc;
+  if (ACT) {
+    for (int off = 32; off > 0; off >>= 1) slope_acc += __shfl_down(slope_acc, off, 64);
+    if (lane == 0) dred[wave] = slope_acc;
+  }
   __syncthreads();
   if (tid < 128) {
     const int which = tid >> 6, c = tid & 63;
-    float s = 0.f;
-#pragma unroll
-    for (int q = 0; q < 16; ++q) s += red[(which * 16 + q) * 64 + c];
-    if (which == 0) {
-      if (part_db && c < FoP) part_db[(size_t)blockIdx.x * REC + c] = s;
-    } else {
-      if (part_cs) part_cs[(size_t)blockIdx.x * REC + c] = s;
-    }
-  }
-  if (part_slope && tid == 0) part_slope[blockIdx.x] = (dred[0] + dred[1]) + (dred[2] + dred[3]);
+    if (which == 0 ? DB : CS) {
+      float s = 0.f;
+#pragma unroll
+      for (int q = 0; q < 16; ++q) s += red[(which * 16 + q) * 64 + c];
+      if (which == 0) {
+        if (part_db && c < FoP) part_db[(size_t)blockIdx.x * REC + c] = s;
+      } else {
+        if (part_cs) part_cs[(size_t)blockIdx.x * REC + c] = s;
+      }
+    }
+  }
+  if (ACT && part_slope && tid == 0) part_slope[blockIdx.x] = (dred[0] + dred[1]) + (dred[2] + dred[3]);
+}
+
+template <int NO>
+__global__ __launch_bounds__(256, 2) void linear_x3_bwd_kernel(
+    const float* __restrict__ dY, int64_t lddy, const float* __restrict__ W, const float* __restrict__ P,
+    int64_t ldp, const float* __restrict__ in_slope, float* __restrict__ dX, int64_t lddx, int64_t rows, int32_t Fin,
+    int32_t Fout, float* __restrict__ part_dw, float* __restrict__ part_db, float* __restrict__ part_cs,
+    double* __restrict__ part_slope) {
+  linear_x3_bwd_body<NO, true, true, true, true>(dY, lddy, W, P, ldp, in_slope, dX, lddx, rows, Fin, Fout, part_dw, part_db,
+                                                 part_cs, part_slope);
+}
+
+template <int NO, bool ACT, bool DB, bool CS, bool YMASK>
+__global__ __launch_bounds__(256, 2) void linear_x3_bwd_lean_kernel(
+    const float* __restrict__ dY, int64_t lddy, const float* __restrict__ W, const float* __restrict__ P,
+    int64_t ldp, const float* __restrict__ in_slope, float* __restrict__ dX, int64_t lddx, int64_t rows, int32_t Fin,
+    int32_t Fout, float* __restrict__ part_dw, float* __restrict__ part_db, float* __restrict__ part_cs,
+    double* __restrict__ part_slope) {
+  linear_x3_bwd_body<NO, ACT, DB, CS, YMASK>(dY, lddy, W, P, ldp, in_slope, dX, lddx, rows, Fin, Fout, part_dw, part_db,
+                                             part_cs, part_slope);
 }
 
 int x3_ablate() {
@@ -522,16 +551,45 @@
                   float* part_cs, double* part_slope, hipStream_t st) {
   const int grid = x3_linear_bwd_blocks(rows);
   const size_t lds = 6 * (size_t)kImg64B + 64 * 64 * sizeof(float);
-#define GCL_X3B(NO_)                                                                                              \
+#define GCL_X3B_GO(KERN_)                                                                                         \
   do {                                                                                                            \
-    auto kern = linear_x3_bwd_kernel<NO_>;                                                                        \
+    auto kern = KERN_;                                                                                            \
     GCL_ENSURE_DYN_LDS(kern, gcl::kLdsBytes);                                                                     \
     hipLaunchKernelGGL(kern, dim3(grid), dim3(256), lds, st, dy, lddy, W, x, ldx, in_slope, dx, lddx, rows, Fin, Fout, \
                        part_dw, part_db, part_cs, part_slope);                                                    \
   } while (0)
-  if (Fout > 32) GCL_X3B(2);
-  else GCL_X3B(1);
+#define GCL_X3B(NO_) GCL_X3B_GO((linear_x3_bwd_kernel<NO_>))
+  const bool act = in_slope != nullptr, wdb = part_db != nullptr, wcs = part_cs != nullptr, ymask = (Fout & 3) != 0;
+  if ((wdb && wcs) || !env_int("GCL_X3_BWD_LEAN", 1)) {
+    if (Fout > 32) GCL_X3B(2);
+    else GCL_X3B(1);
+  } else {
+#define GCL_X3L(NO_, A_, D_, C_, M_) GCL_X3B_GO((linear_x3_bwd_lean_kernel<NO_, A_, D_, C_, M_>))
+#define GCL_X3L_M(NO_, A_, D_, C_)          \
+  do {                                      \
+    if (ymask) GCL_X3L(NO_, A_, D_, C_, true); \
+    else GCL_X3L(NO_, A_, D_, C_, false);   \
+  } while (0)
+#define GCL_X3L_A(NO_, A_)                          \
+  do {                                              \
+    if (wdb) GCL_X3L_M(NO_, A_, true, false);       \
+    else if (wcs) GCL_X3L_M(NO_, A_, false, true);  \
+    else GCL_X3L_M(NO_, A_, false, false);          \
+  } while (0)
+#define GCL_X3L_NO(NO_)           \
+  do {                            \
+    if (act) GCL_X3L_A(NO_, true); \
+    else GCL_X3L_A(NO_, false);   \
+  } while (0)
+    if (Fout > 32) GCL_X3L_NO(2);
+    else GCL_X3L_NO(1);
+#undef GCL_X3L_NO
+#undef GCL_X3L_A
+#undef GCL_X3L_M
+#undef GCL_X3L
+  }
 #undef GCL_X3B
+#undef GCL_X3B_GO
   GCL_CHECK_LAUNCH();
   return GCL_OK;
 }
diff --git a/graphcast-lite_amd/csrc/misc.hip b/graphcast-lite_amd/csrc/misc.hip
--- a/graphcast-lite_amd/csrc/misc.hip
+++ b/graphcast-lite_amd/csrc/misc.hip
@@ -72,13 +72,14 @@
   }
 }
 
+template <bool OUTLD>
 __global__ __launch_bounds__(256) void wmse_kernel(const float* __restrict__ delta, int64_t ldd, int64_t bsd,
                                                    const float* __restrict__ xl, int64_t ldx, int64_t bsx,
                                                    const float* __restrict__ y, int64_t ldy, int64_t bsy,
                                                    const float* __restrict__ node_w, const float* __restrict__ chan_w,
                                                    float inv_wsum, float grad_scale, float* __restrict__ dd,
                                                    float* __restrict__ out_state, float* __restrict__ part,
-                                                   int32_t B, int32_t G, int32_t C) {
+                                                   int32_t B, int32_t G, int32_t C, int64_t ldo, int64_t bso) {
   __shared__ float red[4];
   const int64_t total = (int64_t)B * G * C;
   float acc = 0.f;
@@ -95,7 +96,16 @@
     if (node_w) w *= node_w[g];
     const float d = o - t;
     acc += (d * d) * w;
-    if (dd) dd[idx] = 2.f * w * d * inv_wsum * grad_scale;
+    if (OUTLD) {
+      if (dd) {
+        float* row = dd + b * bso + (int64_t)g * ldo;
+        row[c] = 2.f * w * d * inv_wsum * grad_scale;
+        if (c == C - 1)
+          for (int q = C; q < ldo; ++q) row[q] = 0.f;
+      }
+    } else {
+      if (dd) dd[idx] = 2.f * w * d * inv_wsum * grad_scale;
+    }
     if (out_state) out_state[idx] = o;
   }
   for (int off = 32; off > 0; off >>= 1) acc += __shfl_down(acc, off, 64);
@@ -329,6 +339,39 @@
   }
 }
 
+template <bool STATE>
+__global__ __launch_bounds__(256) void ar_step_bwd_ld_kernel(const float* __restrict__ dd, int64_t ldd, int64_t bsd,
+                                                             const float* __restrict__ g_loss,
+                                                             const float* __restrict__ g_new,
+                                                             const int32_t* __restrict__ chan_kind, int32_t has_y,
+                                                             int32_t residual, float* __restrict__ d_delta, int64_t ldo,
+                                                             int64_t bso, float* __restrict__ d_state, int32_t B,
+                                                             int32_t G, int32_t obs, int32_t C) {
+  const float gl = g_loss ? *g_loss : 1.f;
+  const int64_t total = (int64_t)B * G * (STATE ? obs : 1) * C;
+  const int64_t stride = (int64_t)gridDim.x * 256;
+  int64_t idx = (int64_t)blockIdx.x * 256 + threadIdx.x;
+  for (Walk3 w(idx, stride, STATE ? obs : G, C); idx < total; idx += stride, w.next()) {
+    const int c = w.c, k = STATE ? w.i : obs - 1;
+    const int64_t bb = STATE ? (int64_t)((uint64_t)w.b / (uint32_t)G) : w.b;
+    const int64_t gg = STATE ? w.b - bb * G : (int64_t)w.i;
+    const int64_t sidx = STATE ? idx : ((bb * G + gg) * obs + (obs - 1)) * C + c;
+    float ds = (STATE && g_new && k >= 1) ? g_new[sidx - C] : 0.f;
+    if (k == obs - 1) {
+      int kind = chan_kind ? chan_kind[c] : 0;
+      if (kind == 2 && !has_y) kind = 0;
+      const float gd = gl * dd[bb * bsd + gg * ldd + c];
+      const float gn = g_new ? g_new[sidx] : 0.f;
+      float* row = d_delta + bb * bso + gg * ldo;
+      row[c] = gd + (kind == 0 ? gn : 0.f);
+      if (c == C - 1)
+        for (int q = C; q < ldo; ++q) row[q] = 0.f;
+      ds += (residual ? gd : 0.f) + ((kind == 1 || (kind == 0 && residual)) ? gn : 0.f);
+    }
+    if (STATE) d_state[sidx] = ds;
+  }
+}
+
 __global__ __launch_bounds__(256) void pad_rows_kernel(const float* __restrict__ src, int64_t lds, int64_t bss,
                                                        int32_t rows_src, int32_t F_src, float* __restrict__ dst,
                                                        int64_t ldd, int64_t bsd, int32_t rows_dst, int32_t F_dst,
@@ -376,23 +419,47 @@
   return (size_t)kLossBlocks * sizeof(float);
 }
 
-extern "C" int gcl_wmse_fwd_bwd(const float* delta, int64_t ldd, int64_t bsd, const float* x_last, int64_t ldx,
-                                int64_t bsx, const float* y, int64_t ldy, int64_t bsy, const float* node_w,
-                                const float* chan_w, float inv_wsum, float grad_scale, float* d_delta,
-                                float* out_state, const float* loss_prev, float* loss_out, int32_t B, int32_t G,
-                                int32_t C, void* ws, size_t ws_bytes, gcl_stream_t stream) {
+static int wmse_impl(const float* delta, int64_t ldd, int64_t bsd, const float* x_last, int64_t ldx, int64_t bsx,
+                     const float* y, int64_t ldy, int64_t bsy, const float* node_w, const float* chan_w, float inv_wsum,
+                     float grad_scale, float* d_delta, bool outld, int64_t ldd_out, int64_t bsd_out, float* out_state,
+                     const float* loss_prev, float* loss_out, int32_t B, int32_t G, int32_t C, void* ws, size_t ws_bytes,
+                     gcl_stream_t stream) {
   GCL_CHECK_ARG(delta && y && loss_out, "wmse: null argument");
   GCL_CHECK_ARG(B > 0 && G > 0 && C > 0 && ldd >= C && ldy >= C && (!x_last || ldx >= C), "wmse: bad shape");
   GCL_CHECK_ARG(ws && ws_bytes >= gcl_wmse_ws_bytes(B, G, C), "wmse: workspace too small");
   hipStream_t st = (hipStream_t)stream;
   const int64_t total = (int64_t)B * G * C;
   const unsigned nb = grid_for(total, kLossBlocks);
-  hipLaunchKernelGGL(wmse_kernel, dim3(nb), dim3(256), 0, st, delta, ldd, bsd, x_last, ldx, bsx, y, ldy, bsy, node_w,
-                     chan_w, inv_wsum, grad_scale, d_delta, out_state, (float*)ws, B, G, C);
+  if (outld)
+    hipLaunchKernelGGL(wmse_kernel<true>, dim3(nb), dim3(256), 0, st, delta, ldd, bsd, x_last, ldx, bsx, y, ldy, bsy, node_w,
+                       chan_w, inv_wsum, grad_scale, d_delta, out_state, (float*)ws, B, G, C, ldd_out, bsd_out);
+  else
+    hipLaunchKernelGGL(wmse_kernel<false>, dim3(nb), dim3(256), 0, st, delta, ldd, bsd, x_last, ldx, bsx, y, ldy, bsy, node_w,
+                       chan_w, inv_wsum, grad_scale, d_delta, out_state, (float*)ws, B, G, C, (int64_t)0, (int64_t)0);
   hipLaunchKernelGGL(wmse_final_kernel, dim3(1), dim3(256), 0, st, (const float*)ws, (int)nb, inv_wsum, loss_prev,
                      loss_out);
   GCL_CHECK_LAUNCH();
   return GCL_OK;
+}
+
+extern "C" int gcl_wmse_fwd_bwd(const float* delta, int64_t ldd, int64_t bsd, const float* x_last, int64_t ldx,
+                                int64_t bsx, const float* y, int64_t ldy, int64_t bsy, const float* node_w,
+                                const float* chan_w, float inv_wsum, float grad_scale, float* d_delta,
+                                float* out_state, const float* loss_prev, float* loss_out, int32_t B, int32_t G,
+                                int32_t C, void* ws, size_t ws_bytes, gcl_stream_t stream) {
+  return wmse_impl(delta, ldd, bsd, x_last, ldx, bsx, y, ldy, bsy, node_w, chan_w, inv_wsum, grad_scale, d_delta, false, 0, 0,
+                   out_state, loss_prev, loss_out, B, G, C, ws, ws_bytes, stream);
+}
+
+extern "C" int gcl_wmse_fwd_bwd_ld(const float* delta, int64_t ldd, int64_t bsd, const float* x_last, int64_t ldx,
+                                   int64_t bsx, const float* y, int64_t ldy, int64_t bsy, const float* node_w,
+                                   const float* chan_w, float inv_wsum, float grad_scale, float* d_delta, int64_t ldd_out,
+                                   int64_t bsd_out, float* out_state, const float* loss_prev, float* loss_out, int32_t B,
+                                   int32_t G, int32_t C, void* ws, size_t ws_bytes, gcl_stream_t stream) {
+  GCL_CHECK_ARG(!d_delta || (ldd_out >= C && bsd_out >= (int64_t)(G - 1) * ldd_out + ldd_out),
+                "wmse: output rows overlap (ldd_out=%lld, bsd_out=%lld)", (long long)ldd_out, (long long)bsd_out);
+  return wmse_impl(delta, ldd, bsd, x_last, ldx, bsx, y, ldy, bsy, node_w, chan_w, inv_wsum, grad_scale, d_delta, true, ldd_out,
+                   bsd_out, out_state, loss_prev, loss_out, B, G, C, ws, ws_bytes, stream);
 }
 
 extern "C" int gcl_adam_step(float* p, const float* g, float* m, float* v, int64_t count, float lr, float beta1,
@@ -475,6 +542,27 @@
   return GCL_OK;
 }
 
+extern "C" int gcl_ar_step_bwd_ld(const float* dd, int64_t ldd, int64_t bsd, const float* g_loss, const float* g_new,
+                                  const int32_t* chan_kind, int32_t has_y, int32_t residual, float* d_delta, int64_t ldd_out,
+                                  int64_t bsd_out, float* d_state, int32_t B, int32_t G, int32_t obs, int32_t C,
+                                  gcl_stream_t stream) {
+  GCL_CHECK_ARG(dd && d_delta, "ar_step_bwd: null argument");
+  GCL_CHECK_ARG(B > 0 && G > 0 && obs >= 1 && C > 0 && ldd >= C, "ar_step_bwd: bad shape");
+  GCL_CHECK_ARG(ldd_out >= C && bsd_out >= (int64_t)G * ldd_out, "ar_step_bwd: output rows overlap (ldd_out=%lld, bsd_out=%lld)",
+                (long long)ldd_out, (long long)bsd_out);
+  if (d_state) {
+    const int64_t total = (int64_t)B * G * obs * C;
+    hipLaunchKernelGGL(ar_step_bwd_ld_kernel<true>, dim3(grid_for(total, 8192)), dim3(256), 0, (hipStream_t)stream, dd, ldd,
+                       bsd, g_loss, g_new, chan_kind, has_y, residual, d_delta, ldd_out, bsd_out, d_state, B, G, obs, C);
+  } else {
+    const int64_t total = (int64_t)B * G * C;
+    hipLaunchKernelGGL(ar_step_bwd_ld_kernel<false>, dim3(grid_for(total, 8192)), dim3(256), 0, (hipStream_t)stream, dd, ldd,
+                       bsd, g_loss, g_new, chan_kind, has_y, residual, d_delta, ldd_out, bsd_out, d_state, B, G, obs, C);
+  }
+  GCL_CHECK_LAUNCH();
+  return GCL_OK;
+}
+
 extern "C" int gcl_pad_rows(const float* src, int64_t lds, int64_t bss, int32_t rows_src, int32_t F_src, float* dst,
                             int64_t ldd, int64_t bsd, int32_t rows_dst, int32_t F_dst, int32_t B, gcl_stream_t stream) {
   GCL_CHECK_ARG(src && dst, "pad_rows: null argument");
diff --git a/graphcast-lite_amd/functional.py b/graphcast-lite_amd/functional.py
--- a/graphcast-lite_amd/functional.py
+++ b/graphcast-lite_amd/functional.py
@@ -40,6 +40,35 @@
         with torch.inference_mode(False):
             z = _ZERO[like.device] = torch.zeros((), dtype=torch.float32, device=like.device)
     return z.expand(shape)
+
+
+_ONE = {}
+
+
+def const_one(like: torch.Tensor):
+    one = _ONE.get(like.device)
+    if one is None:
+        if like.is_cuda and torch.cuda.is_current_stream_capturing():
+            return None
+        with torch.inference_mode(False):
+            one = _ONE[like.device] = torch.ones((), dtype=torch.float32, device=like.device)
+    return one
+
+
+def _loss_grad_inplace() -> bool:
+    return os.environ.get("GCL_NO_LOSS_GRAD_INPLACE", "0") != "1"
+
+
+def _wide_in_place(dy: torch.Tensor, Fp: int):
+    if dy.dim() != 3 or dy.dtype != torch.float32 or not dy.is_cuda:
+        return None
+    B, rows, Fo = dy.shape
+    if Fo > Fp or rows == 0 or dy.stride(2) != 1 or dy.stride(1) != Fp or dy.stride(0) != rows * Fp or dy.data_ptr() % 16:
+        return None
+    off = dy.storage_offset()
+    if (off + B * rows * Fp) * 4 > dy.untyped_storage().nbytes():
+        return None
+    return torch.as_strided(dy, (B, rows, Fp), (rows * Fp, Fp, 1), off)
 
 
 def _flat3(x: torch.Tensor):
@@ -294,10 +323,13 @@
         G = _Grads(list(params), needs)
         dy, parts = GradLanding.claim_parts(ctx.split, dy)
         dy, dy_map = GradLanding.claim(ctx.land, dy)
-        dy3 = dy if (dy_map is not None or parts is not None) else _flat3(dy)
+        pad = ctx.pad_last
+        wide = None
+        if pad is not None and dy_map is None and parts is None and _loss_grad_inplace():
+            wide = _wide_in_place(dy, pad[0])
+        dy3 = dy if (dy_map is not None or parts is not None or wide is not None) else _flat3(dy)
         B, n = dy3.shape[0], ctx.n_rows
         ps = ctx.ps
-        pad = ctx.pad_last
         dy_rows = dy3
         if ctx.out_rows and (ctx.has_ln or pad is None):
             dy3 = hip.pad_rows(dy3, n, dy3.shape[2])
@@ -326,11 +358,14 @@
         Fp = Fo
         if pad is not None:
             Fp = pad[0]
-            dp = hip.pad_rows(dy_rows if not ctx.has_ln else dp, n, Fp)
+            dp = hip.pad_rows(dy_rows if not ctx.has_ln else dp, n, Fp) if wide is None else None
         if G.dst[bi_last] is not None and not cs_done:
             src = dy_rows if not ctx.has_ln else dp[..., :Fo]
             if parts is not None:
                 hip.colsum_split(parts[0], parts[1], G.dst[bi_last], G.acc[bi_last])
+            elif wide is not None:
+                hip.colsum(torch.as_strided(dy, (B * dy.shape[1], Fo), (Fp, 1), dy.storage_offset()), G.dst[bi_last],
+                           G.acc[bi_last])
             else:
                 hip.colsum(src.reshape(-1, Fo), G.dst[bi_last], G.acc[bi_last])
         dzc = None
@@ -343,6 +378,8 @@
                 dh2 = hip.aggregate_present(graph, dp, ctx.present, transpose=True).view(B * n, -1)
             elif k == L - 1 and parts is not None:
                 dh2 = hip.aggregate_split(graph, parts[0], parts[1], transpose=True).view(B * n, -1)
+            elif k == L - 1 and wide is not None:
+                dh2 = hip.aggregate_head(graph, wide, transpose=True).view(B * n, -1)
             elif (k == 0 and ctx.lat is not None and ctx.lat.smap is not None and ctx.lat.Md > 0 and _compact_store()
                   and dp.is_contiguous() and hip.aggregate_compact_ok(graph, dp, transpose=True)):
                 dzc = torch.empty(B, ctx.lat.Md + ctx.lat.r, dp.shape[2], dtype=torch.float32, device=dp.device)
@@ -561,8 +598,11 @@
         if d3.stride(2) != 1:
             d3 = d3.contiguous()
         x_last = st[:, :, obs - 1, :] if residual else None
+        ctx.inplace = _loss_grad_inplace()
+        ldp = (Cc + 3) // 4 * 4
+        ctx.ldo = ldp if (ctx.inplace and ldp != Cc and d3.stride(1) == ldp) else None
         loss, dd, _ = hip.wmse_fwd_bwd(d3, x_last, y3, node_w, chan_w, inv_wsum, 1.0, want_grad=True,
-                                       loss_prev=loss_prev.detach() if loss_prev is not None else None)
+                                       loss_prev=loss_prev.detach() if loss_prev is not None else None, ldd_out=ctx.ldo)
         new_state = hip.ar_advance(st, d3, y3, kinds, None, 0, residual) if advance else st.new_empty(0)
         ctx.dd, ctx.kinds, ctx.residual, ctx.advance, ctx.obs, ctx.has_y = dd, kinds, residual, advance, obs, y3 is not None
         if not advance:
@@ -572,8 +612,13 @@
     @staticmethod
     def backward(ctx, g_loss, g_new):
         g_new = g_new if (ctx.advance and g_new is not None and g_new.numel()) else None
+        one = _ONE.get(g_loss.device)
+        if (ctx.inplace and g_new is None and not ctx.needs_input_grad[0] and one is not None
+                and g_loss.data_ptr() == one.data_ptr()):
+            return None, ctx.dd[..., :ctx.dd.shape[2]], None, (g_loss if ctx.needs_input_grad[3] else None), None, None, None, \
+                None, None, None
         d_delta, d_state = hip.ar_step_bwd(ctx.dd, g_loss, g_new, ctx.kinds, ctx.has_y, ctx.residual, ctx.obs,
-                                           want_state=ctx.needs_input_grad[0])
+                                           want_state=ctx.needs_input_grad[0], ldd_out=ctx.ldo)
         return d_state, d_delta, None, (g_loss if ctx.needs_input_grad[3] else None), None, None, None, None, None, None
 
 
diff --git a/graphcast-lite_amd/hip.py b/graphcast-lite_amd/hip.py
--- a/graphcast-lite_amd/hip.py
+++ b/graphcast-lite_amd/hip.py
@@ -52,6 +52,7 @@
     "gcl_aggregate_heavy_launches": (_i64, []),
     "gcl_aggregate_split": (C.c_int, [_vp, _i32, _vp, _i64, _i64, _vp, _i64, _i64, _i32, _vp, _vp, _i64, _i64, _i32, _i32,
                                       _vp]),
+    "gcl_aggregate_head": (C.c_int, [_vp, _i32, _vp, _i64, _i64, _i32, _vp, _vp, _i64, _i64, _i32, _i32, _vp]),
     "gcl_gat_fwd": (C.c_int, [_vp, _vp, _i64, _i64, _vp, _vp, _vp, _vp, _vp, _vp, _vp, _i64, _i64, _i32, _i32, _i32, _vp]),
     "gcl_gat_bwd": (C.c_int, [_vp, _vp, _i64, _i64, _vp, _i64, _i64, _vp, _vp, _vp, _vp, _vp, _vp, _i64, _i64,
                               _vp, _vp, _vp, _i32, _i32, _i32, _i32, _vp, _sz, _vp]),
@@ -84,7 +85,11 @@
     "gcl_assemble_input_tail": (C.c_int, [_vp, _vp, _vp, _vp, _i32, _vp, _i64, _i32, _i32, _i32, _i32, _i32, _vp]),
     "gcl_wmse_fwd_bwd": (C.c_int, [_vp, _i64, _i64, _vp, _i64, _i64, _vp, _i64, _i64, _vp, _vp, _f32, _f32, _vp,
                                    _vp, _vp, _vp, _i32, _i32, _i32, _vp, _sz, _vp]),
+    "gcl_wmse_fwd_bwd_ld": (C.c_int, [_vp, _i64, _i64, _vp, _i64, _i64, _vp, _i64, _i64, _vp, _vp, _f32, _f32, _vp, _i64, _i64,
+                                      _vp, _vp, _vp, _i32, _i32, _i32, _vp, _sz, _vp]),
     "gcl_ar_step_bwd": (C.c_int, [_vp, _vp, _vp, _vp, _i32, _i32, _vp, _vp, _i32, _i32, _i32, _i32, _vp]),
+    "gcl_ar_step_bwd_ld": (C.c_int, [_vp, _i64, _i64, _vp, _vp, _vp, _i32, _i32, _vp, _i64, _i64, _vp, _i32, _i32, _i32, _i32,
+                                     _vp]),
     "gcl_pad_rows": (C.c_int, [_vp, _i64, _i64, _i32, _i32, _vp, _i64, _i64, _i32, _i32, _i32, _vp]),
     "gcl_zero": (C.c_int, [_vp, _sz, _vp]),
     "gcl_wmse_ws_bytes": (_sz, [_i32, _i32, _i32]),
@@ -640,6 +645,19 @@
     return out
 
 
+def aggregate_head(graph: Graph, a3, transpose=False, out=None):
+    B, head, F = a3.shape
+    n = graph.n
+    assert 0 < head <= n and a3.stride(2) == 1
+    if out is None:
+        out = torch.empty(B, n, F, dtype=torch.float32, device=a3.device)
+    tok = _probe_begin("aggregate_head", graph=graph, transpose=bool(transpose), B=B, F=F)
+    _check(lib().gcl_aggregate_head(graph.handle, _agg_flags(transpose), _p(a3), a3.stride(1), a3.stride(0), head, None,
+                                    _p(out), out.stride(1), out.stride(0), B, F, _stream()))
+    _probe_end(tok)
+    return out
+
+
 def layernorm_fwd(x, gamma, beta, eps=1e-5):
     rows, F = x.shape
     y = torch.empty(rows, F, dtype=torch.float32, device=x.device)
@@ -832,21 +850,28 @@
 
 
 def wmse_fwd_bwd(delta3, x_last3, y3, node_w, chan_w, inv_wsum, grad_scale, want_grad=True, want_state=False,
-                 loss_prev=None):
+                 loss_prev=None, ldd_out=None):
     B, G, Cc = delta3.shape
     dev = delta3.device
     if delta3.stride(2) != 1:
         delta3 = delta3.contiguous()
-    dd = torch.empty(B, G, Cc, dtype=torch.float32, device=dev) if want_grad else None
+    dd = None
+    if want_grad:
+        dd = torch.empty(B, G, ldd_out if ldd_out else Cc, dtype=torch.float32, device=dev)
     st = torch.empty(B, G, Cc, dtype=torch.float32, device=dev) if want_state else None
     loss = torch.empty((), dtype=torch.float32, device=dev)
     nb = lib().gcl_wmse_ws_bytes(B, G, Cc)
     ws = workspace(nb, dev)
     xl = x_last3
-    _check(lib().gcl_wmse_fwd_bwd(
-        _p(delta3), delta3.stride(1), delta3.stride(0), _p(xl), xl.stride(1) if xl is not None else 0, xl.stride(0) if xl is not None else 0,
-        _p(y3), y3.stride(1), y3.stride(0), _p(node_w), _p(chan_w), float(inv_wsum), float(grad_scale), _p(dd), _p(st),
-        _p(loss_prev), _p(loss), B, G, Cc, ws.data_ptr(), ws.numel(), _stream()))
+    head = (_p(delta3), delta3.stride(1), delta3.stride(0), _p(xl), xl.stride(1) if xl is not None else 0,
+            xl.stride(0) if xl is not None else 0, _p(y3), y3.stride(1), y3.stride(0), _p(node_w), _p(chan_w), float(inv_wsum),
+            float(grad_scale), _p(dd))
+    tail = (_p(st), _p(loss_prev), _p(loss), B, G, Cc, ws.data_ptr(), ws.numel(), _stream())
+    if ldd_out:
+        assert ldd_out >= Cc
+        _check(lib().gcl_wmse_fwd_bwd_ld(*head, int(ldd_out), G * int(ldd_out), *tail))
+        return loss, (dd[..., :Cc] if dd is not None else None), st
+    _check(lib().gcl_wmse_fwd_bwd(*head, *tail))
     return loss, dd, st
 
 
@@ -973,12 +998,20 @@
     return new_state
 
 
-def ar_step_bwd(dd3, g_loss, g_new4, chan_kind, has_y: bool, residual: bool, obs: int, want_state: bool):
+def ar_step_bwd(dd3, g_loss, g_new4, chan_kind, has_y: bool, residual: bool, obs: int, want_state: bool, ldd_out=None):
     B, G, Cc = dd3.shape
-    d_delta = torch.empty_like(dd3)
     d_state = torch.empty(B, G, obs, Cc, dtype=torch.float32, device=dd3.device) if want_state else None
     if g_new4 is not None and not g_new4.is_contiguous():
         g_new4 = g_new4.contiguous()
+    if ldd_out or not dd3.is_contiguous():
+        assert dd3.stride(2) == 1
+        ldo = int(ldd_out) if ldd_out else Cc
+        d_delta = torch.empty(B, G, ldo, dtype=torch.float32, device=dd3.device)
+        _check(lib().gcl_ar_step_bwd_ld(_p(dd3), dd3.stride(1), dd3.stride(0), _p(g_loss), _p(g_new4), _pi(chan_kind),
+                                        1 if has_y else 0, 1 if residual else 0, _p(d_delta), ldo, G * ldo, _p(d_state), B, G,
+                                        obs, Cc, _stream()))
+        return d_delta[..., :Cc], d_state
+    d_delta = torch.empty_like(dd3)
     _check(lib().gcl_ar_step_bwd(_p(dd3), _p(g_loss), _p(g_new4), _pi(chan_kind), 1 if has_y else 0, 1 if residual else 0,
                                  _p(d_delta), _p(d_state), B, G, obs, Cc, _stream()))
     return d_delta, d_state
diff --git a/graphcast-lite_amd/train.py b/graphcast-lite_amd/train.py
--- a/graphcast-lite_amd/train.py
+++ b/graphcast-lite_amd/train.py
@@ -5,7 +5,7 @@
 
 from . import hip
 from .capture import Captured, graph_enabled
-from .functional import ARStepLossFn, WeightedMSEFn
+from .functional import ARStepLossFn, WeightedMSEFn, const_one
 
 
 class FileNames:
@@ -583,14 +583,9 @@
         return loss.detach()
 
     def _loss_root(self, loss):
-        one = getattr(self, "_one", None)
-        if one is not None and one.device == loss.device and one.dtype == loss.dtype and loss.dim() == 0:
-            return one
-        if loss.dim() != 0 or not loss.is_cuda or torch.cuda.is_current_stream_capturing():
+        if loss.dim() != 0 or not loss.is_cuda or loss.dtype != torch.float32:
             return None
-        with torch.inference_mode(False):
-            self._one = torch.ones((), dtype=loss.dtype, device=loss.device)
-        return self._one
+        return const_one(loss)
 
     def _finish(self):
         scale = allreduce_gradients(self.flat, self.world)
diff --git a/include/gcl.h b/include/gcl.h
--- a/include/gcl.h
+++ b/include/gcl.h
@@ -124,6 +124,8 @@
 int gcl_aggregate_split(const gcl_graph_t* g, int32_t transpose, const float* h, int64_t ldh, int64_t bsh,
                         const float* h2, int64_t ldh2, int64_t bsh2, int32_t head, const float* bias, float* y,
                         int64_t ldy, int64_t bsy, int32_t B, int32_t F, gcl_stream_t stream);
+int gcl_aggregate_head(const gcl_graph_t* g, int32_t transpose, const float* h, int64_t ldh, int64_t bsh, int32_t head,
+                       const float* bias, float* y, int64_t ldy, int64_t bsy, int32_t B, int32_t F, gcl_stream_t stream);
 int gcl_aggregate_compact_ok(const gcl_graph_t* g, int32_t transpose, int64_t ldh, int64_t bsh, int64_t ldy, int64_t bsy,
                              int32_t B, int32_t F);
 int gcl_aggregate_compact(const gcl_graph_t* g, int32_t transpose, const float* h, int64_t ldh, int64_t bsh,
@@ -214,6 +216,11 @@
                      const float* chan_w, float inv_wsum, float grad_scale, float* d_delta,
                      float* out_state, const float* loss_prev, float* loss_out, int32_t B, int32_t G,
                      int32_t C, void* ws, size_t ws_bytes, gcl_stream_t stream);
+int gcl_wmse_fwd_bwd_ld(const float* delta, int64_t ldd, int64_t bsd, const float* x_last, int64_t ldx,
+                        int64_t bsx, const float* y, int64_t ldy_, int64_t bsy, const float* node_w,
+                        const float* chan_w, float inv_wsum, float grad_scale, float* d_delta, int64_t ldd_out,
+                        int64_t bsd_out, float* out_state, const float* loss_prev, float* loss_out, int32_t B,
+                        int32_t G, int32_t C, void* ws, size_t ws_bytes, gcl_stream_t stream);
 size_t gcl_wmse_ws_bytes(int32_t B, int32_t G, int32_t C);
 
 int gcl_adam_step(float* p, const float* g, float* m, float* v, int64_t count, float lr, float beta1,
@@ -282,6 +289,10 @@
 int gcl_ar_step_bwd(const float* dd, const float* g_loss, const float* g_new, const int32_t* chan_kind,
                     int32_t has_y, int32_t residual, float* d_delta, float* d_state, int32_t B, int32_t G,
                     int32_t obs, int32_t C, gcl_stream_t stream);
+int gcl_ar_step_bwd_ld(const float* dd, int64_t ldd, int64_t bsd, const float* g_loss, const float* g_new,
+                       const int32_t* chan_kind, int32_t has_y, int32_t residual, float* d_delta, int64_t ldd_out,
+                       int64_t bsd_out, float* d_state, int32_t B, int32_t G, int32_t obs, int32_t C,
+                       gcl_stream_t stream);
 
 int gcl_pad_rows(const float* src, int64_t lds, int64_t bss, int32_t rows_src, int32_t F_src, float* dst,
                  int64_t ldd, int64_t bsd, int32_t rows_dst, int32_t F_dst, int32_t B, gcl_stream_t stream);
```

After: 27850 (median of 6 runs). 1.02x the previous value.
